# karenyang/GCN-VAE

Hardware: AMD Instinct MI355X
Metric: edges/sec R-GCN forward+backward, FB15k-237 emb=200 (higher is better)
Workload: dtype f32; 1 GPU; FB15k-237-shaped synthetic full graph (BASELINE configs[1]): 14541 entities, 474 directed relation types, E=544230 directed edges on this rank (544230 in the trained graph), 2-layer R-GCN-VAE bdd num_bases=100 emb_dim=200 dropout 0.2, 0 IAF blocks, DistMult decoder on T=220000 triplets per rank, step = fwd + loss(BCE+reg+KL+MMD) + bwd + clip + Adam; edges_per_gpu=544230, trained_graph_edges=544230, nodes=14541, triplets_per_gpu=220000, n_flows=0, gemm_precision=f32, launch=hipgraph, parallelism=single GPU, optimizer=replicated clip + Adam, k1_operands=f32

## Files before the change

### gcn-vae_amd/csrc/k_bdd.hip

```cpp
#include <stdlib.h>

#include "common.h"

namespace gv {

struct AggParams {
    const int4* items;
    int n_items;
    const int* nbr;
    const int* etype;
    const float* coef;
    const int* coef_idx;
    const float* feat;
    int ld_feat;
    const float* w;
    int w_row;
    const float* addend;
    int ld_add;
    int act;
    const uint8_t* keep;
    float keep_scale;
    float* out;
    int ld_out;
    float* partial;
    int out_dim;
    int nb;
    int p, q;
    int nbp;
};

__device__ __forceinline__ int rl_i(int v, int lane) { return __builtin_amdgcn_readlane(v, lane); }
__device__ __forceinline__ float rl_f(float v, int lane) {
    return __int_as_float(__builtin_amdgcn_readlane(__float_as_int(v), lane));
}


template <int P, int Q, bool TRANS, int BPL>
__device__ __forceinline__ void block_fma(const float (&x)[BPL * P], const float (&w)[BPL * P * Q], float c,
                                          float (&acc)[BPL * Q]) {
#pragma unroll
    for (int b = 0; b < BPL; ++b) {
#pragma unroll
        for (int q = 0; q < Q; ++q) {
            float t = 0.f;
#pragma unroll
            for (int p = 0; p < P; ++p) {
                const float wv = TRANS ? w[b * P * Q + q * P + p] : w[b * P * Q + p * Q + q];
                t = fmaf(x[b * P + p], wv, t);
            }
            acc[b * Q + q] = fmaf(t, c, acc[b * Q + q]);
        }
    }
}

template <int P, int Q, bool TRANS, int BPL, int U>
__global__ __launch_bounds__(256) void k_agg_fast(const AggParams a) {
    constexpr int GV = BPL * P, PV = BPL * Q, WV = BPL * P * Q;
    constexpr bool RUNS = P * Q >= 4;
    const int lane = threadIdx.x & 63;
    const int wave = __builtin_amdgcn_readfirstlane((int)(blockIdx.x * (blockDim.x >> 6) + (threadIdx.x >> 6)));
    if (wave >= a.n_items) return;
    const int4 it = a.items[wave];
    if (it.x < 0) return;
    if (it.w >= 0 && !a.partial) return;
    const bool active = lane * BPL < a.nbp;
    const int blk0 = blockIdx.y * a.nbp + lane * BPL;
    const float* __restrict__ fbase = a.feat + blk0 * P;
    const float* __restrict__ wbase = a.w + blk0 * (P * Q);

    float acc[PV];
#pragma unroll
    for (int i = 0; i < PV; ++i) acc[i] = 0.f;
    float wkeep[WV];
#pragma unroll
    for (int i = 0; i < WV; ++i) wkeep[i] = 0.f;
    int r_keep = -1;

    for (int e0 = it.y; e0 < it.z; e0 += 64) {
        const int cnt = min(64, it.z - e0);
        int my_n = 0, my_t = 0;
        float my_c = 1.f;
        if (lane < cnt) {
            my_n = a.nbr[e0 + lane];
            my_t = a.etype[e0 + lane];
            if (a.coef) my_c = a.coef_idx ? a.coef[a.coef_idx[e0 + lane]] : a.coef[e0 + lane];
// ... 634 lines not shown
#pragma unroll
                    for (int q = 0; q < QS; ++q) acc[p * QS + q] = fmaf(xc, gvv[q], acc[p * QS + q]);
                }
            }
        }
    }
    if (!active) return;
    float* o = (it.w >= 0 ? a.partial + (size_t)it.w * a.w_row : a.grad_w + (size_t)it.x * a.w_row) + blk * (P * Q) + sub * QS;
#pragma unroll
    for (int p = 0; p < P; ++p) {
        float t[QS];
#pragma unroll
        for (int q = 0; q < QS; ++q) t[q] = acc[p * QS + q];
        if (it.w < 0 && a.accumulate) {
            float old[QS];
            load_vec<QS>(o + p * Q, old);
#pragma unroll
            for (int q = 0; q < QS; ++q) t[q] += old[q];
        }
        store_vec<QS>(o + p * Q, t);
    }
}


__global__ __launch_bounds__(256) void k_gradw_generic(const GradWParams a) {
    const int lane = threadIdx.x & 63;
    const int wave = __builtin_amdgcn_readfirstlane((int)(blockIdx.x * (blockDim.x >> 6) + (threadIdx.x >> 6)));
    if (wave >= a.n_items) return;
    const int4 it = a.items[wave];
    if (it.x < 0) return;
    if (it.w >= 0 && !a.partial) return;
    const int P = a.p, Q = a.q;
    for (int c0 = 0; c0 < a.w_row; c0 += 64) {
        const int c = c0 + lane;
        const bool active = c < a.w_row;
        const int b = active ? c / (P * Q) : 0;
        const int rem = c - b * P * Q;
        const int p = rem / Q, q = rem - p * Q;
        float acc = 0.f;
        for (int e0 = it.y; e0 < it.z; e0 += 64) {
            const int cnt = min(64, it.z - e0);
            int my_s = 0, my_d = 0;
            float my_c = 1.f;
            if (lane < cnt) {
                my_s = a.src[e0 + lane];
                my_d = a.dst[e0 + lane];
                if (a.coef) my_c = a.coef_idx ? a.coef[a.coef_idx[e0 + lane]] : a.coef[e0 + lane];
            }
            for (int j = 0; j < cnt; ++j) {
                const int s = rl_i(my_s, j);
                const int d = rl_i(my_d, j);
                const float cf = rl_f(my_c, j);
                if (active)
                    acc = fmaf(a.x[(size_t)s * a.ld_x + b * P + p] * cf, a.g[(size_t)d * a.ld_g + b * Q + q], acc);
            }
        }
        if (!active) continue;
        if (it.w >= 0) {
            a.partial[(size_t)it.w * a.w_row + c] = acc;
        } else {
            float* o = a.grad_w + (size_t)it.x * a.w_row + c;
            *o = a.accumulate ? *o + acc : acc;
        }
    }
}

__global__ __launch_bounds__(256) void k_gradw_fixup(const int4* fix, int n_fix, const float* partial, int w_row,
                                                     float* grad_w, int accumulate) {
    const int lane = threadIdx.x & 63;
    const int tiles = (w_row + 63) >> 6;
    const int wave = __builtin_amdgcn_readfirstlane((int)(blockIdx.x * (blockDim.x >> 6) + (threadIdx.x >> 6)));
    if (wave >= n_fix * tiles) return;
    const int4 f = fix[wave / tiles];
    if (f.x < 0) return;
    const int c = (wave % tiles) * 64 + lane;
    if (c >= w_row) return;
    const float acc = ordered_slot_sum(partial + (size_t)f.y * w_row + c, f.z, w_row);
    float* o = grad_w + (size_t)f.x * w_row + c;
    *o = accumulate ? *o + acc : acc;
}

__global__ __launch_bounds__(256) void k_gradw_fixup4(const int4* fix, int n_fix, const float* partial, int w_row,
                                                      float* grad_w, int accumulate) {
    const int lane = threadIdx.x & 63;
    const int quads = w_row >> 2, tiles = (quads + 63) >> 6;
    const int wave = __builtin_amdgcn_readfirstlane((int)(blockIdx.x * (blockDim.x >> 6) + (threadIdx.x >> 6)));
    if (wave >= n_fix * tiles) return;
    const int4 f = fix[wave / tiles];
    if (f.x < 0) return;
    const int c4 = (wave % tiles) * 64 + lane;
    if (c4 >= quads) return;
    const float4* __restrict__ p = reinterpret_cast<const float4*>(partial + (size_t)f.y * w_row) + c4;
    const size_t stride = (size_t)quads;
    const int n = f.z;
    float4 a0 = make_float4(0.f, 0.f, 0.f, 0.f), a1 = a0, a2 = a0, a3 = a0;
    auto add = [](float4& a, const float4& v) { a.x += v.x; a.y += v.y; a.z += v.z; a.w += v.w; };
    int k = 0;
    for (; k + 8 <= n; k += 8) {
        const float4 v0 = p[(size_t)(k + 0) * stride], v1 = p[(size_t)(k + 1) * stride];
        const float4 v2 = p[(size_t)(k + 2) * stride], v3 = p[(size_t)(k + 3) * stride];
        const float4 v4 = p[(size_t)(k + 4) * stride], v5 = p[(size_t)(k + 5) * stride];
        const float4 v6 = p[(size_t)(k + 6) * stride], v7 = p[(size_t)(k + 7) * stride];
        add(a0, v0); add(a1, v1); add(a2, v2); add(a3, v3);
        add(a0, v4); add(a1, v5); add(a2, v6); add(a3, v7);
    }
    for (; k < n; ++k) add(a0, p[(size_t)k * stride]);
    float4 acc = make_float4((a0.x + a1.x) + (a2.x + a3.x), (a0.y + a1.y) + (a2.y + a3.y), (a0.z + a1.z) + (a2.z + a3.z),
                             (a0.w + a1.w) + (a2.w + a3.w));
    float4* o = reinterpret_cast<float4*>(grad_w + (size_t)f.x * w_row) + c4;
    if (accumulate) {
        const float4 t = *o;
        acc.x = t.x + acc.x; acc.y = t.y + acc.y; acc.z = t.z + acc.z; acc.w = t.w + acc.w;
    }
    *o = acc;
}

__global__ void k_items_count(const int* rowptr, int n_seg, int chunk, int* n_chunks, int* n_slots, int* is_split) {
    const int s = blockIdx.x * blockDim.x + threadIdx.x;
    if (s >= n_seg) return;
    const int deg = rowptr[s + 1] - rowptr[s];
    const int nch = max(1, (deg + chunk - 1) / chunk);
    n_chunks[s] = nch;
    n_slots[s] = nch > 1 ? nch : 0;
    is_split[s] = nch > 1 ? 1 : 0;
}

__global__ void k_items_fill(const int* rowptr, int n_seg, int chunk, const int* item_off, const int* slot_off,
                             const int* fix_off, int4* items, int4* fix) {
    const int s = blockIdx.x * blockDim.x + threadIdx.x;
    if (s >= n_seg) return;
    const int beg = rowptr[s], end = rowptr[s + 1];
    const int nch = max(1, (end - beg + chunk - 1) / chunk);
    const int ib = item_off[s];
    for (int k = 0; k < nch; ++k) {
        const int b = beg + k * chunk;
        items[ib + k] = make_int4(s, b, min(end, b + chunk), nch > 1 ? slot_off[s] + k : -1);
    }
    if (nch > 1) fix[fix_off[s]] = make_int4(s, slot_off[s], nch, 0);
}

template <typename K, typename Pm>
static int launch_items(K kern, const Pm& p, int n_items, hipStream_t st, const char* what, int parts = 1) {
    if (n_items <= 0) return GV_OK;
    const int waves_per_block = 4;
    dim3 grid((n_items + waves_per_block - 1) / waves_per_block, parts), block(64 * waves_per_block);
    hipLaunchKernelGGL(kern, grid, block, 0, st, p);
    return launch_status(what);
}

}

using namespace gv;

extern "C" int gv_segment_items_count(const int32_t* rowptr, int n_seg, int chunk, int32_t* n_chunks,
                                      int32_t* n_slots, int32_t* is_split, void* stream) {
    GV_REQUIRE(rowptr && n_chunks && n_slots && is_split, GV_ERR_NULL, "gv_segment_items_count: NULL pointer");
    GV_REQUIRE(n_seg >= 0 && chunk > 0, GV_ERR_SHAPE, "gv_segment_items_count: n_seg=%d chunk=%d", n_seg, chunk);
    if (n_seg == 0) return GV_OK;
    hipLaunchKernelGGL(k_items_count, dim3((n_seg + 255) / 256), dim3(256), 0, (hipStream_t)stream, rowptr, n_seg,
                       chunk, n_chunks, n_slots, is_split);
    return launch_status("gv_segment_items_count");
}

extern "C" int gv_segment_items_fill(const int32_t* rowptr, int n_seg, int chunk, const int32_t* item_off,
                                     const int32_t* slot_off, const int32_t* fix_off, int32_t* items, int32_t* fix,
                                     void* stream) {
    GV_REQUIRE(rowptr && item_off && slot_off && fix_off && items, GV_ERR_NULL, "gv_segment_items_fill: NULL pointer");
    GV_REQUIRE(n_seg >= 0 && chunk > 0, GV_ERR_SHAPE, "gv_segment_items_fill: n_seg=%d chunk=%d", n_seg, chunk);
    if (n_seg == 0) return GV_OK;
    hipLaunchKernelGGL(k_items_fill, dim3((n_seg + 255) / 256), dim3(256), 0, (hipStream_t)stream, rowptr, n_seg,
                       chunk, item_off, slot_off, fix_off, (int4*)items, (int4*)fix);
    return launch_status("gv_segment_items_fill");
}

namespace {
struct LanePlan { int bpl; int parts; };
bool lane_plan(int nb, int p, LanePlan* out, bool aggregate = false) {
    int cands[3] = {0, 0, 0};
    switch (p) {
        case 1: cands[0] = 4; cands[1] = 2; break;
        case 2: cands[0] = 2; cands[1] = 4; cands[2] = 1; break;
        case 4: cands[0] = 1; cands[1] = 2; break;
        case 8: cands[0] = 1; break;
        case 5: {
            static const int bpl1 = getenv("GV_K1_BPL1") ? atoi(getenv("GV_K1_BPL1")) : 1;
            if (bpl1 && aggregate) { cands[0] = 1; cands[1] = 2; } else cands[0] = 2;
            break;
        }
        case 10: cands[0] = 1; break;
        default: return false;
    }
    for (int c = 0; c < 3 && cands[c]; ++c) {
        const int bpl = cands[c];
        if (nb % bpl) continue;
        const int lanes = nb / bpl;
        for (int parts = 1; parts <= 16; ++parts) {
            if (lanes % parts) continue;
// ... 130 lines not shown
    const bool has_plan = lane_plan(num_bases, blk_in, &lp, true);
    const int bpl = has_plan ? lp.bpl : 0;
    if (rc == -1000) a.nbp = has_plan ? num_bases / lp.parts : num_bases;
#define GV_AGG_CASE(P_, Q_, T_, B_, U_)                                                               \
    if (rc == -1000 && vec_ok && blk_in == P_ && blk_out == Q_ && (transpose_w != 0) == T_ && bpl == B_) \
        rc = launch_items(k_agg_fast<P_, Q_, T_, B_, U_>, a, n_items, st, "gv_rgcn_bdd_aggregate", lp.parts);
#define GV_AGG_U(P_, Q_, T_, B_)                                                                              \
    if (rc == -1000 && u_env && vec_ok && blk_in == P_ && blk_out == Q_ && (transpose_w != 0) == T_ && bpl == B_) { \
        if (u_env == 2) rc = launch_items(k_agg_fast<P_, Q_, T_, B_, 2>, a, n_items, st, "agg(U2)", lp.parts);          \
        if (u_env == 4) rc = launch_items(k_agg_fast<P_, Q_, T_, B_, 4>, a, n_items, st, "agg(U4)", lp.parts);          \
        if (u_env == 8) rc = launch_items(k_agg_fast<P_, Q_, T_, B_, 8>, a, n_items, st, "agg(U8)", lp.parts);          \
    }
    GV_AGG_U(2, 2, false, 2) GV_AGG_U(2, 4, false, 2) GV_AGG_U(2, 2, true, 2) GV_AGG_U(4, 2, true, 2)
#undef GV_AGG_U
    GV_AGG_CASE(1, 1, false, 4, 8)
    GV_AGG_CASE(1, 2, false, 4, 4)
    GV_AGG_CASE(2, 2, false, 2, 8)
    GV_AGG_CASE(2, 4, false, 2, 4)
    GV_AGG_CASE(4, 4, false, 1, 4)
    GV_AGG_CASE(4, 4, false, 2, 2)
    GV_AGG_CASE(4, 8, false, 1, 2)
    GV_AGG_CASE(4, 8, false, 2, 2)
    GV_AGG_CASE(1, 1, true, 4, 8)
    GV_AGG_CASE(2, 1, true, 2, 8)
    GV_AGG_CASE(2, 2, true, 2, 8)
    GV_AGG_CASE(4, 2, true, 1, 8)
    GV_AGG_CASE(4, 2, true, 2, 4)
    GV_AGG_CASE(4, 4, true, 1, 4)
    GV_AGG_CASE(4, 4, true, 2, 2)
    GV_AGG_CASE(8, 4, true, 1, 2)
    GV_AGG_CASE(5, 5, false, 1, 2)
    GV_AGG_CASE(5, 10, false, 1, 2)
    GV_AGG_CASE(5, 5, true, 1, 2)
    GV_AGG_CASE(5, 5, false, 2, 2)
    GV_AGG_CASE(5, 10, false, 2, 1)
    GV_AGG_CASE(5, 5, true, 2, 2)
    GV_AGG_CASE(10, 5, true, 1, 1)
    GV_AGG_CASE(10, 10, false, 1, 1)
    GV_AGG_CASE(10, 10, true, 1, 1)
#undef GV_AGG_CASE
    if (rc == -1000) {
        if (transpose_w)
            rc = launch_items(k_agg_generic<true>, a, n_items, st, "gv_rgcn_bdd_aggregate(generic)");
        else
            rc = launch_items(k_agg_generic<false>, a, n_items, st, "gv_rgcn_bdd_aggregate(generic)");
    }
    if (rc != GV_OK) return rc;
    if (n_fix > 0) {
        const int pairs = n_fix * ((a.out_dim + 63) / 64);
        hipLaunchKernelGGL(k_agg_fixup, dim3(pairs), dim3(pairs >= 65536 ? 1024 : 256), 0, st, (const int4*)fix, n_fix, partial,
                           a.out_dim, addend, ld_addend, act, keep, keep_scale, out, ld_out);
        return launch_status("gv_rgcn_bdd_aggregate(fixup)");
    }
    return GV_OK;
}

extern "C" int gv_rgcn_bdd_fixup(const int32_t* fix, int n_fix, const float* partial, int out_dim, const float* addend,
                                 int ld_addend, int act, const uint8_t* keep, float keep_scale, float* out, int ld_out,
                                 void* stream) {
    GV_REQUIRE(n_fix >= 0, GV_ERR_SHAPE, "gv_rgcn_bdd_fixup: negative count");
    if (n_fix == 0) return GV_OK;
    GV_REQUIRE(fix && partial && out, GV_ERR_NULL, "gv_rgcn_bdd_fixup: NULL pointer");
    const int pairs = n_fix * ((out_dim + 63) / 64);
    hipLaunchKernelGGL(k_agg_fixup, dim3(pairs), dim3(pairs >= 65536 ? 1024 : 256), 0, (hipStream_t)stream, (const int4*)fix, n_fix,
                       partial, out_dim, addend, ld_addend, act, keep, keep_scale, out, ld_out);
    return launch_status("gv_rgcn_bdd_fixup");
}

extern "C" int gv_rgcn_bdd_grad_weight(const int32_t* items, int n_items, const int32_t* fix, int n_fix,
                                       const int32_t* src, const int32_t* dst, const float* coef,
                                       const int32_t* coef_idx, const float* x, int ld_x, const float* g, int ld_g,
                                       int num_bases, int blk_in, int blk_out, float* grad_w, float* partial,
                                       int accumulate, void* stream) {
    GV_REQUIRE(n_items >= 0 && n_fix >= 0, GV_ERR_SHAPE, "gv_rgcn_bdd_grad_weight: negative item count");
    if (n_items == 0) return GV_OK;
    GV_REQUIRE(items && x && g && grad_w, GV_ERR_NULL, "gv_rgcn_bdd_grad_weight: NULL pointer");
    GV_REQUIRE(num_bases > 0 && blk_in > 0 && blk_out > 0, GV_ERR_SHAPE, "gv_rgcn_bdd_grad_weight: bad block sizes");
    GV_REQUIRE(n_fix == 0 || (fix && partial), GV_ERR_NULL, "gv_rgcn_bdd_grad_weight: split segments need fix+partial");
    GV_REQUIRE(ld_x >= num_bases * blk_in && ld_g >= num_bases * blk_out, GV_ERR_SHAPE,
               "gv_rgcn_bdd_grad_weight: leading dimension smaller than the row");
    GradWParams a;
    a.items = (const int4*)items; a.n_items = n_items; a.src = src; a.dst = dst; a.coef = coef; a.coef_idx = coef_idx;
    a.x = x; a.ld_x = ld_x; a.g = g; a.ld_g = ld_g; a.grad_w = grad_w; a.w_row = num_bases * blk_in * blk_out;
    a.partial = partial; a.accumulate = accumulate; a.nb = num_bases; a.p = blk_in; a.q = blk_out;
    hipStream_t st = (hipStream_t)stream;
    const bool vec_ok = aligned16(x) && aligned16(g) && aligned16(grad_w) && (ld_x % 4 == 0) && (ld_g % 4 == 0) &&
                        (!partial || aligned16(partial)) && (a.w_row % 4 == 0);
    int rc = -1000;
#define GV_GW_SPLIT(P_, Q_, QS_, U_, PARTS_)                                                                              \
    if (rc == -1000 && vec_ok && blk_in == P_ && blk_out == Q_ && num_bases % PARTS_ == 0 && num_bases <= 32 &&          \
        (num_bases / PARTS_) * (Q_ / QS_) <= 64) {                                                                        \
        a.nbp = num_bases / PARTS_;                                                                                       \
        rc = launch_items(k_gradw_split<P_, Q_, QS_, U_>, a, n_items, st, "gv_rgcn_bdd_grad_weight(split)", PARTS_);      \
    }
    GV_GW_SPLIT(10, 10, 5, 2, 1) GV_GW_SPLIT(10, 20, 4, 2, 2)
#undef GV_GW_SPLIT
    LanePlan lp{0, 1};
    const bool has_plan = lane_plan(num_bases, blk_in, &lp, blk_in == 5 && blk_out >= 10);
    const int bpl = has_plan ? lp.bpl : 0;
    if (rc == -1000) a.nbp = has_plan ? num_bases / lp.parts : num_bases;
#define GV_GW_CASE(P_, Q_, B_, U_)                                                  \
    if (rc == -1000 && vec_ok && blk_in == P_ && blk_out == Q_ && bpl == B_)        \
        rc = launch_items(k_gradw_fast<P_, Q_, B_, U_>, a, n_items, st, "gv_rgcn_bdd_grad_weight", lp.parts);
    GV_GW_CASE(1, 1, 4, 8)
    GV_GW_CASE(1, 2, 4, 4)
    GV_GW_CASE(2, 2, 2, 8)
    GV_GW_CASE(2, 4, 2, 4)
    GV_GW_CASE(4, 4, 1, 4)
    GV_GW_CASE(4, 4, 2, 2)
    GV_GW_CASE(4, 8, 1, 2)
    GV_GW_CASE(4, 8, 2, 2)
    GV_GW_CASE(5, 5, 2, 2)
    GV_GW_CASE(5, 10, 2, 1)
    GV_GW_CASE(5, 10, 1, 2)
    GV_GW_CASE(10, 10, 1, 1)
#undef GV_GW_CASE
    if (rc == -1000) rc = launch_items(k_gradw_generic, a, n_items, st, "gv_rgcn_bdd_grad_weight(generic)");
    if (rc != GV_OK) return rc;
    if (n_fix > 0) {
        if (a.w_row % 4 == 0 && aligned16(partial) && aligned16(grad_w)) {
            const int waves = n_fix * ((a.w_row / 4 + 63) / 64);
            hipLaunchKernelGGL(k_gradw_fixup4, dim3((waves + 3) / 4), dim3(256), 0, st, (const int4*)fix, n_fix, partial,
                               a.w_row, grad_w, accumulate);
        } else {
            const int waves = n_fix * ((a.w_row + 63) / 64);
            hipLaunchKernelGGL(k_gradw_fixup, dim3((waves + 3) / 4), dim3(256), 0, st, (const int4*)fix, n_fix, partial,
                               a.w_row, grad_w, accumulate);
        }
        return launch_status("gv_rgcn_bdd_grad_weight(fixup)");
    }
    return GV_OK;
}
```

### gcn-vae_amd/csrc/k_gemm.hip

```cpp
#include <limits.h>
#include <stdlib.h>

#include <algorithm>

#include "common.h"

namespace gv {


typedef float f32x16 __attribute__((ext_vector_type(16)));

struct GemmParams {
    const float* a;
    const float* b;
    float* c;
    const float* bias;
    const float* a_mask;
    float* ws;
    int m, n, k, lda, ldb, ldc;
    int act, accumulate, split_k, k_chunk;
    int vec_a, vec_b;
    const int* rows_dev;
    const unsigned long long* kmask;
    const unsigned long long* tmask;
    int tmask_ld;
    int tmask_wanted;
};

template <int VPT>
__device__ __forceinline__ void load_run(const float* src, int pos, int lim, bool ok, bool vec, float (&r)[VPT], int off) {
#pragma unroll
    for (int h = 0; h < VPT / 4; ++h) {
        const int q = pos + 4 * h;
        if (ok && vec && q + 3 < lim) {
            const float4 v = *reinterpret_cast<const float4*>(src + 4 * h);
            r[off + 4 * h] = v.x; r[off + 4 * h + 1] = v.y; r[off + 4 * h + 2] = v.z; r[off + 4 * h + 3] = v.w;
        } else {
#pragma unroll
            for (int i = 0; i < 4; ++i) r[off + 4 * h + i] = (ok && q + i < lim) ? src[4 * h + i] : 0.f;
        }
    }
}

template <int VPT>
__device__ __forceinline__ void mask_run(const float* msk, int pos, int lim, bool ok, bool vec, float (&r)[VPT]) {
    float mv[VPT];
    load_run<VPT>(msk, pos, lim, ok, vec, mv, 0);
#pragma unroll
    for (int i = 0; i < VPT; ++i) r[i] = mv[i] > 0.f ? r[i] : 0.f;
}

template <bool TA, int BM, int BK>
__device__ __forceinline__ void load_a(const GemmParams& p, int m0, int k0, int kend, float (&r)[BM * BK / 256]) {
    constexpr int APT = BM * BK / 256;
    const int t = threadIdx.x;
    if constexpr (!TA) {
        constexpr int TPR = BK / APT;
        const int m = m0 + t / TPR, kk = k0 + (t % TPR) * APT;
        load_run<APT>(p.a + (size_t)m * p.lda + kk, kk, kend, m < p.m, p.vec_a, r, 0);
        if (p.a_mask) mask_run<APT>(p.a_mask + (size_t)m * p.lda + kk, kk, kend, m < p.m, p.vec_a, r);
    } else {
        constexpr int TPK = BM / APT;
        const int kq = k0 + t / TPK, m = m0 + (t % TPK) * APT;
        load_run<APT>(p.a + (size_t)kq * p.lda + m, m, p.m, kq < kend, p.vec_a, r, 0);
        if (p.a_mask) mask_run<APT>(p.a_mask + (size_t)kq * p.lda + m, m, p.m, kq < kend, p.vec_a, r);
    }
}

template <bool TB, int BN, int BK>
__device__ __forceinline__ void load_b(const GemmParams& p, int n0, int k0, int kend, float (&r)[BN * BK / 256]) {
    constexpr int BPT = BN * BK / 256;
    const int t = threadIdx.x;
    if constexpr (!TB) {
        constexpr int TPK = BN / BPT;
        const int kq = k0 + t / TPK, n = n0 + (t % TPK) * BPT;
        load_run<BPT>(p.b + (size_t)kq * p.ldb + n, n, p.n, kq < kend, p.vec_b, r, 0);
    } else {
        constexpr int TPN = BK / BPT;
        const int n = n0 + t / TPN, kq = k0 + (t % TPN) * BPT;
        load_run<BPT>(p.b + (size_t)n * p.ldb + kq, kq, kend, n < p.n, p.vec_b, r, 0);
    }
}

template <bool TA, int BM, int BK>
__device__ __forceinline__ void stage_a(float* As, const float (&r)[BM * BK / 256]) {
    constexpr int APT = BM * BK / 256, LDA_S = BM + 1;
    const int t = threadIdx.x;
    if constexpr (!TA) {
// ... 670 lines not shown
    const float* src = base + (size_t)row * ld + kk;
    load_run<8>(src, kk, kend, ok, vec, r, 0);
    if (mask) mask_run<8>(mask + (size_t)row * ld + kk, kk, kend, ok, vec, r);
}

__device__ __forceinline__ void hb_load_ks(const float* base, const float* mask, int ld, int row0, int rows, int k0, int kend,
                                           float (&r)[8]) {
    const int t = threadIdx.x;
    const int row = row0 + (t & 63), kk = k0 + (t >> 6) * 8;
    const bool ok = row < rows;
#pragma unroll
    for (int j = 0; j < 8; ++j) {
        const bool in = ok && kk + j < kend;
        float v = in ? base[(size_t)(kk + j) * ld + row] : 0.f;
        if (mask && in) v = mask[(size_t)(kk + j) * ld + row] > 0.f ? v : 0.f;
        r[j] = v;
    }
}

template <bool KC>
__device__ __forceinline__ void hb_stage(__bf16* S, const float (&r)[8]) {
    const int t = threadIdx.x;
    const int row = KC ? (t >> 2) : (t & 63), kk = KC ? (t & 3) * 8 : (t >> 6) * 8;
    bf16x8 v;
#pragma unroll
    for (int j = 0; j < 8; ++j) v[j] = (__bf16)r[j];
    *reinterpret_cast<bf16x8*>(S + row * HB_LD + kk) = v;
}

template <bool TA, bool TB>
__global__ __launch_bounds__(256) void k_gemm_bf16(const GemmParams p) {
    __shared__ __attribute__((aligned(16))) __bf16 As[64 * HB_LD];
    __shared__ __attribute__((aligned(16))) __bf16 Bs[64 * HB_LD];
    const int m0 = blockIdx.y * 64, n0 = blockIdx.x * 64;
    const int kbeg = blockIdx.z * p.k_chunk;
    const int kend = min(p.k, kbeg + p.k_chunk);
    const int lane = threadIdx.x & 63, wid = threadIdx.x >> 6;
    const int wm = (wid >> 1) * 32, wn = (wid & 1) * 32;
    const int l31 = lane & 31, lhi = lane >> 5;
    f32x16 acc;
#pragma unroll
    for (int i = 0; i < 16; ++i) acc[i] = 0.f;

    float ra[8], rb[8];
    auto load_tiles = [&](int k0) {
        if constexpr (!TA) hb_load_kc(p.a, p.a_mask, p.lda, m0, p.m, k0, kend, p.vec_a, ra);
        else hb_load_ks(p.a, p.a_mask, p.lda, m0, p.m, k0, kend, ra);
        if constexpr (TB) hb_load_kc(p.b, nullptr, p.ldb, n0, p.n, k0, kend, p.vec_b, rb);
        else hb_load_ks(p.b, nullptr, p.ldb, n0, p.n, k0, kend, rb);
    };
    load_tiles(kbeg);
    for (int k0 = kbeg; k0 < kend; k0 += HB_BK) {
        hb_stage<!TA>(As, ra);
        hb_stage<TB>(Bs, rb);
        __syncthreads();
        if (k0 + HB_BK < kend) load_tiles(k0 + HB_BK);
#pragma unroll
        for (int kk = 0; kk < HB_BK; kk += 16) {
            const bf16x8 af = *reinterpret_cast<const bf16x8*>(As + (wm + l31) * HB_LD + kk + 8 * lhi);
            const bf16x8 bf = *reinterpret_cast<const bf16x8*>(Bs + (wn + l31) * HB_LD + kk + 8 * lhi);
            acc = __builtin_amdgcn_mfma_f32_32x32x16_bf16(af, bf, acc, 0, 0, 0);
        }
        __syncthreads();
    }
    const int col = n0 + wn + l31;
    if (col >= p.n) return;
    const float bv = (p.bias && p.split_k == 1) ? p.bias[col] : 0.f;
#pragma unroll
    for (int r = 0; r < 16; ++r) {
        const int row = m0 + wm + (r & 3) + 8 * (r >> 2) + 4 * lhi;
        if (row >= p.m) continue;
        float v = acc[r];
        if (p.split_k > 1) {
            p.ws[((size_t)blockIdx.z * p.m + row) * p.n + col] = v;
        } else {
            v = apply_act(v + bv, p.act);
            float* dst = p.c + (size_t)row * p.ldc + col;
            *dst = p.accumulate ? *dst + v : v;
        }
    }
}

__global__ __launch_bounds__(256) void k_gemm_splitk_reduce(const GemmParams p) {
    const size_t total = (size_t)p.m * p.n;
    for (size_t i = (size_t)blockIdx.x * blockDim.x + threadIdx.x; i < total; i += (size_t)gridDim.x * blockDim.x) {
        float a0 = 0.f, a1 = 0.f, a2 = 0.f, a3 = 0.f;
        int z = 0;
        for (; z + 8 <= p.split_k; z += 8) {
            float t[8];
#pragma unroll
            for (int q = 0; q < 8; ++q) t[q] = p.ws[(size_t)(z + q) * total + i];
            a0 += t[0]; a1 += t[1]; a2 += t[2]; a3 += t[3];
            a0 += t[4]; a1 += t[5]; a2 += t[6]; a3 += t[7];
        }
        for (; z < p.split_k; ++z) a0 += p.ws[(size_t)z * total + i];
        float v = (a0 + a1) + (a2 + a3);
        const int row = (int)(i / p.n), col = (int)(i - (size_t)row * p.n);
        if (p.tmask_wanted > 0) {
            const int bit = (row >> 6) * p.tmask_ld + (col >> 6);
            if (!((p.tmask[bit >> 6] >> (bit & 63)) & 1ull)) v = 0.f;
        }
        if (p.bias) v += p.bias[col];
        v = apply_act(v, p.act);
        float* dst = p.c + (size_t)row * p.ldc + col;
        *dst = p.accumulate ? *dst + v : v;
    }
}

constexpr int COLSUM_SLICES = 64;

__global__ __launch_bounds__(256) void k_colsum_part(const float* x, const float* msk, int64_t m, int n, int ld, float* part) {
    __shared__ float sm[4][64];
    const int lane = threadIdx.x & 63, w = threadIdx.x >> 6;
    const int c = blockIdx.x * 64 + lane;
    const int64_t per = (m + gridDim.y - 1) / gridDim.y;
    const int64_t r0 = blockIdx.y * per, r1 = min(m, r0 + per);
    float a0 = 0.f, a1 = 0.f, a2 = 0.f, a3 = 0.f;
    if (c < n) {
        int64_t r = r0 + w;
        if (msk) {
            for (; r + 12 < r1; r += 16) {
                const float v0 = x[r * ld + c], v1 = x[(r + 4) * ld + c], v2 = x[(r + 8) * ld + c], v3 = x[(r + 12) * ld + c];
                const float m0 = msk[r * ld + c], m1 = msk[(r + 4) * ld + c], m2 = msk[(r + 8) * ld + c], m3 = msk[(r + 12) * ld + c];
                a0 += m0 > 0.f ? v0 : 0.f; a1 += m1 > 0.f ? v1 : 0.f; a2 += m2 > 0.f ? v2 : 0.f; a3 += m3 > 0.f ? v3 : 0.f;
            }
            for (; r < r1; r += 4) a0 += msk[r * ld + c] > 0.f ? x[r * ld + c] : 0.f;
        } else {
            for (; r + 12 < r1; r += 16) {
                const float v0 = x[r * ld + c], v1 = x[(r + 4) * ld + c], v2 = x[(r + 8) * ld + c], v3 = x[(r + 12) * ld + c];
                a0 += v0; a1 += v1; a2 += v2; a3 += v3;
            }
            for (; r < r1; r += 4) a0 += x[r * ld + c];
        }
    }
    sm[w][lane] = (a0 + a1) + (a2 + a3);
    __syncthreads();
    if (w == 0 && c < n) part[(size_t)blockIdx.y * n + c] = (sm[0][lane] + sm[1][lane]) + (sm[2][lane] + sm[3][lane]);
}

__global__ __launch_bounds__(256) void k_colsum_final(const float* part, int n, int nsl, float* out, int accumulate) {
    const int c = blockIdx.x * blockDim.x + threadIdx.x;
    if (c >= n) return;
    float a0 = 0.f, a1 = 0.f, a2 = 0.f, a3 = 0.f;
    int s = 0;
    for (; s + 4 <= nsl; s += 4) {
        const float v0 = part[(size_t)s * n + c], v1 = part[(size_t)(s + 1) * n + c];
        const float v2 = part[(size_t)(s + 2) * n + c], v3 = part[(size_t)(s + 3) * n + c];
        a0 += v0; a1 += v1; a2 += v2; a3 += v3;
    }
    for (; s < nsl; ++s) a0 += part[(size_t)s * n + c];
    const float acc = (a0 + a1) + (a2 + a3);
    out[c] = accumulate ? out[c] + acc : acc;
}

__global__ __launch_bounds__(1024) void k_colsum_final_wide(const float* part, int n, int nsl, float* out, int accumulate) {
    __shared__ float sm[64][16];
    const int c = blockIdx.x * 16 + (threadIdx.x & 15);
    const float acc = sum_slices_16x64(part, n, nsl, c, sm);
    if ((threadIdx.x >> 4) == 0 && c < n) out[c] = accumulate ? out[c] + acc : acc;
}

}

using namespace gv;

static int k_chunk_for(int k, int split_k) {
    int per = (k + split_k - 1) / split_k;
    return ((per + 31) / 32) * 32;
}

extern "C" int64_t gv_gemm_workspace_bytes(int m, int n, int k, int split_k) {
    (void)k;
    return split_k > 1 ? (int64_t)split_k * m * n * (int64_t)sizeof(float) : 0;
}

static int gemm_any(bool bf16, int trans_a, int trans_b, int m, int n, int k, const float* a, int lda, const float* b,
                    int ldb, float* c, int ldc, const float* bias, int act, int accumulate, int split_k,
                    const float* a_relu_mask, void* workspace, int64_t workspace_bytes, void* stream, const int32_t* rows_dev = nullptr,
                    const uint64_t* kmask = nullptr, const uint64_t* tmask = nullptr, int tiles_wanted = 0) {
    GV_REQUIRE(m >= 0 && n >= 0 && k >= 0, GV_ERR_SHAPE, "gv_gemm_f32: negative size");
    if (m == 0 || n == 0) return GV_OK;
    GV_REQUIRE(c && (k == 0 || (a && b)), GV_ERR_NULL, "gv_gemm_f32: NULL matrix");
    GV_REQUIRE(lda >= (trans_a ? m : k) && ldb >= (trans_b ? k : n) && ldc >= n, GV_ERR_SHAPE,
               "gv_gemm_f32: leading dimension too small (lda=%d ldb=%d ldc=%d)", lda, ldb, ldc);
    GV_REQUIRE(act == GV_ACT_NONE || act == GV_ACT_RELU, GV_ERR_SHAPE, "gv_gemm_f32: unknown act %d", act);
    if (split_k < 1) split_k = 1;
    if (k == 0) split_k = 1;
    GemmParams p;
    p.a = a; p.b = b; p.c = c; p.bias = bias; p.a_mask = a_relu_mask; p.ws = (float*)workspace;
    p.m = m; p.n = n; p.k = k; p.lda = lda; p.ldb = ldb; p.ldc = ldc;
    p.act = act; p.accumulate = accumulate;
    p.k_chunk = k_chunk_for(k > 0 ? k : 1, split_k);
    split_k = k > 0 ? (k + p.k_chunk - 1) / p.k_chunk : 1;
    p.split_k = split_k;
    p.vec_a = aligned16(a) && (lda % 4 == 0) && (!a_relu_mask || aligned16(a_relu_mask));
    p.vec_b = aligned16(b) && (ldb % 4 == 0);
    p.rows_dev = bf16 ? nullptr : rows_dev;
    GV_REQUIRE(!kmask || (!bf16 && split_k == 1 && k <= 64 * 16), GV_ERR_SHAPE,
               "gv_gemm_f32_sparse: k-chunk words cover fp32 products of k <= 1024 without split-K (k=%d split_k=%d)", k, split_k);
    GV_REQUIRE(!tmask || !bf16, GV_ERR_SHAPE, "gv_gemm_f32_sparse: fp32 only");
    p.kmask = (const unsigned long long*)kmask;
    p.tmask = (const unsigned long long*)tmask;
    p.tmask_ld = (n + 63) / 64;
    GV_REQUIRE(tiles_wanted >= 0 && tiles_wanted <= ((m + 63) / 64) * ((n + 63) / 64), GV_ERR_SHAPE, "gv_gemm_f32_sparse: c_tiles_wanted=%d", tiles_wanted);
    p.tmask_wanted = (tmask && tiles_wanted > 0 && split_k > 1) ? tiles_wanted : 0;
    if (split_k > 1) {
        GV_REQUIRE(workspace, GV_ERR_NULL, "gv_gemm_f32: split_k needs a workspace");
        GV_REQUIRE(workspace_bytes >= gv_gemm_workspace_bytes(m, n, k, split_k), GV_ERR_WORKSPACE,
                   "gv_gemm_f32: workspace %lld < %lld bytes", (long long)workspace_bytes,
                   (long long)gv_gemm_workspace_bytes(m, n, k, split_k));
    }
    hipStream_t st = (hipStream_t)stream;
    if (bf16) {
        dim3 grid((n + 63) / 64, (m + 63) / 64, split_k), block(256);
        if (!trans_a && !trans_b) hipLaunchKernelGGL((k_gemm_bf16<false, false>), grid, block, 0, st, p);
        else if (!trans_a && trans_b) hipLaunchKernelGGL((k_gemm_bf16<false, true>), grid, block, 0, st, p);
        else if (trans_a && !trans_b) hipLaunchKernelGGL((k_gemm_bf16<true, false>), grid, block, 0, st, p);
        else hipLaunchKernelGGL((k_gemm_bf16<true, true>), grid, block, 0, st, p);
        int rcb = launch_status("gv_gemm_bf16");
        if (rcb != GV_OK) return rcb;
        if (split_k > 1) {
            const size_t total = (size_t)m * n;
            const int blocks = (int)min((size_t)2048, (total + 255) / 256);
            hipLaunchKernelGGL(k_gemm_splitk_reduce, dim3(blocks), dim3(256), 0, st, p);
            return launch_status("gv_gemm_bf16(split-k reduce)");
        }
        return GV_OK;
    }
    static const int mt_env = getenv("GV_GEMM_MT") ? atoi(getenv("GV_GEMM_MT")) : 0;
    static const int nt_env = getenv("GV_GEMM_NT") ? atoi(getenv("GV_GEMM_NT")) : 0;
    static const int bk_env = getenv("GV_GEMM_BK") ? atoi(getenv("GV_GEMM_BK")) : 0;
    const int nt = (nt_env == 2 && !kmask && !(tmask && tiles_wanted > 0 && split_k > 1)) ? 2 : 1;
    const int bn = 64 * nt;
    const long blocks128 = (long)((n + bn - 1) / bn) * ((m + 127) / 128) * split_k;
    const int mt = p.tmask_wanted ? 1 : (mt_env ? mt_env : (blocks128 >= 1024 ? 2 : 1));
    static const int sparse_bk = getenv("GV_GEMM_SPARSE_BK") ? atoi(getenv("GV_GEMM_SPARSE_BK")) : 16;
    const int bk = kmask ? (sparse_bk == 32 ? 32 : 16) : (bk_env ? (bk_env == 16 ? 16 : 32) : (trans_a ? 32 : 16));
    dim3 grid((n + bn - 1) / bn, (m + 64 * mt - 1) / (64 * mt), split_k), block(256);
    if (p.tmask_wanted) { grid.x = p.tmask_wanted; grid.y = 1; }
#define GV_GEMM_CFG(TA_, TB_, MT_, NT_, BK_) \
    if (mt == MT_ && nt == NT_ && bk == BK_) hipLaunchKernelGGL((k_gemm_f32<TA_, TB_, MT_, NT_, BK_>), grid, block, 0, st, p);
#define GV_GEMM_LAUNCH(TA_, TB_)                                                                       \
    do {                                                                                               \
        GV_GEMM_CFG(TA_, TB_, 1, 1, 16) GV_GEMM_CFG(TA_, TB_, 1, 1, 32) GV_GEMM_CFG(TA_, TB_, 1, 2, 16) \
        GV_GEMM_CFG(TA_, TB_, 1, 2, 32) GV_GEMM_CFG(TA_, TB_, 2, 1, 16) GV_GEMM_CFG(TA_, TB_, 2, 1, 32) \
        GV_GEMM_CFG(TA_, TB_, 2, 2, 16) GV_GEMM_CFG(TA_, TB_, 2, 2, 32)                                 \
    } while (0)
    if (!trans_a && !trans_b) GV_GEMM_LAUNCH(false, false);
    else if (!trans_a && trans_b) GV_GEMM_LAUNCH(false, true);
    else if (trans_a && !trans_b) GV_GEMM_LAUNCH(true, false);
    else GV_GEMM_LAUNCH(true, true);
#undef GV_GEMM_LAUNCH
#undef GV_GEMM_CFG
    int rc = launch_status("gv_gemm_f32");
    if (rc != GV_OK) return rc;
    if (split_k > 1) {
        const size_t total = (size_t)m * n;
        const int blocks = (int)min((size_t)2048, (total + 255) / 256);
        hipLaunchKernelGGL(k_gemm_splitk_reduce, dim3(blocks), dim3(256), 0, st, p);
        return launch_status("gv_gemm_f32(split-k reduce)");
    }
    return GV_OK;
}

extern "C" int gv_gemm_f32(int trans_a, int trans_b, int m, int n, int k, const float* a, int lda, const float* b,
                           int ldb, float* c, int ldc, const float* bias, int act, int accumulate, int split_k,
                           const float* a_relu_mask, void* workspace, int64_t workspace_bytes, void* stream) {
    return gemm_any(false, trans_a, trans_b, m, n, k, a, lda, b, ldb, c, ldc, bias, act, accumulate, split_k, a_relu_mask,
                    workspace, workspace_bytes, stream);
}

extern "C" int gv_gemm_f32_live_rows(int trans_a, int trans_b, int m, int n, int k, const float* a, int lda, const float* b,
                                     int ldb, float* c, int ldc, const float* bias, int act, int accumulate, int split_k,
                                     const float* a_relu_mask, void* workspace, int64_t workspace_bytes, const int32_t* rows_dev,
                                     void* stream) {
    return gemm_any(false, trans_a, trans_b, m, n, k, a, lda, b, ldb, c, ldc, bias, act, accumulate, split_k, a_relu_mask,
                    workspace, workspace_bytes, stream, rows_dev);
}

extern "C" int gv_gemm_f32_sparse(int trans_a, int trans_b, int m, int n, int k, const float* a, int lda, const float* b, int ldb,
                                  float* c, int ldc, const float* bias, int act, int accumulate, int split_k, const float* a_relu_mask,
                                  void* workspace, int64_t workspace_bytes, const int32_t* rows_dev, const uint64_t* b_k_chunks,
                                  const uint64_t* c_tiles, int c_tiles_wanted, void* stream) {
    return gemm_any(false, trans_a, trans_b, m, n, k, a, lda, b, ldb, c, ldc, bias, act, accumulate, split_k, a_relu_mask,
                    workspace, workspace_bytes, stream, rows_dev, b_k_chunks, c_tiles, c_tiles_wanted);
}

extern "C" int gv_gemm_bf16(int trans_a, int trans_b, int m, int n, int k, const float* a, int lda, const float* b,
                            int ldb, float* c, int ldc, const float* bias, int act, int accumulate, int split_k,
                            const float* a_relu_mask, void* workspace, int64_t workspace_bytes, void* stream) {
    return gemm_any(true, trans_a, trans_b, m, n, k, a, lda, b, ldb, c, ldc, bias, act, accumulate, split_k, a_relu_mask,
                    workspace, workspace_bytes, stream);
}

extern "C" int gv_rank_scores(const float* q, int ld_q, const float* e, int ld_e, const int* target, const float* bias,
                              float* tgt, int* count, int m, int v, int h, void* stream) {
    GV_REQUIRE(m >= 0 && v > 0 && h > 0, GV_ERR_SHAPE, "gv_rank_scores: m=%d v=%d h=%d", m, v, h);
    if (m == 0) return GV_OK;
    GV_REQUIRE(q && e && target && tgt && count, GV_ERR_NULL, "gv_rank_scores: NULL pointer");
    GV_REQUIRE(ld_q >= h && ld_e >= h, GV_ERR_SHAPE, "gv_rank_scores: leading dimension too small");
    RankParams rp;
    GemmParams& p = rp.g;
    p.a = q; p.b = e; p.c = nullptr; p.bias = nullptr; p.a_mask = nullptr; p.ws = nullptr;
    p.m = m; p.n = v; p.k = h; p.lda = ld_q; p.ldb = ld_e; p.ldc = v;
    p.act = GV_ACT_NONE; p.accumulate = 0; p.split_k = 1; p.k_chunk = h;
    p.vec_a = aligned16(q) && (ld_q % 4 == 0);
    p.vec_b = aligned16(e) && (ld_e % 4 == 0);
    p.rows_dev = nullptr; p.kmask = nullptr; p.tmask = nullptr; p.tmask_ld = 0; p.tmask_wanted = 0;
    rp.target = target; rp.bias = bias; rp.tgt = tgt; rp.count = count;
    hipStream_t st = (hipStream_t)stream;
    if (fill_words(count, 0u, (size_t)m * sizeof(int), st) != hipSuccess) return launch_status("gv_rank_scores(fill)");
    dim3 grid((v + 63) / 64, (m + 63) / 64), block(256);
    hipLaunchKernelGGL(k_rank_scores<0>, grid, block, 0, st, rp);
    hipLaunchKernelGGL(k_rank_scores<1>, grid, block, 0, st, rp);
    return launch_status("gv_rank_scores");
}

extern "C" int gv_rank_scores_filtered(const float* q, int ld_q, const float* e, int ld_e, const int* target, const float* bias,
                                       const int* filt_lo, const int* filt_hi, const int* filt_ent, int n_filt_ent, float* tgt,
                                       int* count_raw, int* count_filt, int m, int v, int h, void* stream) {
    GV_REQUIRE(m >= 0 && v > 0 && h > 0 && n_filt_ent >= 0, GV_ERR_SHAPE, "gv_rank_scores_filtered: m=%d v=%d h=%d n_filt_ent=%d",
               m, v, h, n_filt_ent);
    if (m == 0) return GV_OK;
    GV_REQUIRE(q && e && target && tgt && count_filt, GV_ERR_NULL, "gv_rank_scores_filtered: NULL pointer");
    GV_REQUIRE(filt_lo && filt_hi && filt_ent, GV_ERR_NULL, "gv_rank_scores_filtered: NULL filter pointer");
    GV_REQUIRE(ld_q >= h && ld_e >= h, GV_ERR_SHAPE, "gv_rank_scores_filtered: leading dimension too small");
    RankFiltParams fp;
    RankParams& rp = fp.rp;
    GemmParams& p = rp.g;
    p.a = q; p.b = e; p.c = nullptr; p.bias = nullptr; p.a_mask = nullptr; p.ws = nullptr;
    p.m = m; p.n = v; p.k = h; p.lda = ld_q; p.ldb = ld_e; p.ldc = v;
    p.act = GV_ACT_NONE; p.accumulate = 0; p.split_k = 1; p.k_chunk = h;
    p.vec_a = aligned16(q) && (ld_q % 4 == 0);
    p.vec_b = aligned16(e) && (ld_e % 4 == 0);
    p.rows_dev = nullptr; p.kmask = nullptr; p.tmask = nullptr; p.tmask_ld = 0; p.tmask_wanted = 0;
    rp.target = target; rp.bias = bias; rp.tgt = tgt; rp.count = count_raw;
    fp.filt_lo = filt_lo; fp.filt_hi = filt_hi; fp.filt_ent = filt_ent; fp.n_ent = n_filt_ent; fp.count_filt = count_filt;
    hipStream_t st = (hipStream_t)stream;
    if (count_raw && fill_words(count_raw, 0u, (size_t)m * sizeof(int), st) != hipSuccess)
// ... 118 lines not shown
```

### gcn-vae_amd/csrc/k_loss.hip

```cpp
#include "common.h"

namespace gv {

constexpr int RED_BLOCKS = 1024;

__device__ __forceinline__ float block_sum_256(float v, float* sm ) {
    v = wave_sum(v);
    const int lane = threadIdx.x & 63, w = threadIdx.x >> 6;
    __syncthreads();
    if (lane == 0) sm[w] = v;
    __syncthreads();
    return sm[0] + sm[1] + sm[2] + sm[3];
}

__global__ __launch_bounds__(256) void k_final_sum(const float* part, int n, float scale, float* out, int accumulate) {
    __shared__ float sm[4];
    float acc = 0.f;
    for (int i = threadIdx.x; i < n; i += 256) acc += part[i];
    const float tot = block_sum_256(acc, sm);
    if (threadIdx.x == 0) *out = accumulate ? *out + scale * tot : scale * tot;
}

__global__ __launch_bounds__(256) void k_loss_combine(const float* p0, int n0, float s0, const float* p1, int n1, float s1,
                                                      const float* p2, int n2, float s2, const float* p3, int n3, float s3,
                                                      float w1, float w2, float w3, float* scal, float* loss,
                                                      const int* rows_dev, float rows_host) {
    __shared__ float sm[4];
    const float* ps[4] = {p0, p1, p2, p3};
    const int ns[4] = {n0, n1, n2, n3};
    if (rows_dev) s2 *= rows_host / (float)*rows_dev;
    const float ss[4] = {s0, s1, s2, s3};
    float term[4];
#pragma unroll
    for (int j = 0; j < 4; ++j) {
        float acc = 0.f;
        if (ps[j])
            for (int i = threadIdx.x; i < ns[j]; i += 256) acc += ps[j][i];
        term[j] = ss[j] * block_sum_256(acc, sm);
    }
    if (threadIdx.x == 0) {
        if (scal) { scal[0] = term[0]; scal[1] = term[1]; scal[2] = term[2]; scal[3] = term[3]; }
        float v = term[0];
        if (p1) v += w1 * term[1];
        if (p2) v += w2 * term[2];
        if (p3) v += w3 * term[3];
        *loss = v;
    }
}

__global__ __launch_bounds__(256) void k_distmult_bce(const float* e, int ld_e, const float* w, int ld_w,
                                                      const int* trip, const int* order, const float* labels,
                                                      const float* bias, float* score, float* part, int64_t T, int h) {
    __shared__ float sm[4];
    const int sub = threadIdx.x & 15;
    const float bv = bias ? *bias : 0.f;
    const bool vec = (h % 4 == 0) && (ld_e % 4 == 0) && (ld_w % 4 == 0);
    float lsum = 0.f;
    const int n_x = gridDim.x >= 8 ? 8 : 1;
    const int64_t per = (T + n_x - 1) / n_x;
    const int64_t lo = (blockIdx.x % n_x) * per, hi = min(T, lo + per);
    const int brank = blockIdx.x / n_x, bper = (gridDim.x + n_x - 1 - (blockIdx.x % n_x)) / n_x;
    auto triplet_dot = [&](int64_t t) -> float {
        const int s = trip[3 * t], r = trip[3 * t + 1], o = trip[3 * t + 2];
        const float* es = e + (size_t)s * ld_e;
        const float* eo = e + (size_t)o * ld_e;
        const float* wr = w + (size_t)r * ld_w;
        float acc = 0.f;
        if (vec && h <= 256) {
            float4 a[4], b[4], d[4];
#pragma unroll
            for (int q = 0; q < 4; ++q) {
                const int c = sub * 4 + 64 * q;
                if (c < h) {
                    a[q] = *reinterpret_cast<const float4*>(es + c);
                    b[q] = *reinterpret_cast<const float4*>(wr + c);
                    d[q] = *reinterpret_cast<const float4*>(eo + c);
                }
            }
#pragma unroll
            for (int q = 0; q < 4; ++q) {
                if (sub * 4 + 64 * q < h) {
                    acc = fmaf(a[q].x * b[q].x, d[q].x, acc);
                    acc = fmaf(a[q].y * b[q].y, d[q].y, acc);
// ... 616 lines not shown
                    *reinterpret_cast<float4*>(gh2 + r * 2 * h + h + col) = make_float4(o1[0], o1[1], o1[2], o1[3]);
                } else {
                    *reinterpret_cast<float4*>(gz + r * h + col) = make_float4(o0[0], o0[1], o0[2], o0[3]);
                    *reinterpret_cast<float4*>(gm + r * h + col) = make_float4(o1[0], o1[1], o1[2], o1[3]);
                    *reinterpret_cast<float4*>(gv + r * h + col) = make_float4(o2[0], o2[1], o2[2], o2[3]);
                }
            }
        }
    }
    for (int j0 = 0; j0 < k; j0 += KLB_KR) {
        __syncthreads();
#pragma unroll
        for (int j = 0; j < KT; ++j) {
            if (j >= j0 && j < j0 + KLB_KR && j < k) {
                red[((2 * (j - j0)) * KLB_WAVES + w) * 64 + lane] = make_float4(amu[j][0], amu[j][1], amu[j][2], amu[j][3]);
                red[((2 * (j - j0) + 1) * KLB_WAVES + w) * 64 + lane] = make_float4(av[j][0], av[j][1], av[j][2], av[j][3]);
            }
        }
        __syncthreads();
        const int j = j0 + (w >> 1), kind = w & 1;
        if (w < 2 * KLB_KR && j < k && ok) {
            float4 t = red[((2 * (j - j0) + kind) * KLB_WAVES) * 64 + lane];
#pragma unroll
            for (int q = 1; q < KLB_WAVES; ++q) {
                const float4 x = red[((2 * (j - j0) + kind) * KLB_WAVES + q) * 64 + lane];
                t.x += x.x; t.y += x.y; t.z += x.z; t.w += x.w;
            }
            float4 o;
            if (kind == 0) {
                const float4 i24 = si2[j * h4];
                o = make_float4(-t.x * 2.f * i24.x, -t.y * 2.f * i24.y, -t.z * 2.f * i24.z, -t.w * 2.f * i24.w);
            } else {
                o = make_float4(-t.x, -t.y, -t.z, -t.w);
            }
            *reinterpret_cast<float4*>(part + ((size_t)blockIdx.y * 2 * k + (kind ? k : 0) + j) * h + col) = o;
        }
    }
}

__global__ __launch_bounds__(256) void k_kl_bwd_mix_part(const float* z, const float* mix, const float* resp,
                                                         float* part, int64_t n, int h, int k) {
    __shared__ float sm[2][4][64];
    const int j = blockIdx.x, slice = blockIdx.z, nsl = gridDim.z;
    const int lane = threadIdx.x & 63, w = threadIdx.x >> 6;
    const int c = blockIdx.y * 64 + lane;
    const int64_t per = (n + nsl - 1) / nsl;
    const int64_t r0 = slice * per, r1 = min(n, r0 + per);
    const int kh = k * h;
    float gmu0 = 0.f, gmu1 = 0.f, gv0 = 0.f, gv1 = 0.f;
    const bool ok = c < h;
    const float muj = ok ? mix[j * h + c] : 0.f, i2 = ok ? mix[kh + j * h + c] : 0.f;
    if (ok) {
        int64_t r = r0 + w;
        for (; r + 4 < r1; r += 8) {
            const float ra = resp[r * k + j], rb = resp[(r + 4) * k + j];
            const float da = z[r * h + c] - muj, db = z[(r + 4) * h + c] - muj;
            gmu0 += ra * da;
            gmu1 += rb * db;
            gv0 += ra * (da * da * 2.f * i2 * i2 - i2);
            gv1 += rb * (db * db * 2.f * i2 * i2 - i2);
        }
        for (; r < r1; r += 4) {
            const float ra = resp[r * k + j];
            const float da = z[r * h + c] - muj;
            gmu0 += ra * da;
            gv0 += ra * (da * da * 2.f * i2 * i2 - i2);
        }
    }
    sm[0][w][lane] = gmu0 + gmu1;
    sm[1][w][lane] = gv0 + gv1;
    __syncthreads();
    if (w == 0 && ok) {
        const float gmu = (sm[0][0][lane] + sm[0][1][lane]) + (sm[0][2][lane] + sm[0][3][lane]);
        const float gvv = (sm[1][0][lane] + sm[1][1][lane]) + (sm[1][2][lane] + sm[1][3][lane]);
        part[((size_t)slice * 2 * k + j) * h + c] = -gmu * 2.f * i2;
        part[((size_t)slice * 2 * k + k + j) * h + c] = -gvv;
    }
}

__global__ __launch_bounds__(1024) void k_kl_bwd_mix_final(const float* part, const float* z_pre, const float* gkl,
                                                           float gscale, float* g_zpre, int accumulate, int64_t n, int h,
                                                           int k, int nsl, const int* rows_dev) {
    __shared__ float sm[64][16];
    const int total = 2 * k * h, kh = k * h;
    const int i = blockIdx.x * 16 + (threadIdx.x & 15);
    float acc = sum_slices_16x64(part, total, nsl, i, sm);
    if ((threadIdx.x >> 4) != 0 || i >= total) return;
    const float cg = gscale * (gkl ? *gkl : 1.f) / (float)(rows_dev ? (int64_t)*rows_dev : n);
    if (i >= kh) {
        const float raw = z_pre[i];
        acc *= raw > 20.f ? 1.f : 1.f / (1.f + expf(-raw));
    }
    g_zpre[i] = accumulate ? g_zpre[i] + cg * acc : cg * acc;
}

constexpr int MMD_WAVES = 16;

template <int CPL>
__device__ __forceinline__ void mmd_load_row(const float* p, int h, int lane, float (&v)[CPL]) {
#pragma unroll
    for (int i = 0; i < CPL; ++i) v[i] = (lane + 64 * i < h) ? p[lane + 64 * i] : 0.f;
}

template <int CPL>
__device__ __forceinline__ float mmd_d2(const float (&a)[CPL], const float (&b)[CPL]) {
    float d2 = 0.f;
#pragma unroll
    for (int i = 0; i < CPL; ++i) { const float d = a[i] - b[i]; d2 = fmaf(d, d, d2); }
    return d2;
}

template <int CPL>
__global__ __launch_bounds__(64 * MMD_WAVES) void k_mmd_fwd(const float* x, const float* y, const int64_t* yidx, int sx, int sy,
                                                             int h, float* part) {
    __shared__ float sm[MMD_WAVES];
    const int lane = threadIdx.x & 63, w = threadIdx.x >> 6;
    const bool is_x = (int)blockIdx.x < sx;
    auto row_of = [&](bool from_y, int j) -> const float* {
        return from_y ? y + (size_t)(yidx ? yidx[j] : j) * h : x + (size_t)j * h;
    };
    float av[CPL];
    mmd_load_row<CPL>(row_of(!is_x, is_x ? (int)blockIdx.x : (int)blockIdx.x - sx), h, lane, av);
    const float inv = 1.f / ((float)h * (float)h);
    float tot = 0.f;
    for (int pass = 0; pass < (is_x ? 2 : 1); ++pass) {
        const bool b_is_y = pass == 0 ? !is_x : true;
        const int nb = pass == 0 ? (is_x ? sx : sy) : sy;
        const float wt = pass == 0 ? 1.f / ((float)nb * (float)nb) : -2.f / ((float)sx * (float)sy);
        for (int j = w; j < nb; j += 4 * MMD_WAVES) {
            float b0[CPL], b1[CPL], b2[CPL], b3[CPL];
            const int j1 = j + MMD_WAVES, j2 = j + 2 * MMD_WAVES, j3 = j + 3 * MMD_WAVES;
            mmd_load_row<CPL>(row_of(b_is_y, j), h, lane, b0);
            mmd_load_row<CPL>(row_of(b_is_y, min(j1, nb - 1)), h, lane, b1);
            mmd_load_row<CPL>(row_of(b_is_y, min(j2, nb - 1)), h, lane, b2);
            mmd_load_row<CPL>(row_of(b_is_y, min(j3, nb - 1)), h, lane, b3);
            const float d0 = wave_sum(mmd_d2<CPL>(av, b0)), d1 = wave_sum(mmd_d2<CPL>(av, b1));
            const float d2 = wave_sum(mmd_d2<CPL>(av, b2)), d3 = wave_sum(mmd_d2<CPL>(av, b3));
            tot += wt * expf(-d0 * inv);
            if (j1 < nb) tot += wt * expf(-d1 * inv);
            if (j2 < nb) tot += wt * expf(-d2 * inv);
            if (j3 < nb) tot += wt * expf(-d3 * inv);
        }
    }
    if (lane == 0) sm[w] = tot;
    __syncthreads();
    if (threadIdx.x == 0) {
        float s = 0.f;
#pragma unroll
        for (int i = 0; i < MMD_WAVES; ++i) s += sm[i];
        part[blockIdx.x] = s;
    }
}

template <int CPL>
__global__ __launch_bounds__(64 * MMD_WAVES) void k_mmd_bwd(const float* x, const float* y, const int64_t* yidx, int sx, int sy,
                                                             int h, const float* gmmd, float gscale, float* gx, float* gy) {
    __shared__ float sm[MMD_WAVES][64 * CPL];
    const int lane = threadIdx.x & 63, w = threadIdx.x >> 6;
    const bool is_x = (int)blockIdx.x < sx;
    const int row = is_x ? blockIdx.x : blockIdx.x - sx;
    auto row_of = [&](bool from_y, int j) -> const float* {
        return from_y ? y + (size_t)(yidx ? yidx[j] : j) * h : x + (size_t)j * h;
    };
    float av[CPL], acc[CPL];
    mmd_load_row<CPL>(row_of(!is_x, row), h, lane, av);
#pragma unroll
    for (int i = 0; i < CPL; ++i) acc[i] = 0.f;
    const float inv = 1.f / ((float)h * (float)h);
    const float g = gscale * (gmmd ? *gmmd : 1.f);
    const int n_same = is_x ? sx : sy, n_other = is_x ? sy : sx;
    const float c_same = g * (-2.f * inv) * 2.f / ((float)n_same * (float)n_same);
    const float c_other = g * (-2.f * inv) * (-2.f) / ((float)sx * (float)sy);
    for (int pass = 0; pass < 2; ++pass) {
        const bool b_is_y = pass == 0 ? !is_x : is_x;
        const int nb = pass == 0 ? n_same : n_other;
        const float cf = pass == 0 ? c_same : c_other;
// ... 101 lines not shown
#pragma unroll
    for (int g = 0; g < G; ++g) { col[g] = 4 * (l16 + 16 * g); on[g] = col[g] < h; }
    float4 av[G], acc[G];
    mmd_load_row4<G>(row_of(!is_x, row), on, col, av);
#pragma unroll
    for (int g = 0; g < G; ++g) acc[g] = make_float4(0.f, 0.f, 0.f, 0.f);
    const float inv = 1.f / ((float)h * (float)h);
    const float gg = gscale * (gmmd ? *gmmd : 1.f);
    const int n_same = is_x ? sx : sy, n_other = is_x ? sy : sx;
    const float c_same = gg * (-2.f * inv) * 2.f / ((float)n_same * (float)n_same);
    const float c_other = gg * (-2.f * inv) * (-2.f) / ((float)sx * (float)sy);
    for (int pass = 0; pass < 2; ++pass) {
        const bool b_is_y = pass == 0 ? !is_x : is_x;
        const int nb = pass == 0 ? n_same : n_other;
        const float cf = pass == 0 ? c_same : c_other;
        for (int j0 = 0; j0 < nb; j0 += 2 * NG) {
            const int j = j0 + grp, j1 = j + NG;
            float4 b0[G], b1[G];
            mmd_load_row4<G>(row_of(b_is_y, min(j, nb - 1)), on, col, b0);
            mmd_load_row4<G>(row_of(b_is_y, min(j1, nb - 1)), on, col, b1);
            const float d0 = row16_sum(mmd_d2_4<G>(av, b0)), d1 = row16_sum(mmd_d2_4<G>(av, b1));
            const float k0 = j < nb ? cf * expf(-d0 * inv) : 0.f, k1 = j1 < nb ? cf * expf(-d1 * inv) : 0.f;
#pragma unroll
            for (int g = 0; g < G; ++g) {
                acc[g].x = fmaf(k0, av[g].x - b0[g].x, fmaf(k1, av[g].x - b1[g].x, acc[g].x));
                acc[g].y = fmaf(k0, av[g].y - b0[g].y, fmaf(k1, av[g].y - b1[g].y, acc[g].y));
                acc[g].z = fmaf(k0, av[g].z - b0[g].z, fmaf(k1, av[g].z - b1[g].z, acc[g].z));
                acc[g].w = fmaf(k0, av[g].w - b0[g].w, fmaf(k1, av[g].w - b1[g].w, acc[g].w));
            }
        }
    }
#pragma unroll
    for (int g = 0; g < G; ++g) {
        float4 t;
        t.x = (rl_dyn(acc[g].x, l16) + rl_dyn(acc[g].x, 16 + l16)) + (rl_dyn(acc[g].x, 32 + l16) + rl_dyn(acc[g].x, 48 + l16));
        t.y = (rl_dyn(acc[g].y, l16) + rl_dyn(acc[g].y, 16 + l16)) + (rl_dyn(acc[g].y, 32 + l16) + rl_dyn(acc[g].y, 48 + l16));
        t.z = (rl_dyn(acc[g].z, l16) + rl_dyn(acc[g].z, 16 + l16)) + (rl_dyn(acc[g].z, 32 + l16) + rl_dyn(acc[g].z, 48 + l16));
        t.w = (rl_dyn(acc[g].w, l16) + rl_dyn(acc[g].w, 16 + l16)) + (rl_dyn(acc[g].w, 32 + l16) + rl_dyn(acc[g].w, 48 + l16));
        if (lane < 16) sm[w][l16 + 16 * g] = t;
    }
    __syncthreads();
    const bool indexed = !is_x && yidx;
    float* o = is_x ? gx + (size_t)row * h : gy + (size_t)(yidx ? yidx[row] : row) * h;
    for (int q = threadIdx.x; q < (h >> 2); q += 64 * MMD_WAVES) {
        float4 s4 = sm[0][q];
#pragma unroll
        for (int i = 1; i < MMD_WAVES; ++i) { const float4 t = sm[i][q]; s4.x += t.x; s4.y += t.y; s4.z += t.z; s4.w += t.w; }
        if (indexed) {
            atomicAdd(o + 4 * q, s4.x); atomicAdd(o + 4 * q + 1, s4.y); atomicAdd(o + 4 * q + 2, s4.z); atomicAdd(o + 4 * q + 3, s4.w);
        } else {
            *reinterpret_cast<float4*>(o + 4 * q) = s4;
        }
    }
}

__global__ __launch_bounds__(256) void k_prior_sample_fwd(const float* z_pre, const float* eps, float* out, int s, int k, int h) {
    const int total = s * h;
    for (int i = blockIdx.x * 256 + threadIdx.x; i < total; i += gridDim.x * 256) {
        const int r = i / h, c = i - r * h, j = r % k;
        const float v = softplus_t(z_pre[(size_t)(k + j) * h + c]) + 1e-8f;
        out[i] = z_pre[(size_t)j * h + c] + eps[i] * sqrtf(v);
    }
}

__global__ __launch_bounds__(256) void k_prior_sample_bwd(const float* z_pre, const float* eps, const float* g, float* gz_pre,
                                                          int accumulate, int s, int k, int h) {
    const int total = k * h;
    for (int i = blockIdx.x * 256 + threadIdx.x; i < total; i += gridDim.x * 256) {
        const int j = i / h, c = i - j * h;
        const float raw = z_pre[(size_t)(k + j) * h + c];
        const float v = softplus_t(raw) + 1e-8f;
        float gm = 0.f, gs = 0.f;
        for (int r = j; r < s; r += k) {
            gm += g[(size_t)r * h + c];
            gs += g[(size_t)r * h + c] * eps[(size_t)r * h + c];
        }
        const float gr = gs * 0.5f / sqrtf(v) * (raw > 20.f ? 1.f : 1.f / (1.f + expf(-raw)));
        gz_pre[i] = accumulate ? gz_pre[i] + gm : gm;
        gz_pre[total + i] = accumulate ? gz_pre[total + i] + gr : gr;
    }
}

constexpr int KL_SLICES = 256;
constexpr int KL_FUSED_KT = 16;

}

using namespace gv;

#define GV_ST ((hipStream_t)stream)

static int red_blocks(int64_t n, int per_block) {
    int64_t b = (n + per_block - 1) / per_block;
    return (int)(b < 1 ? 1 : (b > RED_BLOCKS ? RED_BLOCKS : b));
}

static int sq2_blocks(int64_t n, int cap) {
    const int b = red_blocks(n, 4096);
    return b > cap ? cap : b;
}

static int kl_blocks(int64_t n) { return (int)((n + 3) / 4 > RED_BLOCKS ? RED_BLOCKS : (n + 3) / 4); }

extern "C" int gv_distmult_bce_fwd(const float* embed, int ld_e, const float* w_rel, int ld_w,
                                   const int32_t* triplets, const int32_t* order, const float* labels, const float* bias,
                                   float* score, float* loss, float* workspace, int64_t t, int h, void* stream) {
    GV_REQUIRE(embed && w_rel && triplets && labels && score && workspace, GV_ERR_NULL,
               "gv_distmult_bce_fwd: NULL pointer");
    GV_REQUIRE(t > 0 && h > 0 && ld_e >= h && ld_w >= h, GV_ERR_SHAPE, "gv_distmult_bce_fwd: bad shape");
    const int nb = red_blocks(t, 16);
    hipLaunchKernelGGL(k_distmult_bce, dim3(nb), dim3(256), 0, GV_ST, embed, ld_e, w_rel, ld_w, triplets, order, labels,
                       bias, score, workspace, t, h);
    if (loss) hipLaunchKernelGGL(k_final_sum, dim3(1), dim3(256), 0, GV_ST, workspace, nb, 1.f / (float)t, loss, 0);
    return launch_status("gv_distmult_bce_fwd");
}

extern "C" int gv_bce_grad(const float* score, const float* labels, const float* gloss, float* dscore,
                           const int32_t* pos3, float* dscore_inc, float* dscore_rel, float* dbias, float* workspace,
                           int64_t t, void* stream) {
    GV_REQUIRE(score && labels && dscore && workspace, GV_ERR_NULL, "gv_bce_grad: NULL pointer");
    GV_REQUIRE(!pos3 || (dscore_inc && dscore_rel), GV_ERR_NULL, "gv_bce_grad: pos3 needs dscore_inc and dscore_rel");
    GV_REQUIRE(t > 0, GV_ERR_SHAPE, "gv_bce_grad: t=%lld", (long long)t);
    const int nb = red_blocks(t, 256);
    hipLaunchKernelGGL(k_bce_grad, dim3(nb), dim3(256), 0, GV_ST, score, labels, gloss, dscore, pos3, dscore_inc,
                       dscore_rel, workspace, t);
    if (dbias) hipLaunchKernelGGL(k_final_sum, dim3(1), dim3(256), 0, GV_ST, workspace, nb, 1.f, dbias, 0);
    return launch_status("gv_bce_grad");
}

extern "C" int gv_mean_sq(const float* x, int64_t n, float scale, float* out, float* workspace, int accumulate,
                          void* stream) {
    GV_REQUIRE(x && out && workspace, GV_ERR_NULL, "gv_mean_sq: NULL pointer");
    GV_REQUIRE(n > 0, GV_ERR_SHAPE, "gv_mean_sq: n=%lld", (long long)n);
    const int nb = red_blocks(n, 4096);
    hipLaunchKernelGGL(k_sumsq_part, dim3(nb), dim3(256), 0, GV_ST, x, n, workspace);
    hipLaunchKernelGGL(k_final_sum, dim3(1), dim3(256), 0, GV_ST, workspace, nb, scale, out, accumulate);
    return launch_status("gv_mean_sq");
}

__global__ __launch_bounds__(256) void k_sumsq2_part(const float* x1, int64_t n1, float s1, int nb1, const float* x2,
                                                     int64_t n2, float s2, float* part, const int* rows_dev, int64_t rows_host) {
    __shared__ float sm[4];
    if (rows_dev) {
        const int64_t rows = *rows_dev;
        n1 = n1 / rows_host * rows;
        s1 *= (float)rows_host / (float)rows;
    }
    const bool first = (int)blockIdx.x < nb1;
    const float* x = first ? x1 : x2;
    const int64_t n = first ? n1 : n2;
    const int b = first ? blockIdx.x : blockIdx.x - nb1, nb = first ? nb1 : gridDim.x - nb1;
    float acc = 0.f;
    for (int64_t i = (int64_t)b * 256 + threadIdx.x; i < n; i += (int64_t)nb * 256) acc = fmaf(x[i], x[i], acc);
    const float tot = block_sum_256(acc, sm);
    if (threadIdx.x == 0) part[blockIdx.x] = tot * (first ? s1 : s2);
}

extern "C" int gv_mean_sq2(const float* x1, int64_t n1, float scale1, const float* x2, int64_t n2, float scale2, float* out,
                           float* workspace, const int32_t* rows_dev, int64_t rows_host, void* stream) {
    GV_REQUIRE(x1 && x2 && workspace, GV_ERR_NULL, "gv_mean_sq2: NULL pointer");
    GV_REQUIRE(n1 > 0 && n2 > 0, GV_ERR_SHAPE, "gv_mean_sq2: empty input");
    GV_REQUIRE(!rows_dev || (rows_host > 0 && n1 % rows_host == 0), GV_ERR_SHAPE, "gv_mean_sq2: rows_host=%lld does not divide n1",
               (long long)rows_host);
    const int nb1 = sq2_blocks(n1, 768), nb2 = sq2_blocks(n2, 255);
    hipLaunchKernelGGL(k_sumsq2_part, dim3(nb1 + nb2), dim3(256), 0, GV_ST, x1, n1, scale1, nb1, x2, n2, scale2, workspace, rows_dev,
                       rows_host);
// ... 67 lines not shown
                    (!eps || aligned16(eps)) && (!gz_up || aligned16(gz_up)) && (!gh2 || aligned16(gh2));
    if (!env || h % 4 != 0 || h > 1024 || k > 10 || !al) return false;
    const size_t lds = ((size_t)2 * k * h / 4 + (size_t)2 * KLB_KR * KLB_WAVES * 64) * sizeof(float4);
    if (lds > 128 * 1024) return false;
    static unsigned long long lds_done = 0;
    if (lds > 64 * 1024 && !raise_dynamic_lds((const void*)k_kl_bwd_cols4<10>, 128 * 1024, lds_done, "gv_kl_bwd")) return false;
#define GV_KLB(KT_) hipLaunchKernelGGL(k_kl_bwd_cols4<KT_>, dim3((h + 255) / 256, KL_SLICES), dim3(64 * KLB_WAVES), lds, st, z, m, ld_m, v, mix, resp, gkl, \
                                       gscale, z_extra, gz, gm, gv, part, n, h, k, rows_dev, h2, eps, gz_up, gh2)
    GV_KLB(10);
#undef GV_KLB
    return true;
}

extern "C" int gv_kl_bwd(const float* z, const float* m, int ld_m, const float* v, const float* z_pre,
                         const float* resp, const float* gkl, float gscale, float z_extra, float* gz, float* gm,
                         float* gv, float* g_zpre, int accumulate_zpre, float* workspace, int mix_ready, int64_t n, int h,
                         int k, const int32_t* rows_dev, void* stream) {
    GV_REQUIRE(z && m && v && z_pre && resp && gz && gm && gv && g_zpre && workspace, GV_ERR_NULL,
               "gv_kl_bwd: NULL pointer");
    GV_REQUIRE(n > 0 && h > 0 && k > 0 && k <= KL_KMAX && ld_m >= h, GV_ERR_SHAPE, "gv_kl_bwd: bad shape");
    float* mix = workspace;
    if (!mix_ready) hipLaunchKernelGGL(k_kl_mix, dim3((k * h + 255) / 256), dim3(256), 0, GV_ST, z_pre, k, h, mix);
    float* part = workspace + 3 * (size_t)k * h + RED_BLOCKS;
    if (kl_bwd_cols4(GV_ST, z, m, ld_m, v, mix, resp, gkl, gscale, z_extra, gz, gm, gv, part, n, h, k, rows_dev, nullptr, nullptr,
                     nullptr, nullptr)) {
    } else if (k <= KL_FUSED_KT) {
        hipLaunchKernelGGL(k_kl_bwd_fused<KL_FUSED_KT>, dim3((h + 63) / 64, KL_SLICES), dim3(256), 0, GV_ST, z, m, ld_m, v, mix,
                           resp, gkl, gscale, z_extra, gz, gm, gv, part, n, h, k, rows_dev);
    } else {
        GV_REQUIRE(!rows_dev, GV_ERR_SHAPE, "gv_kl_bwd: rows_dev needs k <= %d mixture components", KL_FUSED_KT);
        const size_t lds = (size_t)2 * k * h * sizeof(float);
        const int nb = (int)((n + 3) / 4 > 1024 ? 1024 : (n + 3) / 4);
        hipLaunchKernelGGL(k_kl_bwd_nodes, dim3(nb), dim3(256), lds, GV_ST, z, m, ld_m, v, mix, resp, gkl, gscale, z_extra,
                           gz, gm, gv, n, h, k);
        hipLaunchKernelGGL(k_kl_bwd_mix_part, dim3(k, (h + 63) / 64, KL_SLICES), dim3(256), 0, GV_ST, z, mix, resp, part, n,
                           h, k);
    }
    hipLaunchKernelGGL(k_kl_bwd_mix_final, dim3((2 * k * h + 15) / 16), dim3(1024), 0, GV_ST, part, z_pre, gkl,
                       gscale, g_zpre, accumulate_zpre, n, h, k, KL_SLICES, rows_dev);
    return launch_status("gv_kl_bwd");
}

extern "C" int gv_reparam_kl_fwd(const float* h2, const float* eps, const float* z_pre, float* z, float* v, float* m_out,
                                 float* resp, float* workspace, int64_t n, int h, int k, void* stream) {
    GV_REQUIRE(h2 && eps && z_pre && z && v && resp && workspace, GV_ERR_NULL, "gv_reparam_kl_fwd: NULL pointer");
    GV_REQUIRE(n > 0 && h > 0 && h <= 1024 && k > 0 && k <= KL_KMAX, GV_ERR_SHAPE, "gv_reparam_kl_fwd: n=%lld h=%d k=%d", (long long)n,
               h, k);
    const size_t lds = (size_t)2 * k * h * sizeof(float);
    GV_REQUIRE(lds <= 64 * 1024, GV_ERR_SHAPE, "gv_reparam_kl_fwd: mixture table %zu B exceeds the 64 KiB LDS budget", lds);
    float* mix = workspace;
    float* part = workspace + 3 * (size_t)k * h;
    hipLaunchKernelGGL(k_kl_mix, dim3((k * h + 255) / 256), dim3(256), 0, GV_ST, z_pre, k, h, mix);
    const int nb = kl_blocks(n);
    const float* none = nullptr;
    const int* no_rows = nullptr;
#define GV_RKL_FWD(CPL_)                                                                                                       \
    hipLaunchKernelGGL(k_kl_fwd<CPL_>, dim3(nb), dim3(256), lds, GV_ST, none, none, h, none, (const float*)mix, none, resp, part, n, h, \
                       k, no_rows, h2, eps, z, v, m_out)
    if (kl_fwd_v4(nb, lds, GV_ST, none, none, h, none, mix, none, resp, part, n, h, k, no_rows, h2, eps, z, v, m_out)) {}
    else if (h <= 64) GV_RKL_FWD(1);
    else if (h <= 128) GV_RKL_FWD(2);
    else if (h <= 256) GV_RKL_FWD(4);
    else if (h <= 512) GV_RKL_FWD(8);
    else GV_RKL_FWD(16);
#undef GV_RKL_FWD
    return launch_status("gv_reparam_kl_fwd");
}

extern "C" int gv_reparam_kl_bwd(const float* z, const float* h2, const float* v, const float* eps, const float* z_pre,
                                 const float* resp, const float* gkl, float gscale, float z_extra, const float* gz_up,
                                 float* gh2, float* g_zpre, int accumulate_zpre, float* workspace, int64_t n, int h, int k,
                                 void* stream) {
    GV_REQUIRE(z && h2 && v && eps && z_pre && resp && gh2 && g_zpre && workspace, GV_ERR_NULL, "gv_reparam_kl_bwd: NULL pointer");
    GV_REQUIRE(n > 0 && h > 0 && k > 0 && k <= KL_FUSED_KT, GV_ERR_SHAPE, "gv_reparam_kl_bwd: n=%lld h=%d k=%d (k <= %d)", (long long)n,
               h, k, KL_FUSED_KT);
    float* mix = workspace;
    float* part = workspace + 3 * (size_t)k * h + RED_BLOCKS;
    float* none = nullptr;
    const int* no_rows = nullptr;
    if (!kl_bwd_cols4(GV_ST, z, h2, 2 * h, v, mix, resp, gkl, gscale, z_extra, none, none, none, part, n, h, k, no_rows, h2, eps, gz_up,
                      gh2))
        hipLaunchKernelGGL(k_kl_bwd_fused<KL_FUSED_KT>, dim3((h + 63) / 64, KL_SLICES), dim3(256), 0, GV_ST, z, h2, 2 * h, v,
                           (const float*)mix, resp, gkl, gscale, z_extra, none, none, none, part, n, h, k, no_rows, h2, eps, gz_up, gh2);
    hipLaunchKernelGGL(k_kl_bwd_mix_final, dim3((2 * k * h + 15) / 16), dim3(1024), 0, GV_ST, (const float*)part, z_pre, gkl, gscale,
                       g_zpre, accumulate_zpre, n, h, k, KL_SLICES, no_rows);
    return launch_status("gv_reparam_kl_bwd");
}

__global__ void k_lincomb(const float* a0, float c0, const float* a1, float c1, const float* a2, float c2, const float* a3,
                          float c3, float* out) {
    if (threadIdx.x == 0 && blockIdx.x == 0) {
        float v = 0.f;
        if (a0) v += c0 * *a0;
        if (a1) v += c1 * *a1;
        if (a2) v += c2 * *a2;
        if (a3) v += c3 * *a3;
        *out = v;
    }
}

extern "C" int gv_lincomb4(const float* a0, float c0, const float* a1, float c1, const float* a2, float c2,
                           const float* a3, float c3, float* out, void* stream) {
    GV_REQUIRE(out, GV_ERR_NULL, "gv_lincomb4: NULL output");
    hipLaunchKernelGGL(k_lincomb, dim3(1), dim3(64), 0, GV_ST, a0, c0, a1, c1, a2, c2, a3, c3, out);
    return launch_status("gv_lincomb4");
}

extern "C" int gv_mmd_fwd(const float* x, const float* y, const int64_t* y_index, int sx, int sy, int h, float* mmd,
                          float* workspace, void* stream) {
    GV_REQUIRE(x && y && workspace, GV_ERR_NULL, "gv_mmd_fwd: NULL pointer");
    GV_REQUIRE(sx > 0 && sy > 0 && h > 0 && h <= 1024 && sx + sy <= RED_BLOCKS, GV_ERR_SHAPE,
               "gv_mmd_fwd: sx=%d sy=%d h=%d (need h <= 1024, sx+sy <= %d)", sx, sy, h, RED_BLOCKS);
    static const int v2 = getenv("GV_MMD_ROWS16") ? atoi(getenv("GV_MMD_ROWS16")) : 1;
    const bool al = h % 4 == 0 && aligned16(x) && aligned16(y);
    if (v2 && al && h <= 256) hipLaunchKernelGGL(k_mmd_fwd_g<4>, dim3(sx + sy), dim3(64 * MMD_WAVES), 0, GV_ST, x, y, y_index, sx, sy, h, workspace);
    else if (v2 && al && h <= 512) hipLaunchKernelGGL(k_mmd_fwd_g<8>, dim3(sx + sy), dim3(64 * MMD_WAVES), 0, GV_ST, x, y, y_index, sx, sy, h, workspace);
    else if (h <= 256) hipLaunchKernelGGL(k_mmd_fwd<4>, dim3(sx + sy), dim3(64 * MMD_WAVES), 0, GV_ST, x, y, y_index, sx, sy, h, workspace);
    else hipLaunchKernelGGL(k_mmd_fwd<16>, dim3(sx + sy), dim3(64 * MMD_WAVES), 0, GV_ST, x, y, y_index, sx, sy, h, workspace);
    if (mmd) hipLaunchKernelGGL(k_final_sum, dim3(1), dim3(256), 0, GV_ST, workspace, sx + sy, 1.f, mmd, 0);
    return launch_status("gv_mmd_fwd");
}

extern "C" int gv_loss_combine(const float* ws_pred, int64_t t, const float* ws_reg, int64_t n_embed, int64_t n_wrel,
                               const float* ws_kl, int64_t n_nodes, int h, int k, const float* ws_mmd, int sx, int sy,
                               float reg_w, float kl_w, float mmd_w, float* scal, float* loss, const int32_t* rows_dev,
                               void* stream) {
    GV_REQUIRE(ws_pred && loss, GV_ERR_NULL, "gv_loss_combine: NULL pointer");
    GV_REQUIRE(t > 0, GV_ERR_SHAPE, "gv_loss_combine: t=%lld", (long long)t);
    const int n0 = red_blocks(t, 16);
    const int n1 = ws_reg ? sq2_blocks(n_embed, 768) + sq2_blocks(n_wrel, 255) : 0;
    const int n2 = ws_kl ? kl_blocks(n_nodes) : 0;
    const int n3 = ws_mmd ? sx + sy : 0;
    const float* kl_part = ws_kl ? ws_kl + 3 * (size_t)k * h : nullptr;
    hipLaunchKernelGGL(k_loss_combine, dim3(1), dim3(256), 0, GV_ST, ws_pred, n0, 1.f / (float)t, ws_reg, n1, 1.f, kl_part,
                       n2, ws_kl ? 1.f / (float)n_nodes : 0.f, ws_mmd, n3, 1.f, reg_w, kl_w, mmd_w, scal, loss, rows_dev,
                       (float)n_nodes);
    return launch_status("gv_loss_combine");
}

extern "C" int gv_mmd_bwd(const float* x, const float* y, const int64_t* y_index, int sx, int sy, int h, const float* gmmd,
                          float gscale, float* gx, float* gy, void* stream) {
    GV_REQUIRE(x && y && gx && gy, GV_ERR_NULL, "gv_mmd_bwd: NULL pointer");
    GV_REQUIRE(sx > 0 && sy > 0 && h > 0 && h <= 1024, GV_ERR_SHAPE, "gv_mmd_bwd: bad shape");
    static const int v2 = getenv("GV_MMD_ROWS16") ? atoi(getenv("GV_MMD_ROWS16")) : 1;
    const bool al = h % 4 == 0 && aligned16(x) && aligned16(y) && aligned16(gx) && aligned16(gy);
    if (v2 && al && h <= 256) hipLaunchKernelGGL(k_mmd_bwd_g<4>, dim3(sx + sy), dim3(64 * MMD_WAVES), 0, GV_ST, x, y, y_index, sx, sy, h, gmmd, gscale, gx, gy);
    else if (h <= 256) hipLaunchKernelGGL(k_mmd_bwd<4>, dim3(sx + sy), dim3(64 * MMD_WAVES), 0, GV_ST, x, y, y_index, sx, sy, h, gmmd, gscale, gx, gy);
    else hipLaunchKernelGGL(k_mmd_bwd<16>, dim3(sx + sy), dim3(64 * MMD_WAVES), 0, GV_ST, x, y, y_index, sx, sy, h, gmmd, gscale, gx, gy);
    return launch_status("gv_mmd_bwd");
}

extern "C" int gv_prior_sample_fwd(const float* z_pre, const float* eps, float* out, int s, int k, int h, void* stream) {
    GV_REQUIRE(z_pre && eps && out, GV_ERR_NULL, "gv_prior_sample_fwd: NULL pointer");
    GV_REQUIRE(s > 0 && k > 0 && h > 0, GV_ERR_SHAPE, "gv_prior_sample_fwd: bad shape");
    hipLaunchKernelGGL(k_prior_sample_fwd, dim3((s * h + 255) / 256), dim3(256), 0, GV_ST, z_pre, eps, out, s, k, h);
    return launch_status("gv_prior_sample_fwd");
}

extern "C" int gv_prior_sample_bwd(const float* z_pre, const float* eps, const float* g, float* gz_pre, int accumulate,
                                   int s, int k, int h, void* stream) {
    GV_REQUIRE(z_pre && eps && g && gz_pre, GV_ERR_NULL, "gv_prior_sample_bwd: NULL pointer");
    GV_REQUIRE(s > 0 && k > 0 && h > 0, GV_ERR_SHAPE, "gv_prior_sample_bwd: bad shape");
    hipLaunchKernelGGL(k_prior_sample_bwd, dim3((k * h + 255) / 256), dim3(256), 0, GV_ST, z_pre, eps, g, gz_pre, accumulate, s, k, h);
    return launch_status("gv_prior_sample_bwd");
}
```

### gcn-vae_amd/distributed.py

```python
import os

import numpy as np
import torch
import torch.distributed as dist


def env_world():
    return int(os.environ.get('RANK', 0)), int(os.environ.get('LOCAL_RANK', 0)), int(os.environ.get('WORLD_SIZE', 1))


def collective_timeout():
    import datetime
    return datetime.timedelta(seconds=float(os.environ.get('GV_DIST_TIMEOUT', '300')))


def init_process_group(backend=None):
    rank, local_rank, world = env_world()
    if world > 1 and not dist.is_initialized():
        os.environ.setdefault('MASTER_ADDR', '127.0.0.1')
        os.environ.setdefault('MASTER_PORT', '29500')
        os.environ.setdefault('HSA_ENABLE_IPC_MODE_LEGACY', '0')
        if backend is None:
            backend = 'nccl' if torch.cuda.is_available() else 'gloo'
        if backend == 'nccl':
# ... 29 lines not shown

class AllReduceSum(torch.autograd.Function):

    @staticmethod
    def forward(ctx, x, group):
        ctx.group = group
        y = x.clone()
        if dist.is_initialized():
            start_collective(lambda: dist.all_reduce(y, op=dist.ReduceOp.SUM, group=group, async_op=True)).wait()
        return y

    @staticmethod
    def backward(ctx, g):
        g = g.contiguous().clone()
        if dist.is_initialized():
            start_collective(lambda: dist.all_reduce(g, op=dist.ReduceOp.SUM, group=ctx.group, async_op=True)).wait()
        return g, None


def average_gradients(params, group=None):
    world = dist.get_world_size(group)
    grads = [p.grad for p in params if p.grad is not None]
    if not grads or world == 1:
        return
    flat = torch.cat([g.reshape(-1) for g in grads])
    dist.all_reduce(flat, op=dist.ReduceOp.SUM, group=group)
    flat.div_(world)
    off = 0
    for g in grads:
        n = g.numel()
        g.copy_(flat[off:off + n].view_as(g))
        off += n


def average_flat(flat_grads, group=None):
    world = dist.get_world_size(group)
    if dist.is_initialized():
        start_collective(lambda: dist.all_reduce(flat_grads, op=dist.ReduceOp.SUM, group=group, async_op=True)).wait()
        if world > 1:
            flat_grads.div_(world)


def arena_order(model):
    first = ('encoder.input_layer.', 'encoder.rconv_layer_1.', 'encoder.rconv_layer_2.')
    named = [(k, p) for k, p in model.named_parameters() if p.requires_grad]

    def rank_of(k):
        for i, pre in enumerate(first):
            if k.startswith(pre):
                return i
        return len(first)
    return [p for _, p in sorted(named, key=lambda kp: rank_of(kp[0]))]


class BucketedArenaReduce:

    def __init__(self, flat_grads, offsets, group=None, average=True):
        self.flat, self.offsets, self.group, self.average = flat_grads, dict(offsets), group, average
        self.reset()

    def reset(self):
        self.hi = self.flat.numel()
        self.handles = []
        self.log = []

    def _launch(self, lo):
        if lo >= self.hi or not dist.is_initialized():
            self.hi = min(self.hi, lo)
            return
        piece = self.flat[lo:self.hi]
        self.log.append((lo, self.hi))
        self.hi = lo
        self.handles.append(start_collective(
            lambda: dist.all_reduce(piece, op=dist.ReduceOp.SUM, group=self.group, async_op=True)))

    def milestone(self, activation, first_param):
        if not activation.requires_grad:
            return activation
        lo = self.offsets[first_param]

        def fire(grad):
            self._launch(lo)
            return grad
        activation.register_hook(fire)
        return activation

    def finish(self):
        self._launch(0)
        for h in self.handles:
            h.wait()
        if self.average and dist.is_initialized():
            world = dist.get_world_size(self.group)
            if world > 1:
                self.flat.div_(world)
        self.reset()


def shard_edges_by_relation(etypes, num_rels, world, rank):
    et = np.asarray(etypes)
    counts = np.bincount(et, minlength=num_rels)
    csum = np.cumsum(counts)
    total = csum[-1] if len(csum) else 0
    bounds = [0]
    for p in range(1, world):
        bounds.append(int(np.searchsorted(csum, total * p / world, side='left')) + 1 if total else 0)
    bounds.append(num_rels)
    bounds = np.minimum.accumulate(np.array(bounds[::-1]))[::-1]
    lo, hi = int(bounds[rank]), int(bounds[rank + 1])
    return np.nonzero((et >= lo) & (et < hi))[0], (lo, hi)


def global_in_degree_norm(dst_local, num_nodes, group=None, device=None):
    deg = torch.bincount(torch.as_tensor(dst_local, dtype=torch.int64), minlength=num_nodes).to(torch.float32)
    if device is not None:
        deg = deg.to(device)
    if dist.is_initialized() and dist.get_world_size(group) > 1:
        dist.all_reduce(deg, op=dist.ReduceOp.SUM, group=group)
    norm = torch.zeros_like(deg)
    nz = deg > 0
    norm[nz] = 1.0 / deg[nz]
    return norm


class RowPartition:
    def __init__(self, world, rank, counts, group=None, native=None):
        self.world, self.rank = int(world), int(rank)
        self.counts = [int(c) for c in counts]
        if len(self.counts) != self.world:
            raise ValueError('one row count per rank')
        self.slot_rows = max(max(self.counts), 1)
        self.own_rows = self.counts[self.rank]
        self.row0 = self.rank * self.slot_rows
        self.total_rows = self.world * self.slot_rows
        self.real_rows = sum(self.counts)
        self.group = group
        if native is None:
            native = dist.is_available() and dist.is_initialized() and dist.get_backend(group) == 'nccl'
        self.native = bool(native)
        self.chunks = max(1, int(os.environ.get('GV_DIST_ROW_CHUNKS', '1')))

    def chunk_bounds(self, chunks=None):
        c = max(1, min(int(chunks or self.chunks), self.slot_rows))
        cuts = sorted(set([0] + [(self.slot_rows * k) // c for k in range(1, c)] + [self.slot_rows]))
        return [(cuts[i], cuts[i + 1]) for i in range(len(cuts) - 1)]

    def _views(self, full, a, b):
        return [full[r * self.slot_rows + a:r * self.slot_rows + b] for r in range(self.world)]

    def gather_rows(self, out_full, x_slot, a, b):
        if self.world == 1:
            out_full[a:b].copy_(x_slot[a:b])
            return _Done()
        mine = x_slot[a:b].contiguous()
        if self.native:
            views = self._views(out_full, a, b)
            return start_collective(lambda: dist.all_gather(views, mine, group=self.group, async_op=True))
        tmp = torch.zeros(self.world, b - a, x_slot.shape[1], dtype=x_slot.dtype, device=x_slot.device)
        tmp[self.rank].copy_(mine)
        start_collective(lambda: dist.all_reduce(tmp, op=dist.ReduceOp.SUM, group=self.group, async_op=True)).wait()
        for r, v in enumerate(self._views(out_full, a, b)):
            v.copy_(tmp[r])
        return _Done()

    def reduce_scatter_rows(self, out_slot, g_full, a, b):
        if self.world == 1:
            out_slot[a:b].copy_(g_full[a:b])
# ... 230 lines not shown
```

### gcn-vae_amd/lib.py

```python
import ctypes
import os

import torch

_HERE = os.path.dirname(os.path.abspath(__file__))
LIB_PATH = os.path.join(_HERE, 'libgcnvae_hip.so')

_P, _I, _L, _F = ctypes.c_void_p, ctypes.c_int, ctypes.c_int64, ctypes.c_float

SIGNATURES = {
    'gv_version': (_I, []),
    'gv_last_error_string': (ctypes.c_char_p, []),
    'gv_index_caps': (None, [_L, _I, _I, _P, _P, _P]),
    'gv_index_workspace_bytes': (_L, [_L, _I]),
    'gv_build_csr': (_I, [_P, _L, _I, _I, _P, _P, _P, _I, _P, _I, _P, _L, _P]),
    'gv_build_csr_batch_workspace_bytes': (_L, [_P, _I]),
    'gv_build_csr_batch': (_I, [_P, _I, _P, _L, _P]),
    'gv_triplet_lists': (_I, [_P, _I, _L, _P, _P, _P, _P, _P, _P, _P, _P, _P]),
    'gv_widen2_i32': (_I, [_P, _P, _L, _P, _P, _L, _P]),
    'gv_graph_index_build': (_I, [_P, _P, _L, _I, _I, _I, _I, _P, _P, _P, _P, _I, _P, _I, _P, _P, _P, _P, _I, _P, _I, _P, _L, _P]),
    'gv_relation_index_build': (_I, [_P, _P, _P, _P, _P, _L, _I, _I, _P, _P, _P, _P, _P, _P, _P, _I, _P, _I, _P, _L, _P]),
    'gv_triplet_index_build': (_I, [_P, _L, _I, _I, _I, _I, _P, _P, _P, _P, _P, _I, _P, _I, _P, _P, _P, _P, _P, _I, _P, _I,
                                    _P, _L, _P]),
    'gv_perm_sample': (_I, [_L, _L, ctypes.c_uint64, ctypes.c_uint64, _P, _P, ctypes.c_uint32, _P, _P]),
    'gv_neighborhood_sample_workspace_bytes': (_L, [_I, _L]),
    'gv_neighborhood_sample': (_I, [_P, _P, _P, _P, _I, _L, _I, ctypes.c_uint64, ctypes.c_uint64, _P, ctypes.c_uint32, _P, _P, _L, _P]),
    'gv_relabel_workspace_bytes': (_L, [_I]),
    'gv_relabel_pairs': (_I, [_P, _P, _L, _I, _P, _I, _P, _P, _P, _P, _L, _P]),
    'gv_negative_sampling': (_I, [_P, _P, _P, _L, _I, _P, _P, _P, ctypes.c_uint64, ctypes.c_uint64, _P, ctypes.c_uint32, _P, _P, _P]),
    'gv_graph_from_triplets_workspace_bytes': (_L, [_L, _I, _I]),
    'gv_graph_from_triplets': (_I, [_P, _P, _P, _P, _L, _I, _I, _P, _P, _P, _P, _P, _L, _P]),
    'gv_segment_items_count': (_I, [_P, _I, _I, _P, _P, _P, _P]),
    'gv_segment_items_fill': (_I, [_P, _I, _I, _P, _P, _P, _P, _P, _P]),
    'gv_rgcn_bdd_aggregate': (_I, [_P, _I, _P, _I, _P, _P, _P, _P, _P, _I, _P, _I, _I, _I, _I, _I, _I,
                                   _P, _I, _I, _P, _F, _P, _I, _P, _P]),
    'gv_rgcn_bdd_phase_plan': (_I, [_I, _I, _I, _I, _I, _I, _I, _I, _I, _P]),
    'gv_rgcn_bdd_pack_weight_phase': (_I, [_P, _I, _I, _I, _I, _I, _P, _P]),
    'gv_rgcn_bdd_aggregate_phases': (_I, [_P, _P, _P, _P, _P, _I, _P, _I, _P, _I, _P, _I, _I, _I, _I, _I, _I, _I, _I, _I,
                                          _P, _I, _I, _P, _F, _P, _I, _P, _P]),
    'gv_rgcn_bdd_lds_plan': (_I, [_I, _I, _I, _I, _I, _P]),
    'gv_rgcn_bdd_pack_weight_lds': (_I, [_P, _I, _I, _I, _I, _I, _I, _P, _P]),
    'gv_rgcn_bdd_aggregate_lds': (_I, [_P, _I, _P, _P, _I, _P, _I, _P, _P, _P, _P, _P, _I, _P, _I, _I, _I, _I, _I, _P, _I, _I,
                                       _P, _F, _P, _I, _P, _I, _P]),
    'gv_rgcn_bdd_pack_supported': (_I, [_I, _I, _I, _I]),
    'gv_rgcn_bdd_pack_weight': (_I, [_P, _I, _I, _I, _I, _I, _P, _P]),
    'gv_rgcn_bdd_pack_weight_pair': (_I, [_P, _I, _I, _I, _I, _P, _P, _P]),
    'gv_rgcn_bdd_fixup': (_I, [_P, _I, _P, _I, _P, _I, _I, _P, _F, _P, _I, _P]),
    'gv_rgcn_bdd_grad_weight': (_I, [_P, _I, _P, _I, _P, _P, _P, _P, _P, _I, _P, _I, _I, _I, _I, _P, _P, _I, _P]),
    'gv_rgcn_epilogue_fwd': (_I, [_P, _P, _I, _P, _F, _P, _L, _I, _P]),
    'gv_rgcn_epilogue_bwd': (_I, [_P, _P, _I, _P, _F, _P, _L, _I, _P, _P]),
    'gv_colsum_finish': (_I, [_P, _I, _I, _P, _I, _P]),
    'gv_gemm_workspace_bytes': (_L, [_I, _I, _I, _I]),
    'gv_gemm_f32': (_I, [_I, _I, _I, _I, _I, _P, _I, _P, _I, _P, _I, _P, _I, _I, _I, _P, _P, _L, _P]),
    'gv_gemm_f32_live_rows': (_I, [_I, _I, _I, _I, _I, _P, _I, _P, _I, _P, _I, _P, _I, _I, _I, _P, _P, _L, _P, _P]),
    'gv_gemm_f32_sparse': (_I, [_I, _I, _I, _I, _I, _P, _I, _P, _I, _P, _I, _P, _I, _I, _I, _P, _P, _L, _P, _P, _P, _I, _P]),
    'gv_gemm_bf16': (_I, [_I, _I, _I, _I, _I, _P, _I, _P, _I, _P, _I, _P, _I, _I, _I, _P, _P, _L, _P]),
    'gv_gemm_bf16_nt_workspace_bytes': (_L, [_I, _I, _I]),
    'gv_gemm_bf16_gradw_fits': (_I, [_I, _I, _I, _I]),
    'gv_gemm_bf16_gradw_workspace_bytes': (_L, [_I, _I, _I]),
    'gv_gemm_bf16_gradw': (_I, [_P, _I, _P, _I, _I, _I, _I, _P, _I, _P, _I, _P, _L, _P]),
    'gv_gemm_bf16_gradw_tiles': (_I, [_P, _L, _P, _L, _I, _I, _I, _P, _I, _P, _I, _P, _L, _P]),
    'gv_gemm_bf16_nt': (_I, [_P, _I, _I, _P, _I, _I, _I, _I, _P, _I, _P, _I, _P, _I, _I, _P, _I, _P, _I, _I, _P, _L, _P]),
    'gv_cast_bf16': (_I, [_P, _I, _I, _I, _P, _I, _P, _I, _P]),
    'gv_rowsum_bf16_workspace_floats': (_L, [_I, _I]),
    'gv_iaf_update_fwd_bf16': (_I, [_P, _P, _I, _P, _P, _P, _P, _I, _P, _I, _L, _I, _P]),
    'gv_iaf_update_fwd_bf16_tiles': (_I, [_P, _P, _I, _P, _P, _P, _P, _I, _P, _L, _L, _I, _P]),
    'gv_iaf_update_bwd_bf16': (_I, [_P, _P, _I, _P, _P, _P, _P, _P, _I, _P, _I, _P, _L, _I, _P]),
    'gv_gather3_i32': (_I, [_P, _L, _P, _P, _P, _P, _P, _P, _P]),
    'gv_iaf_update_bwd_row0_workspace_floats': (_L, [_I]),
    'gv_iaf_update_bwd_row0': (_I, [_P, _P, _P, _P, _P, _P, _P, _P, _L, _I, _P]),
    'gv_iaf_update_bwd_bf16_ex': (_I, [_P, _P, _I, _P, _P, _P, _P, _P, _I, _P, _I, _P, _I, _L, _I, _P]),
    'gv_rowsum_bf16': (_I, [_P, _I, _I, _I, _P, _I, _P, _P]),
    'gv_rowsum_bf16_segments': (_I, [_P, _I, _I, _I, _I, _P, _P, _I, _P, _P]),
    'gv_made_pack_weight_elems': (_L, [_I, _I]),
    'gv_made_pack_weight': (_I, [_P, _I, _I, _I, _P, _P, _P]),
    'gv_made_pack_weight_multi': (_I, [_I, _P, _P, _P, _P, _P, _P, _P]),
    'gv_made_pack_weight_multi_iaf': (_I, [_I, _P, _P, _P, _P, _P, _P, _P]),
    'gv_made_pack_weight_iaf': (_I, [_P, _I, _I, _I, _P, _P]),
    'gv_made_chain_fits': (_I, [_I, _P, _P, _I]),
    'gv_made_chain': (_I, [_P, _I, _I, _I, _P, _P]),
    'gv_made_chain_iafb': (_I, [_P, _I, _I, _P, _P]),
    'gv_made_chain_fwd': (_I, [_P, _I, _I, _I, _P, _I, _P, _P]),
    'gv_made_chain_fwd_row0': (_I, [_P, _I, _I, _P, _I, _P, _P]),
    'gv_made_chain_debug_stamps': (_I, [_P]),
    'gv_made_pack_weight_f32_elems': (_L, [_I, _I]),
    'gv_made_pack_weight_f32_multi': (_I, [_I, _P, _P, _P, _P, _P, _P, _P]),
    'gv_made_chain_f32_fits': (_I, [_I, _P, _P]),
    'gv_made_chain_f32_plan': (_I, [_I, _P, _P, _P, _P, _P, _P, _P]),
    'gv_made_chain_f32': (_I, [_P, _I, _I, _I, _P, _P, _P, _P]),
    'gv_made_passes_f32': (_I, [_P, _I, _I, _I, _P, _P, _P, _P, _P]),
    'gv_made_gradw_f32_plan_words': (_L, [_I, _I]),
    'gv_made_gradw_f32_plan': (_I, [_P, _I, _I, _I, _P, _P]),
    'gv_made_gradw_f32_workspace_floats': (_L, [_I, _I, _L]),
    'gv_made_gradw_f32': (_I, [_P, _I, _P, _I, _I, _I, _L, _P, _P, _I, _P, _P, _P, _P, _I, _I, _P, _I, _P, _L, _P]),
    'gv_made_gradw_f32_multi_workspace_floats': (_L, [_I, _P]),
    'gv_made_gradw_f32_multi': (_I, [_I, _P, _P, _L, _P]),
    'gv_made_row_fwd': (_I, [_P, _I, _P, _P]),
    'gv_made_row_bwd': (_I, [_P, _I, _P, _P, _P]),
    'gv_rel_rows_gemm': (_I, [_P, _I, _P, _P, _I, _I, _I, _I, _P, _I, _P, _P]),
    'gv_rel_gradw_gemm': (_I, [_P, _I, _P, _P, _I, _P, _P, _P, _I, _I, _I, _P, _P]),
    'gv_rank_scores': (_I, [_P, _I, _P, _I, _P, _P, _P, _P, _I, _I, _I, _P]),
    'gv_rank_scores_filtered': (_I, [_P, _I, _P, _I, _P, _P, _P, _P, _P, _I, _P, _P, _P, _I, _I, _I, _P]),
    'gv_topk_scores_workspace_bytes': (_L, [_I, _I, _I]),
    'gv_topk_scores': (_I, [_P, _I, _P, _I, _P, _P, _P, _P, _I, _I, _P, _P, _P, _I, _I, _I, _P]),
    'gv_ec_basis_rows_fwd': (_I, [_P, _P, _P, _P, _L, _I, _I, _I, _L, _P, _P]),
    'gv_ec_basis_rows_bwd': (_I, [_P, _P, _P, _P, _P, _P, _L, _P, _P, _L, _I, _I, _I, _L, _P, _P, _P, _I, _P]),
    'gv_ec_head_fwd': (_I, [_P, _P, _P, _P, _L, _I, _P, _P, _P, _P, _P, _P]),
    'gv_ec_head_bwd': (_I, [_P, _P, _P, _P, _P, _P, _L, _I, _P, _P]),
    'gv_transe_sample': (_I, [_P, ctypes.c_uint32, _P, _L, _I, _P, _P, _P, _P, _P, _I, _I, _P, _P, _P, _P, _P]),
    'gv_transe_step': (_I, [_P, _P, _P, _P, _P, _I, _I, _I, _I, _I, _F, _F, _F, _P, _P, _P, _P, _P, _P]),
    'gv_transe_apply': (_I, [_P, _I, _P, _P, _P, _P, _I, _P, _P, _P, _I, _F, _P, _I, _F, _P, _P, _P]),
    'gv_transe_queries': (_I, [_P, _P, _P, _P, _L, _I, _I, _I, _P, _P]),
    'gv_transe_distances': (_I, [_P, _L, _P, _I, _I, _I, _P, _P]),
    'gv_transe_rank_filtered': (_I, [_P, _L, _P, _I, _I, _I, _P, _P, _P, _P, _P, _P, _P]),
    'gv_colsum': (_I, [_P, _P, _L, _I, _I, _P, _P, _I, _P]),
    'gv_gather_rows': (_I, [_P, _P, _P, _L, _I, _P]),
    'gv_gather_rows_rng_tick': (_I, [_P, _P, _P, _L, _I, _P, _P]),
    'gv_rng_fill': (_I, [_P, _I, _P, _P, _P, _P, _P, _P]),
    'gv_rng_tick': (_I, [_P, _P]),
    'gv_scatter_add_rows': (_I, [_P, _P, _P, _L, _I, _P]),
    'gv_reparam_fwd': (_I, [_P, _P, _P, _P, _P, _L, _I, _P]),
    'gv_reparam_bwd': (_I, [_P, _P, _P, _P, _P, _P, _P, _L, _I, _P]),
    'gv_distmult_bce_fwd': (_I, [_P, _I, _P, _I, _P, _P, _P, _P, _P, _P, _P, _L, _I, _P]),
    'gv_bce_grad': (_I, [_P, _P, _P, _P, _P, _P, _P, _P, _P, _L, _P]),
    'gv_mean_sq': (_I, [_P, _L, _F, _P, _P, _I, _P]),
    'gv_mean_sq2': (_I, [_P, _L, _F, _P, _L, _F, _P, _P, _P, _L, _P]),
    'gv_axpby': (_I, [_L, _P, _F, _P, _F, _P, _P]),
    'gv_mul': (_I, [_L, _P, _P, _P, _P]),
    'gv_mul_multi': (_I, [_I, _P, _P, _P, _P, _P]),
    'gv_kl_workspace_bytes': (_L, [_L, _I, _I]),
    'gv_kl_fwd': (_I, [_P, _P, _I, _P, _P, _P, _P, _P, _P, _L, _I, _I, _P, _P]),
    'gv_kl_bwd': (_I, [_P, _P, _I, _P, _P, _P, _P, _F, _F, _P, _P, _P, _P, _I, _P, _I, _L, _I, _I, _P, _P]),
    'gv_reparam_kl_fwd': (_I, [_P, _P, _P, _P, _P, _P, _P, _P, _L, _I, _I, _P]),
    'gv_reparam_kl_bwd': (_I, [_P, _P, _P, _P, _P, _P, _P, _F, _F, _P, _P, _P, _I, _P, _L, _I, _I, _P]),
# ... 82 lines not shown
```

### gcn-vae_amd/ops.py

```python
import contextlib
import ctypes as _ct
import itertools as _it
import os as _os
from dataclasses import dataclass
from typing import Optional

import torch

from . import lib
from .lib import ptr

ACT_NONE, ACT_RELU = 0, 1

DIRECT_GRAD = {}
GRAD_FRESH = set()
DIRECT_EPOCH = [0]


def _stamp_direct(ctx):
    ctx._gv_direct_epoch = DIRECT_EPOCH[0]


def _verify_direct(ctx):
    if getattr(ctx, '_gv_direct_epoch', DIRECT_EPOCH[0]) != DIRECT_EPOCH[0]:
        raise RuntimeError('the optimiser gradient arena (ops.DIRECT_GRAD) changed between this forward and its backward: '
                           'build / drop FlatAdam outside a forward-backward pair')


def _direct(t):
    tgt = DIRECT_GRAD.get(t.data_ptr()) if t is not None else None
    return tgt if (tgt is not None and tgt.shape == t.shape) else None


def _direct_flat(t):
    tgt = DIRECT_GRAD.get(t.data_ptr()) if t is not None else None
    return tgt.view(t.shape) if (tgt is not None and tgt.numel() == t.numel() and tgt.is_contiguous()) else None
EPILOGUE_COLSUM_SLICES = 1024
DEFAULT_CHUNK = 256
DEFAULT_CHUNK_REL = 128


CHUNK_DIV = int(_os.environ.get('GV_CHUNK_DIV', '4096'))


def chunk_for(n_entries: int, most: int = DEFAULT_CHUNK) -> int:
    env = _os.environ.get('GV_CHUNK')
    if env:
        return max(1, int(env))
    div = CHUNK_DIV // 4 if most == DEFAULT_CHUNK_REL else CHUNK_DIV
    c = 16
    while c * 2 <= most and c * 2 * div <= int(n_entries):
        c *= 2
    return c
DIST_FWD_CHUNKS = 2


CONCURRENCY = _os.environ.get('GV_CONCURRENCY', '0') == '1'
_side_streams = {}


def _side(i):
    key = (torch.cuda.current_device(), i)
    if key not in _side_streams:
        _side_streams[key] = torch.cuda.Stream()
    return _side_streams[key]


@contextlib.contextmanager
def fork(i):
    if not CONCURRENCY:
        yield
        return
    s = _side(i)
    s.wait_stream(torch.cuda.current_stream())
    with torch.cuda.stream(s):
        yield


def join(*ids):
    if CONCURRENCY:
        cur = torch.cuda.current_stream()
        for i in ids:
            cur.wait_stream(_side(i))


BWD_SIDE = _os.environ.get('GV_BWD_SIDE', '1') == '1'
_bwd_side_held = []
RGCN_BWD_SIDE = _os.environ.get('GV_RGCN_BWD_SIDE', 'auto')
RGCN_BWD_SIDE_MIN_WORK = 10 ** 8


_bwd_side_others = [False]


def rgcn_bwd_side(num_edges, width):
    layout = launch_layout()
    if not layout.bwd_side or layout.process_group:
        return False
    if RGCN_BWD_SIDE == 'auto':
        return not _bwd_side_others[0] and num_edges * width >= RGCN_BWD_SIDE_MIN_WORK
    return RGCN_BWD_SIDE == '1'


@dataclass(frozen=True)
class LaunchLayout:
    timed: bool
    process_group: bool
    bwd_side: bool
    bwd_side_join_at_collective: bool
    made_prepare: bool
    row_blocks: bool


def launch_layout():
    from . import made as _made
    timed, pg = lib.TIMER is not None, _process_group()
    return LaunchLayout(
        timed=timed, process_group=pg,
        bwd_side=BWD_SIDE and not timed, bwd_side_join_at_collective=pg,
        made_prepare=_made.MADE_PREPARE and not timed and not pg,
        row_blocks=not timed)


def _process_group():
    import torch.distributed as dist
    return dist.is_available() and dist.is_initialized()


@contextlib.contextmanager
def backward_side(enabled, *held, rgcn=False):
    if not (enabled and launch_layout().bwd_side):
        if _bwd_side_held:
            torch.cuda.current_stream().wait_stream(_side('bwd'))
        yield False
        return
    side, main = _side('bwd'), torch.cuda.current_stream()
    side.wait_stream(main)
    with torch.cuda.stream(side):
        yield True
    first = not _bwd_side_held
    _bwd_side_held.append(held)
    if not rgcn:
        _bwd_side_others[0] = True
    if first:
        def _join():
            if not _bwd_side_held:
                return
            main.wait_stream(side)
            cur = torch.cuda.current_stream()
            if cur != main:
                cur.wait_stream(side)
            _bwd_side_held.clear()
            _bwd_side_others[0] = False
        torch.autograd.Variable._execution_engine.queue_callback(_join)


def backward_side_finish():
    if _bwd_side_held:
        torch.cuda.current_stream().wait_stream(_side('bwd'))
        _bwd_side_held.clear()
    _bwd_side_others[0] = False


class StayOnDevice:
    _gv_warned = False

    def _apply(self, fn, *args, **kwargs):
        dev = next((t.device for t in list(self.parameters()) + list(self.buffers()) if t.is_cuda), None)
        if dev is not None:
            try:
                moved = fn(torch.zeros(1, device=dev))
            except Exception:
                moved = None
            if moved is not None and moved.device.type == 'cpu':
                if not StayOnDevice._gv_warned:
                    StayOnDevice._gv_warned = True
                    import sys
                    print('[gcn_vae_amd] .cpu() on a HIP module is a no-op: parameters stay on %s, inputs are copied to them'
                          % dev, file=sys.stderr)
                return self
        return super()._apply(fn, *args, **kwargs)


def to_module_device(param, *tensors):
    dev = param.device
    out = tuple(t if (t is None or not isinstance(t, torch.Tensor) or t.device == dev) else t.to(dev) for t in tensors)
    return out if len(out) != 1 else out[0]


def _chk(t, dtype=torch.float32, name='tensor'):
    if not isinstance(t, torch.Tensor) or not t.is_cuda:
        raise RuntimeError(f'{name}: the gfx950 path needs a CUDA/ROCm tensor (got '
                           f'{type(t).__name__} on {getattr(t, "device", "?")}); there is no CPU fallback')
    if t.dtype != dtype:
        raise TypeError(f'{name}: expected {dtype}, got {t.dtype}')
    if not t.is_contiguous():
        raise ValueError(f'{name}: must be contiguous')
    return t


def _row_major(t, name='matrix'):
    if not isinstance(t, torch.Tensor) or not t.is_cuda:
        raise RuntimeError(f'{name}: the gfx950 path needs a CUDA/ROCm tensor; there is no CPU fallback')
    if t.dtype != torch.float32 or t.dim() != 2:
        raise TypeError(f'{name}: expected 2-D float32, got {t.dtype} {tuple(t.shape)}')
    if t.stride(1) != 1 or (t.shape[0] > 1 and t.stride(0) < t.shape[1]):
        t = t.contiguous()
    return t, (t.stride(0) if t.shape[0] > 1 else t.shape[1])


from .indices import *
from .indices import _carve_i32, _index_caps, _index_workspace, _rowptr_from_sorted
from . import indices
from . import batch_index
from .batch_index import build_batch_indices


RGCN_SIDE_GRADW_FIRST = _os.environ.get('GV_RGCN_SIDE_GRADW_FIRST', 'auto')


def rgcn_side_gradw_first(num_edges, width):
    if RGCN_SIDE_GRADW_FIRST in ('0', '1'):
        return RGCN_SIDE_GRADW_FIRST == '1'
    return num_edges <= 4_000_000 and width <= 256


def _k1_items(gidx, seg):
    if indices.K1_ITEMS_LARGEST_FIRST and not gidx.sync_free:
        return indices.largest_first(seg)
    return seg


def pack_supported(num_bases, blk_in, blk_out, transpose_w=False):
    return bool(lib.load().gv_rgcn_bdd_pack_supported(num_bases, blk_in, blk_out, 1 if transpose_w else 0))


def pack_weight(weight, num_bases, blk_in, blk_out, transpose_w=False):
    weight = _chk(weight, name='weight')
    packed = torch.empty_like(weight)
    lib.call('gv_rgcn_bdd_pack_weight', ptr(weight), weight.shape[0], num_bases, blk_in, blk_out,
             1 if transpose_w else 0, ptr(packed), lib.stream())
    return packed


def _check_items(seg: SegmentItems):
    if seg.n_items < 0 or seg.n_fix < 0 or seg.items.numel() < 4 * seg.n_items or seg.fix.numel() < 4 * seg.n_fix:
        raise ValueError(f'inconsistent work-item lists: n_items={seg.n_items} (buffer {seg.items.numel() // 4}), '
                         f'n_fix={seg.n_fix} (buffer {seg.fix.numel() // 4})')
    if seg.n_items > 0 and seg.items.data_ptr() == 0:
        raise ValueError('work-item list has no storage')


def bdd_aggregate(seg: SegmentItems, nbr, etype, coef, coef_idx, feat, weight, num_bases, blk_in, blk_out,
                  transpose_w=False, addend=None, act=ACT_NONE, keep=None, keep_scale=1.0, out=None, packed=False):
    feat, ld_feat = _row_major(feat, 'feat')
    weight = _chk(weight, name='weight')
    n_seg = seg.rowptr.numel() - 1
    out_dim = num_bases * blk_out
    if feat.shape[1] != num_bases * blk_in:
        raise ValueError(f'feat has {feat.shape[1]} columns, expected num_bases*blk_in = {num_bases * blk_in}')
    num_rels = weight.shape[0]
    if weight.numel() != num_rels * num_bases * blk_in * blk_out:
        raise ValueError('weight shape does not match (R, num_bases*blk_in*blk_out)')
    if out is None:
        out = torch.empty(n_seg, out_dim, dtype=torch.float32, device=feat.device)
    ld_add = 0
    if addend is not None:
        addend, ld_add = _row_major(addend, 'addend')
        if tuple(addend.shape) != (n_seg, out_dim):
            raise ValueError('addend shape mismatch')
    if keep is not None:
        _chk(keep, torch.uint8, 'keep')
        if tuple(keep.shape) != (n_seg, out_dim):
            raise ValueError('keep shape mismatch')
    if coef is not None:
        coef = _chk(coef.reshape(-1), name='coef')
    _check_items(seg)
    partial = None
    if seg.n_fix > 0:
        partial = torch.empty(seg.n_slots, out_dim, dtype=torch.float32, device=feat.device)
    ld_out = out.stride(0) if n_seg > 1 else out_dim
    tag = f'agg_{"T" if transpose_w else "N"}_{blk_in}x{blk_out}_nb{num_bases}'
    timed = lib.TIMER is not None
    lib.call('gv_rgcn_bdd_aggregate', ptr(seg.items), seg.n_items, ptr(seg.fix), 0 if timed else seg.n_fix, ptr(nbr),
             ptr(etype), ptr(coef), ptr(coef_idx), ptr(feat), ld_feat, ptr(weight), num_rels, num_bases, blk_in,
             blk_out, 1 if transpose_w else 0, 1 if packed else 0, ptr(addend), ld_add, act, ptr(keep),
             float(keep_scale), ptr(out), ld_out, ptr(partial), lib.stream(), tag=tag)
    if timed and seg.n_fix > 0:
        lib.call('gv_rgcn_bdd_fixup', ptr(seg.fix), seg.n_fix, ptr(partial), out_dim, ptr(addend), ld_add, act,
                 ptr(keep), float(keep_scale), ptr(out), ld_out, lib.stream())
    return out


def bdd_grad_weight(seg: SegmentItems, src, dst, coef, coef_idx, x, g, num_bases, blk_in, blk_out, out=None,
                    accumulate=False):
    x, ld_x = _row_major(x, 'x')
    g, ld_g = _row_major(g, 'g')
    n_seg = seg.rowptr.numel() - 1
    w_row = num_bases * blk_in * blk_out
    if out is None:
        out = torch.empty(n_seg, w_row, dtype=torch.float32, device=x.device)
        accumulate = False
    if coef is not None:
        coef = _chk(coef.reshape(-1), name='coef')
    partial = None
    if seg.n_fix > 0:
        partial = torch.empty(seg.n_slots, w_row, dtype=torch.float32, device=x.device)
    lib.call('gv_rgcn_bdd_grad_weight', ptr(seg.items), seg.n_items, ptr(seg.fix), seg.n_fix, ptr(src), ptr(dst),
             ptr(coef), ptr(coef_idx), ptr(x), ld_x, ptr(g), ld_g, num_bases, blk_in, blk_out, ptr(out), ptr(partial),
             1 if accumulate else 0, lib.stream(), tag=f'gradw_{blk_in}x{blk_out}_nb{num_bases}')
    return out


GEMM_PRECISION = 'f32'


def set_gemm_precision(precision):
    global GEMM_PRECISION
    if precision not in ('f32', 'bf16'):
        raise ValueError("precision must be 'f32' or 'bf16'")
    GEMM_PRECISION = precision


@contextlib.contextmanager
def gemm_precision(precision):
    old = GEMM_PRECISION
    set_gemm_precision(precision)
    try:
        yield
    finally:
        set_gemm_precision(old)


LIVE_ROWS = None


class live_rows:

    def __init__(self, rows_dev, cap):
        self.val = (rows_dev, int(cap)) if rows_dev is not None else None

    def __enter__(self):
        global LIVE_ROWS
        self.saved, LIVE_ROWS = LIVE_ROWS, self.val
        return self

    def __exit__(self, *exc):
        global LIVE_ROWS
        LIVE_ROWS = self.saved
        return False


def gemm(a, b, trans_a=False, trans_b=False, bias=None, act=ACT_NONE, out=None, accumulate=False, split_k=1,
         a_relu_mask=None, precision=None, b_k_chunks=None, c_tiles=None):
    a, lda = _row_major(a, 'a')
    b, ldb = _row_major(b, 'b')
    m, k = (a.shape[1], a.shape[0]) if trans_a else a.shape
    kb, n = (b.shape[1], b.shape[0]) if trans_b else b.shape
    if k != kb:
        raise ValueError(f'gemm inner dimensions differ: {k} vs {kb}')
    if out is None:
        out = torch.empty(m, n, dtype=torch.float32, device=a.device)
        accumulate = False
    else:
        if not isinstance(out, torch.Tensor) or out.dtype != torch.float32 or out.dim() != 2:
            raise TypeError(f'out: expected a 2-D float32 tensor, got {getattr(out, "dtype", type(out).__name__)} '
                            f'{tuple(getattr(out, "shape", ()))}')
        if out.device != a.device or b.device != a.device:
            raise ValueError(f'out / b must be on the device of a ({a.device}), got {out.device} / {b.device}')
        if tuple(out.shape) != (m, n):
            raise ValueError(f'out: expected shape {(m, n)}, got {tuple(out.shape)}')
        if m * n and ((n > 1 and out.stride(1) != 1) or (m > 1 and out.stride(0) < n)):
            raise ValueError(f'out: needs unit inner stride and a leading dimension >= {n}, got strides {out.stride()}')
    if bias is not None:
        _chk(bias, name='bias')
        if bias.numel() != n or bias.device != a.device:
            raise ValueError(f'bias: expected {n} values on {a.device}, got {bias.numel()} on {bias.device}')
    ws, ws_bytes = None, 0
    if split_k > 1:
        ws_bytes = int(lib.load().gv_gemm_workspace_bytes(m, n, k, split_k))
        ws = torch.empty(ws_bytes // 4, dtype=torch.float32, device=a.device)
    if a_relu_mask is not None:
        a_relu_mask, ld_mask = _row_major(a_relu_mask, 'a_relu_mask')
        if tuple(a_relu_mask.shape) != tuple(a.shape) or ld_mask != lda:
            raise ValueError('a_relu_mask must have the shape and leading dimension of a')
    entry = 'gv_gemm_bf16' if (precision or GEMM_PRECISION) == 'bf16' else 'gv_gemm_f32'
    live = LIVE_ROWS
    if (b_k_chunks is not None or c_tiles is not None) and entry == 'gv_gemm_f32':
        if b_k_chunks is not None and (b_k_chunks.dtype != torch.int64 or b_k_chunks.numel() < (n + 63) // 64 or k > 1024 or split_k != 1):
            raise ValueError('b_k_chunks: one int64 word per 64-column tile, k <= 1024, no split-K')
        if c_tiles is not None and (c_tiles.dtype != torch.int64 or c_tiles.numel() * 64 < ((m + 63) // 64) * ((n + 63) // 64)):
            raise ValueError('c_tiles: one bit per 64 x 64 tile of the result')
        rows = live[0] if (live is not None and a.shape[0] == live[1] and a.device == live[0].device) else None
        lib.call('gv_gemm_f32_sparse', 1 if trans_a else 0, 1 if trans_b else 0, m, n, k, ptr(a), lda, ptr(b), ldb, ptr(out),
                 out.stride(0) if m > 1 else n, ptr(bias), act, 1 if accumulate else 0, split_k, ptr(a_relu_mask), ptr(ws),
                 ws_bytes, ptr(rows), ptr(b_k_chunks), ptr(c_tiles), int(getattr(c_tiles, '_gv_wanted', 0)) if c_tiles is not None else 0,
                 lib.stream())
        return out
    if live is not None and entry == 'gv_gemm_f32' and a.shape[0] == live[1] and a.device == live[0].device:
        lib.call('gv_gemm_f32_live_rows', 1 if trans_a else 0, 1 if trans_b else 0, m, n, k, ptr(a), lda, ptr(b), ldb, ptr(out),
                 out.stride(0) if m > 1 else n, ptr(bias), act, 1 if accumulate else 0, split_k, ptr(a_relu_mask), ptr(ws),
                 ws_bytes, ptr(live[0]), lib.stream())
        return out
    lib.call(entry, 1 if trans_a else 0, 1 if trans_b else 0, m, n, k, ptr(a), lda, ptr(b), ldb, ptr(out),
             out.stride(0) if m > 1 else n, ptr(bias), act, 1 if accumulate else 0, split_k, ptr(a_relu_mask), ptr(ws),
             ws_bytes, lib.stream())
    return out


def block_words(mask, kind):
    import numpy as np
    m = (mask.detach().to('cpu').numpy() != 0)
    o, i = m.shape

    def pad(x, r, c):
        y = np.zeros((-(-x.shape[0] // r) * r, -(-x.shape[1] // c) * c), dtype=bool)
        y[:x.shape[0], :x.shape[1]] = x
        return y
    if kind in ('fwd', 'bwd'):
        mm = m if kind == 'fwd' else m.T
        if mm.shape[1] > 1024:
            return None
        y = pad(mm, 64, 16)
        blk = y.reshape(y.shape[0] // 64, 64, y.shape[1] // 16, 16).any(axis=(1, 3))
        words = np.zeros(blk.shape[0], dtype=np.uint64)
        for c in range(blk.shape[1]):
            words |= blk[:, c].astype(np.uint64) << np.uint64(c)
    elif kind == 'tiles':
        y = pad(m, 64, 64)
        blk = y.reshape(y.shape[0] // 64, 64, y.shape[1] // 64, 64).any(axis=(1, 3)).reshape(-1)
        words = np.zeros((blk.size + 63) // 64, dtype=np.uint64)
        for b in np.nonzero(blk)[0]:
            words[b >> 6] |= np.uint64(1) << np.uint64(b & 63)
    else:
        raise ValueError(kind)
    out = torch.from_numpy(words.view(np.int64).copy()).to(mask.device)
    if kind == 'tiles':
        out._gv_wanted = int(blk.sum())
    return out


def rank_scores(q, entities, target, bias=None):
    q, ld_q = _row_major(q, 'q')
    entities, ld_e = _row_major(entities, 'entities')
    if q.shape[1] != entities.shape[1]:
        raise ValueError('q / entities width mismatch')
    m, v = q.shape[0], entities.shape[0]
    target = target.reshape(-1)
    if target.numel() != m:
        raise ValueError('one target per query row')
    if m and (int(target.min()) < 0 or int(target.max()) >= v):
        raise ValueError(f'targets must lie in [0, {v})')
    tgt32 = target.to(device=q.device, dtype=torch.int32).contiguous()
    if bias is not None:
        bias = _chk(bias.reshape(1).to(torch.float32).contiguous(), name='bias')
    ws = torch.empty(max(m, 1), dtype=torch.float32, device=q.device)
    count = torch.empty(max(m, 1), dtype=torch.int32, device=q.device)
    lib.call('gv_rank_scores', ptr(q), ld_q, ptr(entities), ld_e, ptr(tgt32), ptr(bias), ptr(ws), ptr(count), m, v,
             q.shape[1], lib.stream())
    return count[:m].to(torch.float32) * 0.5


def rank_scores_filtered(q, entities, target, filt_lo, filt_hi, filt_ent, bias=None):
    q, ld_q = _row_major(q, 'q')
    entities, ld_e = _row_major(entities, 'entities')
    if q.shape[1] != entities.shape[1]:
        raise ValueError('q / entities width mismatch')
    m, v = q.shape[0], entities.shape[0]
    target = target.reshape(-1)
    if target.numel() != m:
        raise ValueError('one target per query row')
    filt_lo, filt_hi, filt_ent = filt_lo.reshape(-1), filt_hi.reshape(-1), filt_ent.reshape(-1)
    if filt_lo.numel() != m or filt_hi.numel() != m:
        raise ValueError('one filter range (filt_lo, filt_hi) per query row')
    n_ent = filt_ent.numel()
    if n_ent >= 2 ** 31:
        raise ValueError('filt_ent: more than 2**31 - 1 entries')
    if m and (int(target.min()) < 0 or int(target.max()) >= v):
        raise ValueError(f'targets must lie in [0, {v})')
    if m and (int(filt_lo.min()) < 0 or int(filt_hi.max()) > n_ent or bool((filt_hi < filt_lo).any())):
        raise ValueError(f'filter ranges must satisfy 0 <= filt_lo <= filt_hi <= {n_ent}')
    if n_ent and (int(filt_ent.min()) < 0 or int(filt_ent.max()) >= v):
        raise ValueError(f'filtered entity ids must lie in [0, {v})')
    i32 = dict(device=q.device, dtype=torch.int32)
    tgt32 = target.to(**i32).contiguous()
    lo32, hi32 = filt_lo.to(**i32).contiguous(), filt_hi.to(**i32).contiguous()
    ent32 = filt_ent.to(**i32).contiguous() if n_ent else torch.zeros(1, **i32)
    if bias is not None:
        bias = _chk(bias.reshape(1).to(torch.float32).contiguous(), name='bias')
# ... 8 lines not shown
TOPK_MAX = 128


def topk_scores(q, entities, k, bias=None, filt_lo=None, filt_hi=None, filt_ent=None):
    for name, t in (('q', q), ('entities', entities)):
        if not isinstance(t, torch.Tensor) or t.dim() != 2:
            raise TypeError(f'{name}: expected a 2-D tensor')
    if q.shape[1] != entities.shape[1]:
        raise ValueError('q / entities width mismatch')
    m, v, h = q.shape[0], entities.shape[0], q.shape[1]
    if v < 1 or h < 1:
        raise ValueError(f'need at least one entity and width >= 1 (v={v}, h={h})')
    k = int(k)
    if not 1 <= k <= TOPK_MAX:
        raise ValueError(f'k must lie in [1, {TOPK_MAX}], got {k}')
    given = [t is not None for t in (filt_lo, filt_hi, filt_ent)]
    if any(given) and not all(given):
        raise ValueError('filt_lo, filt_hi and filt_ent are given together or not at all')
    n_ent = 0
    if all(given):
        filt_lo, filt_hi, filt_ent = filt_lo.reshape(-1), filt_hi.reshape(-1), filt_ent.reshape(-1)
        if filt_lo.numel() != m or filt_hi.numel() != m:
            raise ValueError('one filter range (filt_lo, filt_hi) per query row')
        n_ent = filt_ent.numel()
        if n_ent >= 2 ** 31:
            raise ValueError('filt_ent: more than 2**31 - 1 entries')
        if m and (int(filt_lo.min()) < 0 or int(filt_hi.max()) > n_ent or bool((filt_hi < filt_lo).any())):
            raise ValueError(f'filter ranges must satisfy 0 <= filt_lo <= filt_hi <= {n_ent}')
        if n_ent and (int(filt_ent.min()) < 0 or int(filt_ent.max()) >= v):
            raise ValueError(f'filtered entity ids must lie in [0, {v})')
    q, ld_q = _row_major(q, 'q')
    entities, ld_e = _row_major(entities, 'entities')
    ids = torch.empty(m, k, dtype=torch.int32, device=q.device)
    logits = torch.empty(m, k, dtype=torch.float32, device=q.device)
    if m == 0:
        return ids.long(), logits
    lo32 = hi32 = ent32 = None
    if all(given):
        i32 = dict(device=q.device, dtype=torch.int32)
        lo32, hi32 = filt_lo.to(**i32).contiguous(), filt_hi.to(**i32).contiguous()
        ent32 = filt_ent.to(**i32).contiguous() if n_ent else torch.zeros(1, **i32)
    if bias is not None:
        bias = _chk(bias.reshape(1).to(torch.float32).contiguous(), name='bias')
    ws = torch.empty(int(lib.load().gv_topk_scores_workspace_bytes(m, v, k)), dtype=torch.uint8, device=q.device)
    lib.call('gv_topk_scores', ptr(q), ld_q, ptr(entities), ld_e, ptr(bias), ptr(lo32), ptr(hi32), ptr(ent32), n_ent, k,
             ptr(ids), ptr(logits), ptr(ws), m, v, h, lib.stream())
    return ids.long(), logits


def pick_split_k(m_out, n_out, k):
    tiles = ((m_out + 63) // 64) * ((n_out + 63) // 64)
    if tiles >= 256 or k < 2048:
        return 1
    if k >= 65536:
        return 64
    return max(1, min(64, 1024 // tiles, k // 256))


def colsum(x, out=None, accumulate=False, relu_mask=None):
    x, ld = _row_major(x, 'x')
    if relu_mask is not None:
        relu_mask, ldm = _row_major(relu_mask, 'relu_mask')
        if tuple(relu_mask.shape) != tuple(x.shape) or ldm != ld:
            raise ValueError('relu_mask must have the shape and leading dimension of x')
    m, n = x.shape
    if out is None:
        out = torch.empty(n, dtype=torch.float32, device=x.device)
        accumulate = False
    ws = torch.empty(64 * n, dtype=torch.float32, device=x.device)
    lib.call('gv_colsum', ptr(x), ptr(relu_mask), m, n, ld, ptr(out), ptr(ws), 1 if accumulate else 0, lib.stream())
    return out


def epilogue_fwd(agg, addend, act, keep, keep_scale):
    agg = _chk(agg, name='agg')
    out = torch.empty_like(agg)
    if addend is not None:
        addend = _chk(addend, name='addend')
    lib.call('gv_rgcn_epilogue_fwd', ptr(agg), ptr(addend), act, ptr(keep), float(keep_scale), ptr(out),
             agg.shape[0], agg.shape[1], lib.stream())
    return out


def epilogue_bwd(out, grad_out, act, keep, keep_scale, colsum_out=None, colsum_accumulate=False):
    grad_out = _chk(grad_out.contiguous(), name='grad_out')
    g = torch.empty_like(grad_out)
    m, n = grad_out.shape
    fused = colsum_out is not None and n % 4 == 0 and n <= 1024
    part = torch.empty(EPILOGUE_COLSUM_SLICES * n, dtype=torch.float32, device=g.device) if fused else None
    lib.call('gv_rgcn_epilogue_bwd', ptr(out), ptr(grad_out), act, ptr(keep), float(keep_scale), ptr(g), m, n, ptr(part),
             lib.stream())
    if fused:
        lib.call('gv_colsum_finish', ptr(part), n, EPILOGUE_COLSUM_SLICES, ptr(colsum_out), 1 if colsum_accumulate else 0,
                 lib.stream())
    elif colsum_out is not None:
        colsum(g, out=colsum_out, accumulate=colsum_accumulate)
    return g


def axpby(alpha, x, beta=0.0, y=None, a=None):
    x = _chk(x.contiguous(), name='x')
    if y is None:
        y = torch.empty_like(x)
        beta = 0.0
    lib.call('gv_axpby', x.numel(), ptr(a), float(alpha), ptr(x), float(beta), ptr(y), lib.stream())
    return y


def copy_into(dst, src):
    src = _chk(src.contiguous(), name='src')
    if dst.numel() != src.numel() or not dst.is_contiguous():
        raise ValueError('copy_into: same size, contiguous destination')
    lib.call('gv_axpby', src.numel(), None, 1.0, ptr(src), 0.0, ptr(dst), lib.stream())
    return dst


def copy_of(x):
    return copy_into(torch.empty_like(x, memory_format=torch.contiguous_format), x)


class _CatRows(torch.autograd.Function):

    @staticmethod
    def forward(ctx, a, b):
        out = torch.empty(a.shape[0] + b.shape[0], a.shape[1], dtype=torch.float32, device=a.device)
        copy_into(out[:a.shape[0]], a)
        copy_into(out[a.shape[0]:], b)
        ctx.na = a.shape[0]
        return out

    @staticmethod
    def backward(ctx, g):
        return g[:ctx.na], g[ctx.na:]


def cat_rows(a, b):
    return _CatRows.apply(a, b)


class _SplitRows(torch.autograd.Function):

    @staticmethod
    def forward(ctx, x, n):
        ctx.n, ctx.shape = int(n), tuple(x.shape)
        ctx.set_materialize_grads(False)
        return x[:n], x[n:]

    @staticmethod
    def backward(ctx, ga, gb):
        if ga is None and gb is None:
            return None, None
        ref = ga if ga is not None else gb
        out = torch.empty(ctx.shape, dtype=ref.dtype, device=ref.device)
        for part, g in ((out[:ctx.n], ga), (out[ctx.n:], gb)):
            if part.numel() == 0:
                continue
            if g is None:
                part.zero_()
            else:
                copy_into(part, g)
        return out, None


def split_rows(x, n):
    return _SplitRows.apply(x, n)


def mul(a, b):
    a, b = _chk(a.contiguous(), name='a'), _chk(b.contiguous(), name='b')
    out = torch.empty_like(a)
    lib.call('gv_mul', a.numel(), ptr(a), ptr(b), ptr(out), lib.stream())
    return out


def mul_multi(as_, bs, outs=None):
# ... 83 lines not shown
        if tick_rng is not None and ids.numel() > 0:
            lib.call('gv_gather_rows_rng_tick', ptr(table), ptr(ids), ptr(out), ids.numel(), table.shape[1],
                     ptr(tick_rng.folded_tick()), lib.stream())
        else:
            lib.call('gv_gather_rows', ptr(table), ptr(ids), ptr(out), ids.numel(), table.shape[1], lib.stream())
        ctx.save_for_backward(ids)
        ctx.shape = tuple(table.shape)
        ctx.direct = _direct(table)
        _stamp_direct(ctx)
        return out

    @staticmethod
    def backward(ctx, g):
        (ids,) = ctx.saved_tensors
        g = _chk(g.contiguous(), name='grad')
        _verify_direct(ctx)
        tgt = ctx.direct
        gt = tgt if tgt is not None else torch.zeros(ctx.shape, dtype=torch.float32, device=g.device)
        lib.call('gv_scatter_add_rows', ptr(g), ptr(ids), ptr(gt), ids.numel(), ctx.shape[1], lib.stream())
        if tgt is not None:
            GRAD_FRESH.discard(tgt.data_ptr())
        return (None if tgt is not None else gt), None, None


class _EmbeddingIdentity(torch.autograd.Function):

    @staticmethod
    def forward(ctx, table, tick_rng):
        ctx.set_materialize_grads(False)
        if tick_rng is not None:
            tick_rng.tick()
        ctx.direct = _direct(table)
        _stamp_direct(ctx)
        return table.detach().view(table.shape)

    @staticmethod
    def backward(ctx, g):
        if g is None:
            return None, None
        g = _chk(g.contiguous(), name='grad')
        _verify_direct(ctx)
        tgt = ctx.direct
        if tgt is None:
            return g, None
        lib.call('gv_axpby', g.numel(), None, 1.0, ptr(g), 1.0, ptr(tgt), lib.stream())
        GRAD_FRESH.discard(tgt.data_ptr())
        return None, None


_identity_ids = {}


def _ids_are_identity(table, ids):
    if ids.numel() != table.shape[0]:
        return False
    key = (ids.data_ptr(), ids._version, ids.numel())
    hit = _identity_ids.get(key)
    if hit is None:
        if len(_identity_ids) > 64:
            _identity_ids.clear()
        hit = _identity_ids[key] = (bool((ids.reshape(-1) == torch.arange(ids.numel(), device=ids.device)).all()), ids)
    return hit[0]


def embedding(table, ids, tick_rng=None, sole_consumer=False):
    identity = False
    if table.is_cuda and isinstance(ids, torch.Tensor) and ids.is_cuda and ids.dtype == torch.int64:
        if torch.cuda.is_current_stream_capturing():
            hit = _identity_ids.get((ids.data_ptr(), ids._version, ids.numel()))
            identity = bool(hit and hit[0]) and ids.numel() == table.shape[0]
        else:
            identity = _ids_are_identity(table, ids)
    if identity and sole_consumer:
        out = _EmbeddingIdentity.apply(table, tick_rng)
        out._gv_grad_target = _direct(table)
        return out
    return _Embedding.apply(table, ids, tick_rng)


def _epilogue_grad(out, grad_out, act, keep, keep_scale, want_bias, d_b):
    if not want_bias:
        return epilogue_bwd(out, grad_out, act, keep, keep_scale), None
    grad_bias = d_b if d_b is not None else torch.empty(grad_out.shape[1], dtype=torch.float32, device=grad_out.device)
    g = epilogue_bwd(out, grad_out, act, keep, keep_scale, colsum_out=grad_bias, colsum_accumulate=d_b is not None)
    return g, (None if d_b is not None else grad_bias)


def _gemm_addend(x, loop_weight, h_bias, out_feat, loop_bf=None):
    if loop_weight is not None and loop_bf is not None:
        return dense_bf16(x, loop_bf[0], loop_weight.shape[1], loop_weight.shape[0], bias=h_bias)
    if loop_weight is not None:
        return gemm(x, loop_weight, bias=h_bias)
    if h_bias is not None:
        return h_bias.unsqueeze(0).expand(x.shape[0], out_feat).contiguous()
    return None


def _row_addend(h_bias, loop_rows, n, out_feat):
    if h_bias is None:
        return loop_rows
    addend = h_bias.unsqueeze(0).expand(n, out_feat).contiguous()
    if loop_rows is not None:
        lib.call('gv_axpby', addend.numel(), None, 1.0, ptr(loop_rows), 1.0, ptr(addend), lib.stream())
    return addend


def _loop_grads(x, g, loop_weight, d_l, want_loop, want_x, loop_bf=None):
    if loop_weight is None:
        return None, None
    grad_loop = gx_loop = None
    if want_loop:
        grad_loop = gemm(x, g, trans_a=True, split_k=pick_split_k(x.shape[1], g.shape[1], x.shape[0]), out=d_l,
                         accumulate=d_l is not None)
        if d_l is not None:
            grad_loop = None
    if want_x:
        if loop_bf is not None:
            gx_loop = dense_bf16(g, loop_bf[1], loop_weight.shape[0], loop_weight.shape[1])
        else:
            gx_loop = gemm(g, loop_weight, trans_b=True)
    return grad_loop, gx_loop


def _coef_order(gidx, ridx, coef, side):
    if gidx.sync_free or coef is None:
        return coef, (gidx.by_src.perm if side == 'src' else ridx.by_rel.perm)
    return (gidx.coef_in_src_order(coef) if side == 'src' else ridx.coef_in_rel_order(coef)), None


def _relation_weight_grad(gidx, ridx, coef, x, g, nb, si, so, d_w):
    coef_r, idx_r = _coef_order(gidx, ridx, coef, 'rel')
    grad_w = bdd_grad_weight(ridx.by_rel.seg, ridx.src_by_rel, ridx.dst_by_rel, coef_r, idx_r, x, g, nb, si, so, out=d_w,
                             accumulate=d_w is not None)
    return None if d_w is not None else grad_w


def _bdd_weight_fwd(ctx, weight, nb, si, so, pk, pk_bwd):
    ctx.w_bwd_packed = None
    ctx.w_version = weight._version
    if pk and pk_bwd:
        w_fwd, ctx.w_bwd_packed = torch.empty_like(weight), torch.empty_like(weight)
        lib.call('gv_rgcn_bdd_pack_weight_pair', ptr(weight), weight.shape[0], nb, si, so, ptr(w_fwd), ptr(ctx.w_bwd_packed),
                 lib.stream())
        return w_fwd
    return pack_weight(weight, nb, si, so, False) if pk else weight


def _bdd_weight_bwd(ctx, weight, nb, so, si):
    pk = si * so >= 8 and pack_supported(nb, so, si, True)
    if ctx.w_bwd_packed is not None and weight._version == ctx.w_version:
        return ctx.w_bwd_packed, pk
    return (pack_weight(weight, nb, so, si, True) if pk else weight), pk


def _bdd_k1(ctx, side, tl, gidx, ridx, coef, feat, weight, nb, bi, bo, plain_weight, addend, act=ACT_NONE, keep=None,
            keep_scale=1.0, out=None, sharded=False):
    trans, r = side == 'src', weight.shape[0]
    if tl is not None:
        return bdd_aggregate_phases(tl, None if coef is None else tl.coef(coef), feat, pack_weight_phase(tl, weight, nb, bi, bo),
                                    r, nb, bi, bo, addend(), act, keep, keep_scale, out=out)
    seg = gidx.by_src.seg if trans else gidx.by_dst.seg
    nbr, ety = (gidx.nbr_by_src, ridx.et_by_src) if trans else (gidx.nbr_by_dst, ridx.et_by_dst)

    def coef_operands():
        return _coef_order(gidx, ridx, coef, 'src') if trans else (coef, gidx.by_dst.perm)
    lp = None if (ctx.grouped or sharded) else lds_plan(r, nb, bi, bo, bf=ctx.k1_bf if trans else None)
    if lp is not None and lds_graph(gidx, side, lp[2]):
        if not trans:
            ctx.k1_bf = bool(lp[3])
            if not torch.cuda.is_current_stream_capturing():
                lp_b = lds_plan(r, nb, bo, bi, bf=ctx.k1_bf)
                if lp_b is not None:
                    gidx.lds_order('src', lp_b[2])
        c, c_idx = coef_operands()
        return bdd_aggregate_lds(gidx.lds_order(side, lp[2]), nbr, ety, c, c_idx, feat,
                                 pack_weight_lds(weight, nb, bi, bo, trans, lp), r, nb, bi, bo, trans, addend(), act, keep,
                                 keep_scale, out=out, plan=lp)
    w, pk = plain_weight()
    if ctx.grouped:
        seg_g, nbr_g, ety_g, perm = ridx.grouped_order(gidx, side)
        coef_g = None if coef is None else ridx.grouped_coef(coef, side, perm)
        return bdd_aggregate(seg_g, nbr_g, ety_g, coef_g, None, feat, w, nb, bi, bo, trans, addend(), act, keep, keep_scale,
                             out=out, packed=pk)
    if K1_REL_RUNS and not gidx.sync_free and not sharded:
        nbr_r, et_r, _, coef_r = ridx.rel_sorted(gidx, side, coef)
        return bdd_aggregate(_k1_items(gidx, seg), nbr_r, et_r, coef_r, None, feat, w, nb, bi, bo, trans, addend(), act, keep,
                             keep_scale, out=out, packed=pk)
    c, c_idx = coef_operands()
    return bdd_aggregate(_k1_items(gidx, seg), nbr, ety, c, c_idx, feat, w, nb, bi, bo, trans, addend(), act, keep, keep_scale,
                         out=out, packed=pk)


class _RelGraphConvBdd(torch.autograd.Function):

    @staticmethod
    def forward(ctx, x, weight, h_bias, loop_weight, norm, gidx, ridx, num_bases, act, keep, keep_scale,
                reduce_hook):
        x, _ = _row_major(x, 'x')
        n, in_feat = x.shape
        si = in_feat // num_bases
        so = weight.shape[1] // (num_bases * si)
        out_feat = num_bases * so
        coef = None if norm is None else norm.reshape(-1)
        tl = None
        if reduce_hook is None and use_phases(gidx, si, so, False, x.shape[0], in_feat):
            tl = ridx.phase_order(gidx, 'dst', num_bases, si, so)
        pk = tl is None and si * so >= 8 and pack_supported(num_bases, si, so, False)
        bwd_phases = reduce_hook is None and use_phases(gidx, so, si, True, n, out_feat)
        pk_bwd = not bwd_phases and si * so >= 8 and pack_supported(num_bases, so, si, True)
        w_fwd = _bdd_weight_fwd(ctx, weight, num_bases, si, so, pk, pk_bwd and ctx.needs_input_grad[0])
        ctx.loop_bf = dense_bf16_forms(loop_weight) if (loop_weight is not None and x.shape[0] >= 4096) else None

        def addend():
            return _gemm_addend(x, loop_weight, h_bias, out_feat, ctx.loop_bf)

        ctx.grouped = tl is None and reduce_hook is None and use_relation_groups(weight, gidx)
# ... 666 lines not shown
def linear(x, w, b=None, act=ACT_NONE):
    return _Linear.apply(x, w, b, act)


class _Mul(torch.autograd.Function):

    @staticmethod
    def forward(ctx, mask, w):
        ctx.save_for_backward(mask)
        ctx.direct = _direct(w)
        _stamp_direct(ctx)
        return mul(mask, w)

    @staticmethod
    def backward(ctx, g):
        (mask,) = ctx.saved_tensors
        _verify_direct(ctx)
        tgt = ctx.direct
        if tgt is not None and tgt.data_ptr() in GRAD_FRESH and tgt.is_contiguous():
            g = _chk(g.contiguous(), name='grad')
            lib.call('gv_mul', g.numel(), ptr(mask), ptr(g), ptr(tgt), lib.stream())
            GRAD_FRESH.discard(tgt.data_ptr())
            return None, None
        return None, mul(mask, g)


def masked_weight(mask, w):
    return _Mul.apply(mask, w)


class KLLink:
    __slots__ = ('resp', 'ws', 'z_pre_ptr', 'z_pre_version', 'gkl', 'gscale', 'z_extra', 'claimed')

    def __init__(self, resp, ws, z_pre):
        self.resp, self.ws = resp, ws
        self.z_pre_ptr, self.z_pre_version = z_pre.data_ptr(), z_pre._version
        self.gkl = None
        self.gscale = self.z_extra = 0.0
        self.claimed = False

    def matches(self, z_pre):
        return z_pre is not None and z_pre.data_ptr() == self.z_pre_ptr and z_pre._version == self.z_pre_version


FUSE_REPARAM_KL = _os.environ.get('GV_FUSE_REPARAM_KL', '1') == '1'


class _Reparam(torch.autograd.Function):

    @staticmethod
    def forward(ctx, h2, eps, z_pre, link_box):
        ctx.set_materialize_grads(False)
        h2 = _chk(h2.contiguous(), name='h2')
        n, h = h2.shape[0], h2.shape[1] // 2
        eps = _chk(eps.contiguous(), name='eps')
        z = torch.empty(n, h, dtype=torch.float32, device=h2.device)
        v = torch.empty_like(z)
        m = torch.empty_like(z)
        ctx.link = None
        if z_pre is not None:
            z_pre = _chk(z_pre.contiguous(), name='z_pre')
            k = z_pre.shape[0] // 2
            ws = torch.empty(int(lib.load().gv_kl_workspace_bytes(n, h, k)) // 4, dtype=torch.float32, device=h2.device)
            resp = torch.empty(n, k, dtype=torch.float32, device=h2.device)
            lib.call('gv_reparam_kl_fwd', ptr(h2), ptr(eps), ptr(z_pre), ptr(z), ptr(v), ptr(m), ptr(resp), ptr(ws), n, h, k,
                     lib.stream())
            ctx.link = link_box[0] = KLLink(resp, ws, z_pre)
            ctx.save_for_backward(h2, eps, v, z, z_pre)
        else:
            lib.call('gv_reparam_fwd', ptr(h2), ptr(eps), ptr(z), ptr(v), ptr(m), n, h, lib.stream())
            ctx.save_for_backward(h2, eps, v)
        return z, m, v

    @staticmethod
    def backward(ctx, gz, gm, gv):
        link = ctx.link
        if link is not None and link.gkl is not None:
            h2, eps, v, z, z_pre = ctx.saved_tensors
            n, h = v.shape
            gz = None if gz is None else _chk(gz.contiguous(), name='gz')
            d_zp = _direct_flat(z_pre)
            gzp = d_zp if d_zp is not None else torch.empty_like(z_pre)
            gh2 = torch.empty_like(h2)
            lib.call('gv_reparam_kl_bwd', ptr(z), ptr(h2), ptr(v), ptr(eps), ptr(z_pre), ptr(link.resp), ptr(link.gkl),
                     float(link.gscale), float(link.z_extra), ptr(gz), ptr(gh2), ptr(gzp), 1 if d_zp is not None else 0,
                     ptr(link.ws), n, h, z_pre.shape[0] // 2, lib.stream())
            link.gkl = None
            if gm is not None or gv is not None:
                extra = torch.empty_like(h2)
                gm = None if gm is None else _chk(gm.contiguous(), name='gm')
                gv = None if gv is None else _chk(gv.contiguous(), name='gv')
                lib.call('gv_reparam_bwd', ptr(h2), ptr(eps), ptr(v), None, ptr(gm), ptr(gv), ptr(extra), n, h, lib.stream())
                gh2 += extra
            return gh2, None, (None if d_zp is not None else gzp), None
        h2, eps, v = ctx.saved_tensors[:3]
        n, h = v.shape
        gz = None if gz is None else _chk(gz.contiguous(), name='gz')
        gm = None if gm is None else _chk(gm.contiguous(), name='gm')
        gv = None if gv is None else _chk(gv.contiguous(), name='gv')
        gh2 = torch.empty_like(h2)
        lib.call('gv_reparam_bwd', ptr(h2), ptr(eps), ptr(v), ptr(gz), ptr(gm), ptr(gv), ptr(gh2), n, h, lib.stream())
        return gh2, None, None, None


def reparam(h2, eps, z_pre=None):
    if z_pre is None or not FUSE_REPARAM_KL:
        return _Reparam.apply(h2, eps, None, None)
    box = [None]
    z, m, v = _Reparam.apply(h2, eps, z_pre, box)
    z._gv_kl_link = box[0]
    return z, m, v


class _DistMultBCE(torch.autograd.Function):

    @staticmethod
    def forward(ctx, embed, w_rel, bias, labels, tidx):
        ctx.set_materialize_grads(False)
        embed, ld_e = _row_major(embed, 'embed')
        w_rel, ld_w = _row_major(w_rel, 'w_relation')
        labels = _chk(labels.reshape(-1), name='labels')
        T, h = tidx.T, embed.shape[1]
        if labels.numel() != T:
            raise ValueError('labels / triplets length mismatch')
        score = torch.empty(T, dtype=torch.float32, device=embed.device)
        loss = torch.empty((), dtype=torch.float32, device=embed.device)
        ws = torch.empty(1024, dtype=torch.float32, device=embed.device)
        lib.call('gv_distmult_bce_fwd', ptr(embed), ld_e, ptr(w_rel), ld_w, ptr(tidx.trip32), ptr(tidx.fwd_order),
                 ptr(labels), ptr(bias), ptr(score), ptr(loss), ptr(ws), T, h, lib.stream())
        ctx.save_for_backward(embed, w_rel, labels, score)
        ctx.tidx, ctx.has_bias = tidx, bias is not None
        ctx.mark_non_differentiable(score)
        return loss, score

    @staticmethod
    def backward(ctx, gloss, _gscore):
        if gloss is None:
            return None, None, None, None, None
        embed, w_rel, labels, score = ctx.saved_tensors
        tidx = ctx.tidx
        T, h = tidx.T, embed.shape[1]
        dev = embed.device
        gloss = _chk(gloss.reshape(1).contiguous(), name='gloss')
        dscore = torch.empty(T, dtype=torch.float32, device=dev)
        dbias = torch.empty((), dtype=torch.float32, device=dev) if ctx.has_bias else None
        ws = torch.empty(1024, dtype=torch.float32, device=dev)
        lib.call('gv_bce_grad', ptr(score), ptr(labels), ptr(gloss), ptr(dscore), None, None, None, ptr(dbias), ptr(ws), T,
                 lib.stream())
        g_embed = g_w = None
        if ctx.needs_input_grad[0]:
            g_embed = bdd_aggregate(tidx.inc, tidx.inc_other, tidx.inc_rel, dscore, tidx.inc_tid, embed, w_rel,
                                    h, 1, 1)
        if ctx.needs_input_grad[1]:
            g_w = bdd_grad_weight(tidx.rel, tidx.rel_s, tidx.rel_o, dscore, tidx.rel_tid, embed, embed, h, 1, 1)
        return g_embed, g_w, dbias, None, None


def distmult_bce(embed, w_rel, bias, labels, tidx):
    return _DistMultBCE.apply(embed, w_rel, bias, labels, tidx)


class _DistMultScore(torch.autograd.Function):

    @staticmethod
    def forward(ctx, embed, w_rel, tidx):
        embed, ld_e = _row_major(embed, 'embed')
        w_rel, ld_w = _row_major(w_rel, 'w_relation')
        T, h = tidx.T, embed.shape[1]
        score = torch.empty(T, dtype=torch.float32, device=embed.device)
# ... 637 lines not shown
```

### include/gcnvae.h

```cpp
#ifndef GCNVAE_H
#define GCNVAE_H

#include <stdint.h>

#ifdef __cplusplus
extern "C" {
#endif

typedef enum {
    GV_OK = 0,
    GV_ERR_NULL = -1,
    GV_ERR_SHAPE = -2,
    GV_ERR_ALIGN = -3,
    GV_ERR_WORKSPACE = -4
} gv_status;

enum { GV_ACT_NONE = 0, GV_ACT_RELU = 1 };

int gv_version(void);
const char* gv_last_error_string(void);

int gv_segment_items_count(const int32_t* rowptr, int n_seg, int chunk, int32_t* n_chunks, int32_t* n_slots,
                           int32_t* is_split, void* stream);
int gv_segment_items_fill(const int32_t* rowptr, int n_seg, int chunk, const int32_t* item_off,
                          const int32_t* slot_off, const int32_t* fix_off, int32_t* items ,
                          int32_t* fix , void* stream);

int gv_rgcn_bdd_aggregate(const int32_t* items, int n_items, const int32_t* fix, int n_fix,
                          const int32_t* nbr, const int32_t* etype, const float* coef, const int32_t* coef_idx,
                          const float* feat, int ld_feat, const float* weight, int num_rels, int num_bases,
                          int blk_in, int blk_out, int transpose_w, int weight_packed,
                          const float* addend, int ld_addend, int act, const uint8_t* keep, float keep_scale,
                          float* out, int ld_out, float* partial, void* stream);

int gv_rgcn_bdd_pack_supported(int num_bases, int blk_in, int blk_out, int transpose_w);
int gv_rgcn_bdd_pack_weight(const float* weight, int num_rels, int num_bases, int blk_in, int blk_out, int transpose_w,
                            float* packed, void* stream);
int gv_rgcn_bdd_pack_weight_pair(const float* weight, int num_rels, int num_bases, int blk_in, int blk_out, float* packed_fwd,
                                 float* packed_bwd, void* stream);

int gv_rgcn_bdd_phase_plan(int num_bases, int blk_in, int blk_out, int transpose_w, int num_rels, int lds_bytes,
                           int num_buffers, int rows_per_wave, int block_threads, int32_t* plan_host);
int gv_rgcn_bdd_pack_weight_phase(const float* weight, int num_rels, int num_bases, int blk_in, int blk_out, int transpose_w,
                                  float* packed, void* stream);
int gv_rgcn_bdd_aggregate_phases(const int32_t* off, const int32_t* nbr, const int32_t* meta, const float* coef,
                                 const int32_t* tile_items, int n_tiles, const int32_t* fix, int n_fix, const float* feat,
                                 int ld_feat, const float* weight_packed, int num_rels, int num_bases, int blk_in,
                                 int blk_out, int transpose_w, int rows_per_wave, int rels_per_phase, int num_buffers,
                                 int block_threads, const float* addend, int ld_addend, int act, const uint8_t* keep,
                                 float keep_scale, float* out, int ld_out, float* partial, void* stream);

int gv_rgcn_bdd_lds_plan(int num_bases, int blk_in, int blk_out, int num_rels, int bf16_operands, int32_t* plan_host);
int gv_rgcn_bdd_pack_weight_lds(const float* weight, int num_rels, int num_bases, int blk_in, int blk_out, int transpose_w,
                                int bf16_operands, float* packed, void* stream);
int gv_rgcn_bdd_aggregate_lds(const int32_t* sitems, int n_sitems, const int32_t* erow, const int32_t* empty_rows, int n_empty,
                              const int32_t* fix, int n_fix, const int32_t* nbr, const int32_t* etype, const float* coef,
                              const int32_t* coef_idx, const float* feat, int ld_feat, const float* weight_packed,
                              int num_rels, int num_bases, int blk_in, int blk_out, int bf16_operands, const float* addend,
                              int ld_addend, int act, const uint8_t* keep, float keep_scale, float* out, int ld_out,
                              float* partial, int max_workgroups, void* stream);

int gv_rgcn_bdd_fixup(const int32_t* fix, int n_fix, const float* partial, int out_dim, const float* addend,
                      int ld_addend, int act, const uint8_t* keep, float keep_scale, float* out, int ld_out,
                      void* stream);

int gv_rgcn_bdd_grad_weight(const int32_t* items, int n_items, const int32_t* fix, int n_fix,
                            const int32_t* src, const int32_t* dst, const float* coef, const int32_t* coef_idx,
                            const float* x, int ld_x, const float* g, int ld_g, int num_bases, int blk_in,
                            int blk_out, float* grad_w, float* partial, int accumulate, void* stream);

int gv_rgcn_epilogue_fwd(const float* agg, const float* addend, int act, const uint8_t* keep, float keep_scale,
                         float* out, int64_t n_rows, int n_cols, void* stream);
int gv_rgcn_epilogue_bwd(const float* out, const float* grad_out, int act, const uint8_t* keep, float keep_scale,
                         float* g, int64_t n_rows, int n_cols,
                         float* colsum_part , void* stream);
#define GV_EPILOGUE_COLSUM_SLICES 1024
int gv_colsum_finish(const float* part, int n, int n_slices, float* out, int accumulate, void* stream);
int gv_rel_rows_gemm(const float* feat, int ld_feat, const int32_t* rows, const float* w, int num_rels, int in_feat,
                     int out_feat, int transpose_w, const int32_t* tiles, int n_tiles, float* msg, void* stream);
int gv_rel_gradw_gemm(const float* x, int ld_x, const int32_t* x_rows, const float* g, int ld_g, const int32_t* g_rows,
                      const float* scale, const int32_t* relptr, int num_rels, int in_feat, int out_feat, float* grad_w,
                      void* stream);
int gv_iaf_update_fwd_bf16(const float* z, const float* net, int ld_net, const float* x_old, const int32_t* colcount, float* x_new,
                           uint16_t* x_b, int ldb, uint16_t* x_t, int ldt, int64_t n, int d, void* stream);
int gv_iaf_update_fwd_bf16_tiles(const float* z, const float* net, int ld_net, const float* x_old, const int32_t* colcount,
                                 float* x_new, uint16_t* x_b, int ldb, uint16_t* x_t, int64_t t_tile, int64_t n, int d, void* stream);
int gv_iaf_update_bwd_bf16(const float* z, const float* net, int ld_net, const int32_t* colcount, const float* gx, const float* gld,
                           float* gz_accumulate, uint16_t* gnet_b, int ldb, uint16_t* gnet_t, int ldt, float* gx_old, int64_t n,
                           int d, void* stream);
int gv_iaf_update_bwd_bf16_ex(const float* z, const float* ex, int ld_ex, const int32_t* colcount, const float* gx, const float* gld,
                              float* gz_accumulate, uint16_t* gnet_b, int ldb, uint16_t* gnet_t, int ldt, float* gx_old,
                              int flags, int64_t n, int d, void* stream);
int64_t gv_iaf_update_bwd_row0_workspace_floats(int d);
int gv_iaf_update_bwd_row0(const float* z, const float* net_row, const int32_t* colcount, const float* gx, const float* gld,
                           float* gz_accumulate, float* g_row, float* workspace, int64_t n, int d, void* stream);
int64_t gv_gemm_bf16_nt_workspace_bytes(int m, int n, int split_k);
int gv_gemm_bf16_nt(const void* a, int a_is_f32, int lda, const uint16_t* b, int ldb, int m, int n, int k, const float* bias,
                    int relu, const uint16_t* mask, int ldmask, float* c_f32, int ldc, int accumulate, uint16_t* c_bf16,
                    int ldcb, uint16_t* c_bf16_t, int ldct, int split_k, void* workspace, int64_t workspace_bytes,
                    void* stream);
// ... 248 lines not shown
int gv_prior_sample_bwd(const float* z_pre, const float* eps, const float* g, float* gz_pre, int accumulate, int s, int k,
                        int h, void* stream);

int gv_iaf_update_fwd(const float* z, const float* net, int ld_net, const float* x_old, const int32_t* colcount,
                      float* x_new, int64_t n, int d, void* stream);
int gv_iaf_update_bwd(const float* z, const float* net, int ld_net, const int32_t* colcount, const float* g_xnew,
                      const float* g_logdet , float* g_z, float* g_net, float* g_xold, int64_t n, int d,
                      void* stream);
int gv_iaf_update_bwd_acc(const float* z, const float* net, int ld_net, const int32_t* colcount, const float* g_xnew,
                          const float* g_logdet, float* g_z, int gz_accumulate, float* g_net, float* g_xold, int64_t n, int d,
                          void* stream);
int gv_rowsum(const float* x, int ld, int col0, int ncols, float* out, int64_t n, void* stream);
int gv_reverse_cols(const float* x, float* out, int64_t n, int d, void* stream);
int gv_mean_rows_multi(int count, const float* const* x, int64_t n, const int32_t* rows_dev, float* out, float* workspace,
                       void* stream);
int gv_mean_rows_bwd(const float* g, int64_t len, int64_t n, const int32_t* rows_dev, float* out, void* stream);

int gv_adam_step(float* p, const float* g, float* exp_avg, float* exp_avg_sq, int64_t n, const float* sumsq,
                 float max_norm, float lr, float beta1, float beta2, float eps, const float* step, void* stream);
int gv_clip_adam_step(float* p, float* g, float* exp_avg, float* exp_avg_sq, int64_t n, float* workspace,
                      float* sumsq_out, float max_norm, float lr, float beta1, float beta2, float eps, float* step,
                      int zero_grad, void* stream);

void gv_index_caps(int64_t n_entries, int n_seg, int chunk, int* items_cap, int* fix_cap, int* slots_cap);
int64_t gv_index_workspace_bytes(int64_t n_entries, int n_seg_max);
int gv_build_csr(const int32_t* keys, int64_t n, int n_seg, int chunk, int32_t* perm, int32_t* rowptr, int32_t* items,
                 int items_cap, int32_t* fix, int fix_cap, void* workspace, int64_t workspace_bytes, void* stream);
int gv_graph_index_build(const int32_t* src, const int32_t* dst, int64_t n_edges, int n_dst, int n_src, int dst_sorted,
                         int chunk, int32_t* perm_d, int32_t* nbr_by_dst, int32_t* rowptr_d, int32_t* items_d,
                         int items_d_cap, int32_t* fix_d, int fix_d_cap, int32_t* perm_s, int32_t* nbr_by_src,
                         int32_t* rowptr_s, int32_t* items_s, int items_s_cap, int32_t* fix_s, int fix_s_cap,
                         void* workspace, int64_t workspace_bytes, void* stream);
int gv_relation_index_build(const int32_t* src, const int32_t* dst, const int32_t* etype, const int32_t* perm_d ,
                            const int32_t* perm_s, int64_t n_edges, int n_rel, int chunk, int32_t* et_by_dst,
                            int32_t* et_by_src, int32_t* perm_r, int32_t* src_by_rel, int32_t* dst_by_rel, int32_t* rowptr_r,
                            int32_t* items_r, int items_cap, int32_t* fix_r, int fix_cap, void* workspace,
                            int64_t workspace_bytes, void* stream);
int gv_triplet_index_build(const int32_t* trip, int64_t T, int n_ent, int n_rel, int chunk, int chunk_rel, int32_t* inc_other,
                           int32_t* inc_rel, int32_t* inc_tid, int32_t* rowptr_inc, int32_t* items_inc, int items_inc_cap,
                           int32_t* fix_inc, int fix_inc_cap, int32_t* rel_s, int32_t* rel_o, int32_t* rel_tid,
                           int32_t* rowptr_rel, int32_t* items_rel, int items_rel_cap, int32_t* fix_rel, int fix_rel_cap,
                           void* workspace, int64_t workspace_bytes, void* stream);

typedef struct gv_csr_job {
    const int32_t* keys;
    int64_t n;
    int32_t n_seg, chunk;
    int32_t* perm;
    int32_t* rowptr;
    int32_t* items;
    int32_t* fix;
    int32_t items_cap, fix_cap;
    const int32_t* carry_src[3];
    int32_t* carry_out[3];
} gv_csr_job;
int64_t gv_build_csr_batch_workspace_bytes(const gv_csr_job* jobs, int n_jobs);
int gv_build_csr_batch(const gv_csr_job* jobs, int n_jobs, void* workspace, int64_t workspace_bytes, void* stream);
int gv_triplet_lists(const void* trip , int trip_is_int64, int64_t T,
                     int32_t* ent, int32_t* other, int32_t* rel2, int32_t* tid, int32_t* col_s, int32_t* col_r, int32_t* col_o,
                     int32_t* trip32 , void* stream);
int gv_widen2_i32(const int32_t* a, int64_t* a_out, int64_t na, const int32_t* b, int64_t* b_out, int64_t nb, void* stream);

int gv_perm_sample(int64_t n, int64_t k, uint64_t seed, uint64_t tick, const uint64_t* tick_dev, const int32_t* n_dev,
                   uint32_t stream_id, int32_t* out, void* stream);
int64_t gv_neighborhood_sample_workspace_bytes(int num_vertices, int64_t num_triplets);
int gv_neighborhood_sample(const int32_t* adj_ptr, const int32_t* adj_edge, const int32_t* adj_other, const int32_t* degrees,
                           int num_vertices, int64_t num_triplets, int sample_size, uint64_t seed, uint64_t tick,
                           const uint64_t* tick_dev, uint32_t stream_id, int32_t* edges, void* workspace,
                           int64_t workspace_bytes, void* stream);
int64_t gv_relabel_workspace_bytes(int num_ids);
int gv_relabel_pairs(const int32_t* a, const int32_t* b, int64_t k, int num_ids, int32_t* uniq, int uniq_cap, int32_t* a_local,
                     int32_t* b_local, int32_t* count, void* workspace, int64_t workspace_bytes, void* stream);
int gv_negative_sampling(const int32_t* s, const int32_t* r, const int32_t* o, int64_t k, int neg_rate,
                         const int32_t* n_entities_dev, const int32_t* values, const uint8_t* hit_subject, uint64_t seed,
                         uint64_t tick, const uint64_t* tick_dev, uint32_t stream_id, int64_t* samples, float* labels,
                         void* stream);
int64_t gv_graph_from_triplets_workspace_bytes(int64_t m, int n_nodes_bound, int num_rels);
int gv_graph_from_triplets(const int32_t* s, const int32_t* r, const int32_t* o, const int32_t* keep, int64_t m,
                           int n_nodes_bound, int num_rels, int32_t* src2, int32_t* dst2, int32_t* rel2, float* norm,
                           void* workspace, int64_t workspace_bytes, void* stream);
int gv_gather3_i32(const int32_t* idx, int64_t n, const int32_t* a, const int32_t* b, const int32_t* c, int32_t* out_a, int32_t* out_b,
                   int32_t* out_c, void* stream);

#ifdef __cplusplus
}
#endif
#endif
```

Measured before the change: 554.3 million edges/s.

## Batch deferred small finalize kernels into one multi-job launch per backward step

```diff
diff --git a/gcn-vae_amd/csrc/k_bdd.hip b/gcn-vae_amd/csrc/k_bdd.hip
--- a/gcn-vae_amd/csrc/k_bdd.hip
+++ b/gcn-vae_amd/csrc/k_bdd.hip
@@ -1,6 +1,7 @@
 #include <stdlib.h>
 
 #include "common.h"
+#include "k_small.h"
 
 namespace gv {
 
@@ -801,37 +802,8 @@
 
 __global__ __launch_bounds__(256) void k_gradw_fixup4(const int4* fix, int n_fix, const float* partial, int w_row,
                                                       float* grad_w, int accumulate) {
-    const int lane = threadIdx.x & 63;
-    const int quads = w_row >> 2, tiles = (quads + 63) >> 6;
     const int wave = __builtin_amdgcn_readfirstlane((int)(blockIdx.x * (blockDim.x >> 6) + (threadIdx.x >> 6)));
-    if (wave >= n_fix * tiles) return;
-    const int4 f = fix[wave / tiles];
-    if (f.x < 0) return;
-    const int c4 = (wave % tiles) * 64 + lane;
-    if (c4 >= quads) return;
-    const float4* __restrict__ p = reinterpret_cast<const float4*>(partial + (size_t)f.y * w_row) + c4;
-    const size_t stride = (size_t)quads;
-    const int n = f.z;
-    float4 a0 = make_float4(0.f, 0.f, 0.f, 0.f), a1 = a0, a2 = a0, a3 = a0;
-    auto add = [](float4& a, const float4& v) { a.x += v.x; a.y += v.y; a.z += v.z; a.w += v.w; };
-    int k = 0;
-    for (; k + 8 <= n; k += 8) {
-        const float4 v0 = p[(size_t)(k + 0) * stride], v1 = p[(size_t)(k + 1) * stride];
-        const float4 v2 = p[(size_t)(k + 2) * stride], v3 = p[(size_t)(k + 3) * stride];
-        const float4 v4 = p[(size_t)(k + 4) * stride], v5 = p[(size_t)(k + 5) * stride];
-        const float4 v6 = p[(size_t)(k + 6) * stride], v7 = p[(size_t)(k + 7) * stride];
-        add(a0, v0); add(a1, v1); add(a2, v2); add(a3, v3);
-        add(a0, v4); add(a1, v5); add(a2, v6); add(a3, v7);
-    }
-    for (; k < n; ++k) add(a0, p[(size_t)k * stride]);
-    float4 acc = make_float4((a0.x + a1.x) + (a2.x + a3.x), (a0.y + a1.y) + (a2.y + a3.y), (a0.z + a1.z) + (a2.z + a3.z),
-                             (a0.w + a1.w) + (a2.w + a3.w));
-    float4* o = reinterpret_cast<float4*>(grad_w + (size_t)f.x * w_row) + c4;
-    if (accumulate) {
-        const float4 t = *o;
-        acc.x = t.x + acc.x; acc.y = t.y + acc.y; acc.z = t.z + acc.z; acc.w = t.w + acc.w;
-    }
-    *o = acc;
+    gradw_fixup4_body(wave, fix, n_fix, partial, w_row, grad_w, accumulate);
 }
 
 __global__ void k_items_count(const int* rowptr, int n_seg, int chunk, int* n_chunks, int* n_slots, int* is_split) {
@@ -1128,7 +1100,11 @@
     GradWParams a;
     a.items = (const int4*)items; a.n_items = n_items; a.src = src; a.dst = dst; a.coef = coef; a.coef_idx = coef_idx;
     a.x = x; a.ld_x = ld_x; a.g = g; a.ld_g = ld_g; a.grad_w = grad_w; a.w_row = num_bases * blk_in * blk_out;
+    const bool defer_final = (accumulate & GV_ACC_DEFER_FINAL) != 0;
+    accumulate &= GV_ACC_ADD;
     a.partial = partial; a.accumulate = accumulate; a.nb = num_bases; a.p = blk_in; a.q = blk_out;
+    GV_REQUIRE(!defer_final || n_fix == 0 || (a.w_row % 4 == 0 && aligned16(partial) && aligned16(grad_w)), GV_ERR_SHAPE,
+               "gv_rgcn_bdd_grad_weight: GV_ACC_DEFER_FINAL needs 16-B aligned rows of a multiple of 4 columns");
     hipStream_t st = (hipStream_t)stream;
     const bool vec_ok = aligned16(x) && aligned16(g) && aligned16(grad_w) && (ld_x % 4 == 0) && (ld_g % 4 == 0) &&
                         (!partial || aligned16(partial)) && (a.w_row % 4 == 0);
@@ -1163,7 +1139,7 @@
 #undef GV_GW_CASE
     if (rc == -1000) rc = launch_items(k_gradw_generic, a, n_items, st, "gv_rgcn_bdd_grad_weight(generic)");
     if (rc != GV_OK) return rc;
-    if (n_fix > 0) {
+    if (n_fix > 0 && !defer_final) {
         if (a.w_row % 4 == 0 && aligned16(partial) && aligned16(grad_w)) {
             const int waves = n_fix * ((a.w_row / 4 + 63) / 64);
             hipLaunchKernelGGL(k_gradw_fixup4, dim3((waves + 3) / 4), dim3(256), 0, st, (const int4*)fix, n_fix, partial,
diff --git a/gcn-vae_amd/csrc/k_gemm.hip b/gcn-vae_amd/csrc/k_gemm.hip
--- a/gcn-vae_amd/csrc/k_gemm.hip
+++ b/gcn-vae_amd/csrc/k_gemm.hip
@@ -4,6 +4,7 @@
 #include <algorithm>
 
 #include "common.h"
+#include "k_small.h"
 
 namespace gv {
 
@@ -840,29 +841,8 @@
 }
 
 __global__ __launch_bounds__(256) void k_gemm_splitk_reduce(const GemmParams p) {
-    const size_t total = (size_t)p.m * p.n;
-    for (size_t i = (size_t)blockIdx.x * blockDim.x + threadIdx.x; i < total; i += (size_t)gridDim.x * blockDim.x) {
-        float a0 = 0.f, a1 = 0.f, a2 = 0.f, a3 = 0.f;
-        int z = 0;
-        for (; z + 8 <= p.split_k; z += 8) {
-            float t[8];
-#pragma unroll
-            for (int q = 0; q < 8; ++q) t[q] = p.ws[(size_t)(z + q) * total + i];
-            a0 += t[0]; a1 += t[1]; a2 += t[2]; a3 += t[3];
-            a0 += t[4]; a1 += t[5]; a2 += t[6]; a3 += t[7];
-        }
-        for (; z < p.split_k; ++z) a0 += p.ws[(size_t)z * total + i];
-        float v = (a0 + a1) + (a2 + a3);
-        const int row = (int)(i / p.n), col = (int)(i - (size_t)row * p.n);
-        if (p.tmask_wanted > 0) {
-            const int bit = (row >> 6) * p.tmask_ld + (col >> 6);
-            if (!((p.tmask[bit >> 6] >> (bit & 63)) & 1ull)) v = 0.f;
-        }
-        if (p.bias) v += p.bias[col];
-        v = apply_act(v, p.act);
-        float* dst = p.c + (size_t)row * p.ldc + col;
-        *dst = p.accumulate ? *dst + v : v;
-    }
+    splitk_reduce_body((size_t)blockIdx.x * blockDim.x + threadIdx.x, (size_t)gridDim.x * blockDim.x, p.ws, p.split_k, p.m, p.n,
+                       p.tmask, p.tmask_ld, p.tmask_wanted, p.bias, p.act, p.c, p.ldc, p.accumulate);
 }
 
 constexpr int COLSUM_SLICES = 64;
@@ -913,18 +893,18 @@
 
 __global__ __launch_bounds__(1024) void k_colsum_final_wide(const float* part, int n, int nsl, float* out, int accumulate) {
     __shared__ float sm[64][16];
-    const int c = blockIdx.x * 16 + (threadIdx.x & 15);
-    const float acc = sum_slices_16x64(part, n, nsl, c, sm);
-    if ((threadIdx.x >> 4) == 0 && c < n) out[c] = accumulate ? out[c] + acc : acc;
+    colsum_final_wide_body(blockIdx.x, part, n, nsl, out, accumulate, sm);
 }
 
 }
 
 using namespace gv;
 
-static int k_chunk_for(int k, int split_k) {
-    int per = (k + split_k - 1) / split_k;
-    return ((per + 31) / 32) * 32;
+static int k_chunk_for(int k, int split_k) { return gemm_k_chunk_for(k, split_k); }
+
+extern "C" int gv_gemm_split_count(int k, int split_k) {
+    if (k <= 0 || split_k <= 1) return 1;
+    return (k + k_chunk_for(k, split_k) - 1) / k_chunk_for(k, split_k);
 }
 
 extern "C" int64_t gv_gemm_workspace_bytes(int m, int n, int k, int split_k) {
@@ -944,6 +924,10 @@
     GV_REQUIRE(act == GV_ACT_NONE || act == GV_ACT_RELU, GV_ERR_SHAPE, "gv_gemm_f32: unknown act %d", act);
     if (split_k < 1) split_k = 1;
     if (k == 0) split_k = 1;
+    const bool defer_final = (accumulate & GV_ACC_DEFER_FINAL) != 0;
+    accumulate &= GV_ACC_ADD;
+    GV_REQUIRE(!defer_final || (!bf16 && !bias && act == GV_ACT_NONE && !tmask && !kmask && !rows_dev), GV_ERR_SHAPE,
+               "gv_gemm_f32: GV_ACC_DEFER_FINAL takes a plain fp32 product (no bias, activation, block words or live rows)");
     GemmParams p;
     p.a = a; p.b = b; p.c = c; p.bias = bias; p.a_mask = a_relu_mask; p.ws = (float*)workspace;
     p.m = m; p.n = n; p.k = k; p.lda = lda; p.ldb = ldb; p.ldc = ldc;
@@ -1012,7 +996,7 @@
 #undef GV_GEMM_CFG
     int rc = launch_status("gv_gemm_f32");
     if (rc != GV_OK) return rc;
-    if (split_k > 1) {
+    if (split_k > 1 && !defer_final) {
         const size_t total = (size_t)m * n;
         const int blocks = (int)min((size_t)2048, (total + 255) / 256);
         hipLaunchKernelGGL(k_gemm_splitk_reduce, dim3(blocks), dim3(256), 0, st, p);
diff --git a/gcn-vae_amd/csrc/k_loss.hip b/gcn-vae_amd/csrc/k_loss.hip
--- a/gcn-vae_amd/csrc/k_loss.hip
+++ b/gcn-vae_amd/csrc/k_loss.hip
@@ -1,4 +1,5 @@
 #include "common.h"
+#include "k_small.h"
 
 namespace gv {
 
@@ -781,16 +782,7 @@
                                                            float gscale, float* g_zpre, int accumulate, int64_t n, int h,
                                                            int k, int nsl, const int* rows_dev) {
     __shared__ float sm[64][16];
-    const int total = 2 * k * h, kh = k * h;
-    const int i = blockIdx.x * 16 + (threadIdx.x & 15);
-    float acc = sum_slices_16x64(part, total, nsl, i, sm);
-    if ((threadIdx.x >> 4) != 0 || i >= total) return;
-    const float cg = gscale * (gkl ? *gkl : 1.f) / (float)(rows_dev ? (int64_t)*rows_dev : n);
-    if (i >= kh) {
-        const float raw = z_pre[i];
-        acc *= raw > 20.f ? 1.f : 1.f / (1.f + expf(-raw));
-    }
-    g_zpre[i] = accumulate ? g_zpre[i] + cg * acc : cg * acc;
+    kl_bwd_mix_final_body(blockIdx.x, part, z_pre, gkl, gscale, g_zpre, accumulate, n, h, k, nsl, rows_dev, sm);
 }
 
 constexpr int MMD_WAVES = 16;
@@ -1058,6 +1050,7 @@
 }
 
 constexpr int KL_SLICES = 256;
+static_assert(KL_SLICES == GV_KL_SLICES && RED_BLOCKS == 1024, "include/gcnvae.h: GV_KL_SLICES / GV_KL_PART_OFFSET");
 constexpr int KL_FUSED_KT = 16;
 
 }
@@ -1291,8 +1284,9 @@
                       gh2))
         hipLaunchKernelGGL(k_kl_bwd_fused<KL_FUSED_KT>, dim3((h + 63) / 64, KL_SLICES), dim3(256), 0, GV_ST, z, h2, 2 * h, v,
                            (const float*)mix, resp, gkl, gscale, z_extra, none, none, none, part, n, h, k, no_rows, h2, eps, gz_up, gh2);
-    hipLaunchKernelGGL(k_kl_bwd_mix_final, dim3((2 * k * h + 15) / 16), dim3(1024), 0, GV_ST, (const float*)part, z_pre, gkl, gscale,
-                       g_zpre, accumulate_zpre, n, h, k, KL_SLICES, no_rows);
+    if (!(accumulate_zpre & GV_ACC_DEFER_FINAL))
+        hipLaunchKernelGGL(k_kl_bwd_mix_final, dim3((2 * k * h + 15) / 16), dim3(1024), 0, GV_ST, (const float*)part, z_pre, gkl, gscale,
+                           g_zpre, accumulate_zpre & GV_ACC_ADD, n, h, k, KL_SLICES, no_rows);
     return launch_status("gv_reparam_kl_bwd");
 }
 
diff --git a/gcn-vae_amd/csrc/k_small.h b/gcn-vae_amd/csrc/k_small.h
--- /dev/null
+++ b/gcn-vae_amd/csrc/k_small.h
@@ -0,0 +1,97 @@
+#pragma once
+#include "common.h"
+
+namespace gv {
+
+constexpr int SMALL_JOB_THREADS = 1024;
+
+__device__ __forceinline__ void splitk_reduce_body(size_t first, size_t stride, const float* __restrict__ ws, int split_k, int m,
+                                                   int n, const unsigned long long* tmask, int tmask_ld, int tmask_wanted,
+                                                   const float* bias, int act, float* c, int ldc, int accumulate) {
+    const size_t total = (size_t)m * n;
+    for (size_t i = first; i < total; i += stride) {
+        float a0 = 0.f, a1 = 0.f, a2 = 0.f, a3 = 0.f;
+        int z = 0;
+        for (; z + 8 <= split_k; z += 8) {
+            float t[8];
+#pragma unroll
+            for (int q = 0; q < 8; ++q) t[q] = ws[(size_t)(z + q) * total + i];
+            a0 += t[0]; a1 += t[1]; a2 += t[2]; a3 += t[3];
+            a0 += t[4]; a1 += t[5]; a2 += t[6]; a3 += t[7];
+        }
+        for (; z < split_k; ++z) a0 += ws[(size_t)z * total + i];
+        float v = (a0 + a1) + (a2 + a3);
+        const int row = (int)(i / n), col = (int)(i - (size_t)row * n);
+        if (tmask_wanted > 0) {
+            const int bit = (row >> 6) * tmask_ld + (col >> 6);
+            if (!((tmask[bit >> 6] >> (bit & 63)) & 1ull)) v = 0.f;
+        }
+        if (bias) v += bias[col];
+        v = apply_act(v, act);
+        float* dst = c + (size_t)row * ldc + col;
+        *dst = accumulate ? *dst + v : v;
+    }
+}
+
+__device__ __forceinline__ void colsum_final_wide_body(int blk, const float* part, int n, int nsl, float* out, int accumulate,
+                                                       float (*sm)[16]) {
+    const int c = blk * 16 + (threadIdx.x & 15);
+    const float acc = sum_slices_16x64(part, n, nsl, c, sm);
+    if ((threadIdx.x >> 4) == 0 && c < n) out[c] = accumulate ? out[c] + acc : acc;
+}
+
+__device__ __forceinline__ void gradw_fixup4_body(int wave, const int4* fix, int n_fix, const float* partial, int w_row,
+                                                  float* grad_w, int accumulate) {
+    const int lane = threadIdx.x & 63;
+    const int quads = w_row >> 2, tiles = (quads + 63) >> 6;
+    if (wave >= n_fix * tiles) return;
+    const int4 f = fix[wave / tiles];
+    if (f.x < 0) return;
+    const int c4 = (wave % tiles) * 64 + lane;
+    if (c4 >= quads) return;
+    const float4* __restrict__ p = reinterpret_cast<const float4*>(partial + (size_t)f.y * w_row) + c4;
+    const size_t stride = (size_t)quads;
+    const int n = f.z;
+    float4 a0 = make_float4(0.f, 0.f, 0.f, 0.f), a1 = a0, a2 = a0, a3 = a0;
+    auto add = [](float4& a, const float4& v) { a.x += v.x; a.y += v.y; a.z += v.z; a.w += v.w; };
+    int k = 0;
+    for (; k + 8 <= n; k += 8) {
+        const float4 v0 = p[(size_t)(k + 0) * stride], v1 = p[(size_t)(k + 1) * stride];
+        const float4 v2 = p[(size_t)(k + 2) * stride], v3 = p[(size_t)(k + 3) * stride];
+        const float4 v4 = p[(size_t)(k + 4) * stride], v5 = p[(size_t)(k + 5) * stride];
+        const float4 v6 = p[(size_t)(k + 6) * stride], v7 = p[(size_t)(k + 7) * stride];
+        add(a0, v0); add(a1, v1); add(a2, v2); add(a3, v3);
+        add(a0, v4); add(a1, v5); add(a2, v6); add(a3, v7);
+    }
+    for (; k < n; ++k) add(a0, p[(size_t)k * stride]);
+    float4 acc = make_float4((a0.x + a1.x) + (a2.x + a3.x), (a0.y + a1.y) + (a2.y + a3.y), (a0.z + a1.z) + (a2.z + a3.z),
+                             (a0.w + a1.w) + (a2.w + a3.w));
+    float4* o = reinterpret_cast<float4*>(grad_w + (size_t)f.x * w_row) + c4;
+    if (accumulate) {
+        const float4 t = *o;
+        acc.x = t.x + acc.x; acc.y = t.y + acc.y; acc.z = t.z + acc.z; acc.w = t.w + acc.w;
+    }
+    *o = acc;
+}
+
+__device__ __forceinline__ void kl_bwd_mix_final_body(int blk, const float* part, const float* z_pre, const float* gkl, float gscale,
+                                                      float* g_zpre, int accumulate, int64_t n, int h, int k, int nsl,
+                                                      const int* rows_dev, float (*sm)[16]) {
+    const int total = 2 * k * h, kh = k * h;
+    const int i = blk * 16 + (threadIdx.x & 15);
+    float acc = sum_slices_16x64(part, total, nsl, i, sm);
+    if ((threadIdx.x >> 4) != 0 || i >= total) return;
+    const float cg = gscale * (gkl ? *gkl : 1.f) / (float)(rows_dev ? (int64_t)*rows_dev : n);
+    if (i >= kh) {
+        const float raw = z_pre[i];
+        acc *= raw > 20.f ? 1.f : 1.f / (1.f + expf(-raw));
+    }
+    g_zpre[i] = accumulate ? g_zpre[i] + cg * acc : cg * acc;
+}
+
+inline int gemm_k_chunk_for(int k, int split_k) {
+    int per = (k + split_k - 1) / split_k;
+    return ((per + 31) / 32) * 32;
+}
+
+}
diff --git a/gcn-vae_amd/csrc/k_small.hip b/gcn-vae_amd/csrc/k_small.hip
--- /dev/null
+++ b/gcn-vae_amd/csrc/k_small.hip
@@ -0,0 +1,119 @@
+#include <limits.h>
+
+#include <algorithm>
+
+#include "common.h"
+#include "k_small.h"
+
+namespace gv {
+
+struct SmallJobs {
+    gv_small_job job[GV_SMALL_JOBS_MAX];
+    int block0[GV_SMALL_JOBS_MAX + 1];
+    int n_jobs;
+};
+
+__global__ __launch_bounds__(SMALL_JOB_THREADS) void k_small_jobs(const SmallJobs t) {
+    __shared__ float sm[64][16];
+    int j = 0;
+#pragma unroll
+    for (int q = 1; q < GV_SMALL_JOBS_MAX; ++q)
+        if (q < t.n_jobs && (int)blockIdx.x >= t.block0[q]) j = q;
+    const gv_small_job& b = t.job[j];
+    const int blk = (int)blockIdx.x - t.block0[j], nblk = t.block0[j + 1] - t.block0[j];
+    switch (b.kind) {
+    case GV_JOB_SPLITK_REDUCE:
+        splitk_reduce_body((size_t)blk * SMALL_JOB_THREADS + threadIdx.x, (size_t)nblk * SMALL_JOB_THREADS, (const float*)b.src,
+                           b.count, b.m, b.n, nullptr, 0, 0, nullptr, GV_ACT_NONE, (float*)b.out, b.ld, b.accumulate);
+        break;
+    case GV_JOB_COLSUM_FINAL:
+        colsum_final_wide_body(blk, (const float*)b.src, b.n, b.count, (float*)b.out, b.accumulate, sm);
+        break;
+    case GV_JOB_GRADW_FIXUP4:
+        gradw_fixup4_body(__builtin_amdgcn_readfirstlane(blk * (SMALL_JOB_THREADS / 64) + (int)(threadIdx.x >> 6)),
+                          (const int4*)b.fix, b.count, (const float*)b.src, b.n, (float*)b.out, b.accumulate);
+        break;
+    case GV_JOB_KL_MIX_FINAL:
+        kl_bwd_mix_final_body(blk, (const float*)b.src, (const float*)b.aux, (const float*)b.gkl, b.scale, (float*)b.out,
+                              b.accumulate, b.rows, b.m, b.n, b.count, nullptr, sm);
+        break;
+    default:
+        break;
+    }
+}
+
+}
+
+using namespace gv;
+
+static int small_job_blocks(const gv_small_job& b) {
+    switch (b.kind) {
+    case GV_JOB_SPLITK_REDUCE: {
+        if (b.m < 0 || b.n < 0 || b.count < 1 || b.ld < b.n) return -1;
+        const size_t total = (size_t)b.m * b.n;
+        return (int)std::min((size_t)2048, (total + SMALL_JOB_THREADS - 1) / SMALL_JOB_THREADS);
+    }
+    case GV_JOB_COLSUM_FINAL:
+        if (b.n < 1 || b.count < 1) return -1;
+        return (b.n + 15) / 16;
+    case GV_JOB_GRADW_FIXUP4: {
+        if (b.count < 0 || b.n < 4 || b.n % 4 != 0 || !aligned16(b.src) || !aligned16(b.out)) return -1;
+        if (b.count > 0 && !b.fix) return -1;
+        const long long waves = (long long)b.count * ((b.n / 4 + 63) / 64);
+        if (waves > (long long)INT32_MAX / 2) return -1;
+        return (int)((waves + SMALL_JOB_THREADS / 64 - 1) / (SMALL_JOB_THREADS / 64));
+    }
+    case GV_JOB_KL_MIX_FINAL:
+        if (b.m < 1 || b.n < 1 || b.count < 1 || b.rows < 1 || !b.aux || (long long)2 * b.m * b.n > INT32_MAX / 2) return -1;
+        return (2 * b.m * b.n + 15) / 16;
+    default:
+        return -1;
+    }
+}
+
+extern "C" int gv_small_jobs_plan(const gv_small_job* jobs, int n_jobs, int32_t* block0) {
+    GV_REQUIRE(n_jobs >= 0 && n_jobs <= GV_SMALL_JOBS_MAX, GV_ERR_SHAPE, "gv_small_jobs_plan: n_jobs=%d (one launch holds %d)", n_jobs,
+               GV_SMALL_JOBS_MAX);
+    GV_REQUIRE(block0 && (jobs || n_jobs == 0), GV_ERR_NULL, "gv_small_jobs: NULL job table");
+    block0[0] = 0;
+    for (int i = 0; i < n_jobs; ++i) {
+        const int nb = small_job_blocks(jobs[i]);
+        GV_REQUIRE(nb >= 0, GV_ERR_SHAPE, "gv_small_jobs: job %d (kind %d): bad sizes or alignment", i, jobs[i].kind);
+        GV_REQUIRE(nb == 0 || (jobs[i].src && jobs[i].out), GV_ERR_NULL, "gv_small_jobs: job %d: NULL pointer", i);
+        GV_REQUIRE(!(jobs[i].accumulate & ~GV_ACC_ADD), GV_ERR_SHAPE, "gv_small_jobs: job %d: accumulate=%d", i, jobs[i].accumulate);
+        block0[i + 1] = block0[i] + nb;
+    }
+    return GV_OK;
+}
+
+extern "C" int gv_small_jobs(const gv_small_job* jobs, int n_jobs, void* stream) {
+    GV_REQUIRE(n_jobs >= 0, GV_ERR_SHAPE, "gv_small_jobs: n_jobs=%d", n_jobs);
+    if (n_jobs == 0) return GV_OK;
+    GV_REQUIRE(jobs, GV_ERR_NULL, "gv_small_jobs: NULL job table");
+    for (int i0 = 0; i0 < n_jobs; i0 += GV_SMALL_JOBS_MAX) {
+        int32_t chk[GV_SMALL_JOBS_MAX + 1];
+        int rc = gv_small_jobs_plan(jobs + i0, std::min(GV_SMALL_JOBS_MAX, n_jobs - i0), chk);
+        if (rc != GV_OK) return rc;
+    }
+    for (int i0 = 0; i0 < n_jobs; i0 += GV_SMALL_JOBS_MAX) {
+        SmallJobs t;
+        t.n_jobs = 0;
+        t.block0[0] = 0;
+        for (int i = i0; i < n_jobs && i < i0 + GV_SMALL_JOBS_MAX; ++i) {
+            const int nb = small_job_blocks(jobs[i]);
+            if (nb == 0) continue;
+            t.job[t.n_jobs] = jobs[i];
+            t.block0[t.n_jobs + 1] = t.block0[t.n_jobs] + nb;
+            ++t.n_jobs;
+        }
+        if (t.n_jobs == 0) continue;
+        for (int q = t.n_jobs; q < GV_SMALL_JOBS_MAX; ++q) {
+            t.job[q] = gv_small_job{};
+            t.block0[q + 1] = t.block0[t.n_jobs];
+        }
+        hipLaunchKernelGGL(k_small_jobs, dim3(t.block0[t.n_jobs]), dim3(SMALL_JOB_THREADS), 0, (hipStream_t)stream, t);
+        int rc = launch_status("gv_small_jobs");
+        if (rc != GV_OK) return rc;
+    }
+    return GV_OK;
+}
diff --git a/gcn-vae_amd/distributed.py b/gcn-vae_amd/distributed.py
--- a/gcn-vae_amd/distributed.py
+++ b/gcn-vae_amd/distributed.py
@@ -135,6 +135,8 @@
         def fire(grad):
             self._launch(lo)
             return grad
+        from . import small_jobs as _small_jobs
+        _small_jobs.block()
         activation.register_hook(fire)
         return activation
 
diff --git a/gcn-vae_amd/lib.py b/gcn-vae_amd/lib.py
--- a/gcn-vae_amd/lib.py
+++ b/gcn-vae_amd/lib.py
@@ -50,6 +50,9 @@
     'gv_rgcn_epilogue_fwd': (_I, [_P, _P, _I, _P, _F, _P, _L, _I, _P]),
     'gv_rgcn_epilogue_bwd': (_I, [_P, _P, _I, _P, _F, _P, _L, _I, _P, _P]),
     'gv_colsum_finish': (_I, [_P, _I, _I, _P, _I, _P]),
+    'gv_small_jobs': (_I, [_P, _I, _P]),
+    'gv_small_jobs_plan': (_I, [_P, _I, _P]),
+    'gv_gemm_split_count': (_I, [_I, _I]),
     'gv_gemm_workspace_bytes': (_L, [_I, _I, _I, _I]),
     'gv_gemm_f32': (_I, [_I, _I, _I, _I, _I, _P, _I, _P, _I, _P, _I, _P, _I, _I, _I, _P, _P, _L, _P]),
     'gv_gemm_f32_live_rows': (_I, [_I, _I, _I, _I, _I, _P, _I, _P, _I, _P, _I, _P, _I, _I, _I, _P, _P, _L, _P, _P]),
diff --git a/gcn-vae_amd/ops.py b/gcn-vae_amd/ops.py
--- a/gcn-vae_amd/ops.py
+++ b/gcn-vae_amd/ops.py
@@ -91,6 +91,7 @@
 
 
 _bwd_side_others = [False]
+_bwd_side_main = []
 
 
 def rgcn_bwd_side(num_edges, width):
@@ -136,8 +137,12 @@
         return
     side, main = _side('bwd'), torch.cuda.current_stream()
     side.wait_stream(main)
-    with torch.cuda.stream(side):
-        yield True
+    _bwd_side_main.append(main)
+    try:
+        with torch.cuda.stream(side):
+            yield True
+    finally:
+        _bwd_side_main.pop()
     first = not _bwd_side_held
     _bwd_side_held.append(held)
     if not rgcn:
@@ -156,10 +161,35 @@
 
 
 def backward_side_finish():
+    flush_small_jobs()
     if _bwd_side_held:
         torch.cuda.current_stream().wait_stream(_side('bwd'))
         _bwd_side_held.clear()
     _bwd_side_others[0] = False
+
+
+def small_jobs_deferring():
+    layout = launch_layout()
+    return small_jobs.deferring(timed=layout.timed, process_group=layout.process_group)
+
+
+def defer_small_job(j, *held):
+    main = _bwd_side_main[-1] if _bwd_side_main else torch.cuda.current_stream()
+    small_jobs.defer(j, held, main, on_first=lambda: torch.autograd.Variable._execution_engine.queue_callback(flush_small_jobs))
+
+
+def flush_small_jobs():
+    if not small_jobs.pending():
+        return
+    if _bwd_side_held:
+        main = small_jobs._stream[0]
+        main.wait_stream(_side('bwd'))
+        cur = torch.cuda.current_stream()
+        if cur != main:
+            cur.wait_stream(_side('bwd'))
+        _bwd_side_held.clear()
+        _bwd_side_others[0] = False
+    small_jobs.flush()
 
 
 class StayOnDevice:
@@ -213,6 +243,7 @@
 from .indices import _carve_i32, _index_caps, _index_workspace, _rowptr_from_sorted
 from . import indices
 from . import batch_index
+from . import small_jobs
 from .batch_index import build_batch_indices
 
 
@@ -293,7 +324,7 @@
 
 
 def bdd_grad_weight(seg: SegmentItems, src, dst, coef, coef_idx, x, g, num_bases, blk_in, blk_out, out=None,
-                    accumulate=False):
+                    accumulate=False, defer_final=False):
     x, ld_x = _row_major(x, 'x')
     g, ld_g = _row_major(g, 'g')
     n_seg = seg.rowptr.numel() - 1
@@ -306,9 +337,15 @@
     partial = None
     if seg.n_fix > 0:
         partial = torch.empty(seg.n_slots, w_row, dtype=torch.float32, device=x.device)
+    defer = bool(defer_final and seg.n_fix > 0 and seg.n_items > 0 and w_row % 4 == 0 and partial.data_ptr() % 16 == 0
+                 and out.data_ptr() % 16 == 0 and out.is_contiguous() and small_jobs_deferring())
+    acc = (small_jobs.ACC_ADD if accumulate else 0) | (small_jobs.ACC_DEFER_FINAL if defer else 0)
     lib.call('gv_rgcn_bdd_grad_weight', ptr(seg.items), seg.n_items, ptr(seg.fix), seg.n_fix, ptr(src), ptr(dst),
              ptr(coef), ptr(coef_idx), ptr(x), ld_x, ptr(g), ld_g, num_bases, blk_in, blk_out, ptr(out), ptr(partial),
-             1 if accumulate else 0, lib.stream(), tag=f'gradw_{blk_in}x{blk_out}_nb{num_bases}')
+             acc, lib.stream(), tag=f'gradw_{blk_in}x{blk_out}_nb{num_bases}')
+    if defer:
+        defer_small_job(small_jobs.job(small_jobs.JOB_GRADW_FIXUP4, partial, out, accumulate, n=w_row, count=seg.n_fix, fix=seg.fix),
+                        partial, out, seg.fix)
     return out
 
 
@@ -352,7 +389,7 @@
 
 
 def gemm(a, b, trans_a=False, trans_b=False, bias=None, act=ACT_NONE, out=None, accumulate=False, split_k=1,
-         a_relu_mask=None, precision=None, b_k_chunks=None, c_tiles=None):
+         a_relu_mask=None, precision=None, b_k_chunks=None, c_tiles=None, defer_final=False):
     a, lda = _row_major(a, 'a')
     b, ldb = _row_major(b, 'b')
     m, k = (a.shape[1], a.shape[0]) if trans_a else a.shape
@@ -402,9 +439,16 @@
                  out.stride(0) if m > 1 else n, ptr(bias), act, 1 if accumulate else 0, split_k, ptr(a_relu_mask), ptr(ws),
                  ws_bytes, ptr(live[0]), lib.stream())
         return out
+    ldc = out.stride(0) if m > 1 else n
+    splits = 1
+    if defer_final and split_k > 1 and entry == 'gv_gemm_f32' and bias is None and act == ACT_NONE and m * n > 0 and k > 0 \
+            and small_jobs_deferring():
+        splits = int(lib.load().gv_gemm_split_count(k, split_k))
+    acc = (small_jobs.ACC_ADD if accumulate else 0) | (small_jobs.ACC_DEFER_FINAL if splits > 1 else 0)
     lib.call(entry, 1 if trans_a else 0, 1 if trans_b else 0, m, n, k, ptr(a), lda, ptr(b), ldb, ptr(out),
-             out.stride(0) if m > 1 else n, ptr(bias), act, 1 if accumulate else 0, split_k, ptr(a_relu_mask), ptr(ws),
-             ws_bytes, lib.stream())
+             ldc, ptr(bias), act, acc, split_k, ptr(a_relu_mask), ptr(ws), ws_bytes, lib.stream())
+    if splits > 1:
+        defer_small_job(small_jobs.job(small_jobs.JOB_SPLITK_REDUCE, ws, out, accumulate, m=m, n=n, ld=ldc, count=splits), ws, out)
     return out
 
 
@@ -579,7 +623,7 @@
     return out
 
 
-def epilogue_bwd(out, grad_out, act, keep, keep_scale, colsum_out=None, colsum_accumulate=False):
+def epilogue_bwd(out, grad_out, act, keep, keep_scale, colsum_out=None, colsum_accumulate=False, defer_final=False):
     grad_out = _chk(grad_out.contiguous(), name='grad_out')
     g = torch.empty_like(grad_out)
     m, n = grad_out.shape
@@ -587,7 +631,10 @@
     part = torch.empty(EPILOGUE_COLSUM_SLICES * n, dtype=torch.float32, device=g.device) if fused else None
     lib.call('gv_rgcn_epilogue_bwd', ptr(out), ptr(grad_out), act, ptr(keep), float(keep_scale), ptr(g), m, n, ptr(part),
              lib.stream())
-    if fused:
+    if fused and defer_final and colsum_out.is_contiguous() and small_jobs_deferring():
+        defer_small_job(small_jobs.job(small_jobs.JOB_COLSUM_FINAL, part, colsum_out, colsum_accumulate, n=n,
+                                       count=EPILOGUE_COLSUM_SLICES), part, colsum_out)
+    elif fused:
         lib.call('gv_colsum_finish', ptr(part), n, EPILOGUE_COLSUM_SLICES, ptr(colsum_out), 1 if colsum_accumulate else 0,
                  lib.stream())
     elif colsum_out is not None:
@@ -837,7 +884,8 @@
     if not want_bias:
         return epilogue_bwd(out, grad_out, act, keep, keep_scale), None
     grad_bias = d_b if d_b is not None else torch.empty(grad_out.shape[1], dtype=torch.float32, device=grad_out.device)
-    g = epilogue_bwd(out, grad_out, act, keep, keep_scale, colsum_out=grad_bias, colsum_accumulate=d_b is not None)
+    g = epilogue_bwd(out, grad_out, act, keep, keep_scale, colsum_out=grad_bias, colsum_accumulate=d_b is not None,
+                     defer_final=d_b is not None)
     return g, (None if d_b is not None else grad_bias)
 
 
@@ -866,7 +914,7 @@
     grad_loop = gx_loop = None
     if want_loop:
         grad_loop = gemm(x, g, trans_a=True, split_k=pick_split_k(x.shape[1], g.shape[1], x.shape[0]), out=d_l,
-                         accumulate=d_l is not None)
+                         accumulate=d_l is not None, defer_final=d_l is not None)
         if d_l is not None:
             grad_loop = None
     if want_x:
@@ -886,7 +934,7 @@
 def _relation_weight_grad(gidx, ridx, coef, x, g, nb, si, so, d_w):
     coef_r, idx_r = _coef_order(gidx, ridx, coef, 'rel')
     grad_w = bdd_grad_weight(ridx.by_rel.seg, ridx.src_by_rel, ridx.dst_by_rel, coef_r, idx_r, x, g, nb, si, so, out=d_w,
-                             accumulate=d_w is not None)
+                             accumulate=d_w is not None, defer_final=d_w is not None)
     return None if d_w is not None else grad_w
 
 
@@ -1719,9 +1767,17 @@
             d_zp = _direct_flat(z_pre)
             gzp = d_zp if d_zp is not None else torch.empty_like(z_pre)
             gh2 = torch.empty_like(h2)
+            k_mix = z_pre.shape[0] // 2
+            defer = d_zp is not None and small_jobs_deferring()
+            acc = (small_jobs.ACC_ADD if d_zp is not None else 0) | (small_jobs.ACC_DEFER_FINAL if defer else 0)
             lib.call('gv_reparam_kl_bwd', ptr(z), ptr(h2), ptr(v), ptr(eps), ptr(z_pre), ptr(link.resp), ptr(link.gkl),
-                     float(link.gscale), float(link.z_extra), ptr(gz), ptr(gh2), ptr(gzp), 1 if d_zp is not None else 0,
-                     ptr(link.ws), n, h, z_pre.shape[0] // 2, lib.stream())
+                     float(link.gscale), float(link.z_extra), ptr(gz), ptr(gh2), ptr(gzp), acc,
+                     ptr(link.ws), n, h, k_mix, lib.stream())
+            if defer:
+                part = link.ws.data_ptr() + 4 * small_jobs.kl_part_offset(h, k_mix)
+                defer_small_job(small_jobs.job(small_jobs.JOB_KL_MIX_FINAL, part, gzp, True, m=h, n=k_mix, count=small_jobs.KL_SLICES,
+                                               scale=float(link.gscale), rows=n, aux=z_pre, gkl=link.gkl),
+                                link.ws, gzp, z_pre, link.gkl)
             link.gkl = None
             if gm is not None or gv is not None:
                 extra = torch.empty_like(h2)
diff --git a/gcn-vae_amd/small_jobs.py b/gcn-vae_amd/small_jobs.py
--- /dev/null
+++ b/gcn-vae_amd/small_jobs.py
@@ -0,0 +1,91 @@
+import ctypes as _ct
+import os as _os
+
+import torch
+
+from . import lib
+from .lib import ptr
+
+JOB_SPLITK_REDUCE, JOB_COLSUM_FINAL, JOB_GRADW_FIXUP4, JOB_KL_MIX_FINAL = 0, 1, 2, 3
+ACC_ADD, ACC_DEFER_FINAL = 1, 2
+SMALL_JOBS_MAX = 16
+KL_SLICES = 256
+
+
+def kl_part_offset(h, k):
+    return 3 * k * h + 1024
+
+
+class _SmallJob(_ct.Structure):
+    _fields_ = [('kind', _ct.c_int32), ('accumulate', _ct.c_int32), ('m', _ct.c_int32), ('n', _ct.c_int32), ('ld', _ct.c_int32),
+                ('count', _ct.c_int32), ('scale', _ct.c_float), ('reserved', _ct.c_int32), ('rows', _ct.c_int64),
+                ('src', _ct.c_void_p), ('fix', _ct.c_void_p), ('aux', _ct.c_void_p), ('gkl', _ct.c_void_p), ('out', _ct.c_void_p)]
+
+
+def job(kind, src, out, accumulate=False, m=0, n=0, ld=0, count=0, scale=0.0, rows=0, fix=None, aux=None, gkl=None):
+    def addr(t):
+        return ptr(t) if isinstance(t, torch.Tensor) else t
+    j = _SmallJob()
+    j.kind, j.accumulate, j.m, j.n, j.ld, j.count = int(kind), ACC_ADD if accumulate else 0, int(m), int(n), int(ld), int(count)
+    j.scale, j.rows = float(scale), int(rows)
+    j.src, j.fix, j.aux, j.gkl, j.out = addr(src), addr(fix), addr(aux), addr(gkl), addr(out)
+    return j
+
+
+def plan(jobs):
+    arr = (_SmallJob * max(1, len(jobs)))(*jobs)
+    block0 = (_ct.c_int32 * (len(jobs) + 1))()
+    lib.call('gv_small_jobs_plan', _ct.addressof(arr), len(jobs), _ct.addressof(block0))
+    return list(block0)
+
+
+def launch(jobs):
+    if jobs:
+        arr = (_SmallJob * len(jobs))(*jobs)
+        lib.call('gv_small_jobs', _ct.addressof(arr), len(jobs), lib.stream())
+
+
+_pending = []
+_stream = [None]
+_blocked = [False]
+
+
+def enabled():
+    return _os.environ.get('GV_STEP_BATCH_SMALL', '1') != '0'
+
+
+def block():
+    _blocked[0] = True
+
+
+def deferring(timed=False, process_group=False):
+    return (enabled() and not _blocked[0] and not timed and not process_group
+            and torch._C._current_graph_task_id() != -1)
+
+
+def pending():
+    return len(_pending)
+
+
+def defer(j, held, stream, on_first=None):
+    first = not _pending
+    _pending.append((j, held))
+    if first:
+        _stream[0] = stream
+        if on_first is not None:
+            on_first()
+
+
+def flush():
+    if not _pending:
+        return
+    jobs = [j for j, _ in _pending]
+    main, cur = _stream[0], torch.cuda.current_stream()
+    try:
+        with torch.cuda.stream(main):
+            launch(jobs)
+        if cur != main:
+            cur.wait_stream(main)
+    finally:
+        _pending.clear()
+        _stream[0] = None
diff --git a/include/gcnvae.h b/include/gcnvae.h
--- a/include/gcnvae.h
+++ b/include/gcnvae.h
@@ -16,6 +16,7 @@
 } gv_status;
 
 enum { GV_ACT_NONE = 0, GV_ACT_RELU = 1 };
+enum { GV_ACC_ADD = 1, GV_ACC_DEFER_FINAL = 2 };
 
 int gv_version(void);
 const char* gv_last_error_string(void);
@@ -430,6 +431,28 @@
 int gv_gather3_i32(const int32_t* idx, int64_t n, const int32_t* a, const int32_t* b, const int32_t* c, int32_t* out_a, int32_t* out_b,
                    int32_t* out_c, void* stream);
 
+enum { GV_JOB_SPLITK_REDUCE = 0, GV_JOB_COLSUM_FINAL = 1, GV_JOB_GRADW_FIXUP4 = 2, GV_JOB_KL_MIX_FINAL = 3 };
+#define GV_SMALL_JOBS_MAX 16
+#define GV_KL_SLICES 256
+#define GV_KL_PART_OFFSET(h, k) (3 * (int64_t)(k) * (h) + 1024)
+typedef struct gv_small_job {
+    int32_t kind;
+    int32_t accumulate;
+    int32_t m, n, ld;
+    int32_t count;
+    float scale;
+    int32_t reserved;
+    int64_t rows;
+    const void* src;
+    const void* fix;
+    const void* aux;
+    const void* gkl;
+    void* out;
+} gv_small_job;
+int gv_small_jobs(const gv_small_job* jobs, int n_jobs, void* stream);
+int gv_small_jobs_plan(const gv_small_job* jobs, int n_jobs, int32_t* block0);
+int gv_gemm_split_count(int k, int split_k);
+
 #ifdef __cplusplus
 }
 #endif
```

Measured after the change: 560.1 million edges/s (median of 6 runs). 1.0% higher.
